# simonamtoft/downsampled-diffusion

Measured on AMD Instinct MI355X. Metric: images/sec (T=1000 sampling), 256x256 dDDPM-x3, higher is better.
Workload: dtype f32

## Files before the change

### downsampled-diffusion_amd/csrc/attention.hip

```cpp
#include <cstdlib>

#include "cluster_sync.h"
#include "conv_common.h"

namespace ddk {

constexpr int DH = 32;

constexpr int PART = DH + DH + DH * DH;

__global__ __launch_bounds__(256) void linattn_context_kernel(const float* __restrict__ qkv, float* __restrict__ ctx,
                                                              float* __restrict__ part, int HW, int heads, int splits, int rows_per_split,
                                                              int kv_only) {
    __shared__ __attribute__((aligned(16))) float stage[4 * 32 * 33];
    float* kexp = stage;
    float* vs = stage + 64 * DH;
    __shared__ float smax[8 * DH];
    const int bh = blockIdx.x / splits, sp = blockIdx.x % splits;
    const int b = bh / heads, h = bh % heads;
    const int HC = heads * DH, RS = (kv_only ? 2 : 3) * HC;
    const float* base = qkv + (long long)b * HW * RS;
    const float* kp = base + (kv_only ? 0 : HC) + h * DH;
    const float* vp = kp + HC;
    const int tid = threadIdx.x;
// ... 501 lines not shown
    if constexpr (ROWS >= 128) linattn_core_mfma<ROWS>(ks, vs, qs, cs, smax, part, ctx, out, b, h, HW, heads);
    else linattn_small_core<ROWS>(ks, vs, qs, cs, smax, ctx, out, b, h, HW, heads);
}

static size_t small_lds_bytes(int rows) {
    return ((size_t)rows * DH * 2 + (size_t)rows * (DH + 1) + DH * (DH + 4) + 16 * DH + (rows >= 128 ? 4 * 32 * 33 : 0)) * 4;
}

typedef float f32x4_att __attribute__((ext_vector_type(4)));
constexpr int QP_PITCH = 100;

__host__ __device__ static inline size_t small_qkv_lds_bytes(int MB, int C) {
    const size_t xs = (size_t)16 * MB * (C + 4), part = (size_t)4 * 16 * MB * QP_PITCH;
    const size_t core = 64 * DH * 2 + 64 * (DH + 1) + DH * (DH + 4) + 8 * DH + 128 + 192;
    return ((xs > part ? xs : part) + core) * 4;
}

template <int MB>
__global__ __launch_bounds__(256) void linattn_small_qkv_kernel(const float* __restrict__ x, const float* __restrict__ wop,
                                                                const float* __restrict__ c1, const float* __restrict__ c2, float ln_eps,
                                                                float* __restrict__ ctx, float* __restrict__ out, int HW, int C, int heads) {
    extern __shared__ __align__(16) float sm[];
    constexpr int ROWS = 16 * MB;
    const int pitch = C + 4, nch = C >> 5;
    const size_t big = (size_t)ROWS * pitch > (size_t)4 * ROWS * QP_PITCH ? (size_t)ROWS * pitch : (size_t)4 * ROWS * QP_PITCH;
    float* xs = sm;
    float* ks = sm + big;
    float* vs = ks + 64 * DH;
    float* qs = vs + 64 * DH;
    float* cs = qs + 64 * (DH + 1);
    float* smax = cs + DH * (DH + 4);
    float* rowstat = smax + 8 * DH;
    float* cfold = rowstat + 128;
    const int b = blockIdx.x / heads, h = blockIdx.x % heads;
    const int tid = threadIdx.x, lane = tid & 63;
    const int wave = __builtin_amdgcn_readfirstlane(tid >> 6);
    const int m = lane & 15, kq = lane >> 4;
    const int HC = heads * DH;

    const float* wl = wop + (size_t)h * nch * 3072 + lane * 4;
    float4 bA[6][2], bB[6][2];
    auto load_b = [&](int chunk, float4 (&bq)[6][2]) {
        chunk = chunk < nch ? chunk : nch - 1;
        const float* wp = wl + (size_t)chunk * 3072;
#pragma unroll
        for (int nb = 0; nb < 6; ++nb) {
            bq[nb][0] = *reinterpret_cast<const float4*>(wp + nb * 512);
            bq[nb][1] = *reinterpret_cast<const float4*>(wp + nb * 512 + 256);
        }
    };
    load_b(wave, bA);
    load_b(wave + 4, bB);
    if (tid < 192) {
        const int n = tid % 96;
        const int col = (n >> 5) * HC + h * DH + (n & 31);
        cfold[tid] = tid < 96 ? c1[col] : c2[col];
    }
    {
        const int q4 = C >> 2;
        for (int i = tid; i < ROWS * q4; i += 256) {
            const int row = i / q4, c = (i - row * q4) << 2;
            const float4 v = row < HW ? *reinterpret_cast<const float4*>(x + ((long long)b * HW + row) * C + c) : make_float4(0.f, 0.f, 0.f, 0.f);
            *reinterpret_cast<float4*>(xs + row * pitch + c) = v;
        }
    }
    __syncthreads();
    {
        constexpr int TPR = 256 / ROWS;
        const int row = tid / TPR, sub = tid % TPR;
        float s1 = 0.f;
        for (int c = sub * 4; c < C; c += TPR * 4) {
            const float4 v = *reinterpret_cast<const float4*>(xs + row * pitch + c);
            s1 += (v.x + v.y) + (v.z + v.w);
        }
#pragma unroll
        for (int o = 1; o < TPR; o <<= 1) s1 += __shfl_xor(s1, o, 64);
        const float inv_c = 1.0f / (float)C;
        const float mean = s1 * inv_c;
        float s2 = 0.f;
        for (int c = sub * 4; c < C; c += TPR * 4) {
            const float4 v = *reinterpret_cast<const float4*>(xs + row * pitch + c);
            const float a0 = v.x - mean, a1 = v.y - mean, a2 = v.z - mean, a3 = v.w - mean;
            s2 += (a0 * a0 + a1 * a1) + (a2 * a2 + a3 * a3);
        }
#pragma unroll
        for (int o = 1; o < TPR; o <<= 1) s2 += __shfl_xor(s2, o, 64);
        if (sub == 0) {
            const float var = s2 * inv_c;
            const float r = 1.0f / (sqrtf(var) + ln_eps);
            rowstat[2 * row] = r;
            rowstat[2 * row + 1] = r * mean;
        }
    }

    f32x4_att acc[MB][6];
#pragma unroll
    for (int i = 0; i < MB; ++i)
#pragma unroll
        for (int nb = 0; nb < 6; ++nb) acc[i][nb] = f32x4_att{0.f, 0.f, 0.f, 0.f};
    auto compute = [&](int chunk, const float4 (&bq)[6][2]) {
        float4 a[MB][2];
#pragma unroll
        for (int i = 0; i < MB; ++i) {
            const float* ap = xs + (i * 16 + m) * pitch + (chunk << 5) + kq * 8;
            a[i][0] = *reinterpret_cast<const float4*>(ap);
            a[i][1] = *reinterpret_cast<const float4*>(ap + 4);
        }
#pragma unroll
        for (int kk = 0; kk < 8; ++kk)
#pragma unroll
            for (int i = 0; i < MB; ++i) {
                const float av = reinterpret_cast<const float*>(&a[i][0])[kk];
#pragma unroll
                for (int nb = 0; nb < 6; ++nb)
                    acc[i][nb] = __builtin_amdgcn_mfma_f32_16x16x4f32(av, reinterpret_cast<const float*>(&bq[nb][0])[kk], acc[i][nb], 0, 0, 0);
            }
    };
    for (int c = wave; c < nch; c += 8) {
        compute(c, bA);
        load_b(c + 8, bA);
        if (c + 4 < nch) compute(c + 4, bB);
        load_b(c + 12, bB);
    }
    __syncthreads();
#pragma unroll
    for (int i = 0; i < MB; ++i)
#pragma unroll
        for (int nb = 0; nb < 6; ++nb)
#pragma unroll
            for (int r = 0; r < 4; ++r) xs[((wave * ROWS) + i * 16 + kq * 4 + r) * QP_PITCH + nb * 16 + m] = acc[i][nb][r];
    __syncthreads();
    for (int e = tid; e < ROWS * 96; e += 256) {
        const int row = e / 96, n = e - row * 96;
        const int sel = n >> 5, d = n & 31;
        float v = sel == 1 ? -INFINITY : 0.f;
        if (row < HW) {
            float s = xs[row * QP_PITCH + n];
#pragma unroll
            for (int w = 1; w < 4; ++w) s += xs[(w * ROWS + row) * QP_PITCH + n];
            v = rowstat[2 * row] * s - rowstat[2 * row + 1] * cfold[n] + cfold[96 + n];
        }
        if (sel == 0) qs[row * (DH + 1) + d] = v;
        else if (sel == 1) ks[row * DH + d] = v;
        else vs[row * DH + d] = v;
    }
    __syncthreads();
    linattn_small_core<ROWS>(ks, vs, qs, cs, smax, ctx, out, b, h, HW, heads);
}

constexpr int AS_REC = 1152;
constexpr int AS_CNT = 32;
constexpr int AS_RING = 4;

template <int ROWS>
struct AttnSplitGeom {
    static_assert(ROWS == 128 || ROWS == 32, "half of a 16x16 or of an 8x8 map");
    static constexpr int XP = ROWS / 8;
    static constexpr int NP = XP + 12;
    static constexpr int SLOT = (ROWS + 96) * 32;
    static constexpr int NB = ROWS == 128 ? 3 : 1;
    static constexpr int UNITS = ROWS == 128 ? 4 : 3;
    static constexpr int KPART = UNITS * NB * 16 * 64;
    static constexpr int SCR = KPART > 8 * 32 * 33 ? KPART : 8 * 32 * 33;
    static constexpr int RING_FL = AS_RING * SLOT;
    static_assert(SCR + 2 * ROWS * DH + ROWS * (DH + 1) <= RING_FL, "k, v, q of the half live behind the scratch area in the drained ring");
    static constexpr int TAIL = DH * (DH + 4) + 2 * ROWS + 16 * DH + 16 * DH + DH + 192 + AS_REC + 32;
    static constexpr int LDS_FL = RING_FL + TAIL;
};

struct AttnSplitParams {
    const float* x;
    const float* w;
    const float* c1;
    const float* c2;
    float eps;
    float* ctx;
    float* out;
    unsigned* cnt;
    float* rec;
    unsigned* fail;
    int C;
};

__device__ __forceinline__ void wait_vmcnt_le(int n) {
    if (n >= 8) wait_vmcnt<8>();
    else if (n >= 6) wait_vmcnt<6>();
    else if (n >= 4) wait_vmcnt<4>();
    else if (n >= 3) wait_vmcnt<3>();
    else if (n >= 2) wait_vmcnt<2>();
    else wait_vmcnt<0>();
}

template <int ROWS>
__global__ __launch_bounds__(512) void attn_split_kernel(const AttnSplitParams p) {
    using G = AttnSplitGeom<ROWS>;
    constexpr int HW = 2 * ROWS, HC = 4 * DH;
    extern __shared__ __attribute__((aligned(16))) float smem[];
    float* scr = smem;
    float* ks = smem + G::SCR;
    float* vs = ks + ROWS * DH;
    float* qs = vs + ROWS * DH;
    float* cs = smem + G::RING_FL;
    float* rowstat = cs + DH * (DH + 4);
    float* smax = rowstat + 2 * ROWS;
    float* dpart = smax + 16 * DH;
    float* mx = dpart + 16 * DH;
    float* cfold = mx + DH;
    float* own = cfold + 192;
    int* gave_up = reinterpret_cast<int*>(own + AS_REC);
    const int tid = threadIdx.x, lane = tid & 63;
    const int wid = __builtin_amdgcn_readfirstlane(tid >> 6);
    const int half = blockIdx.x, h = blockIdx.y, b = blockIdx.z;
    const int C = p.C, nch = C >> 5;
    const float* xb = p.x + ((long long)b * HW + half * ROWS) * C;
    const unsigned lds_base = (unsigned)(size_t)(__attribute__((address_space(3))) float*)smem;

    const int prow = lane >> 3, ppos = lane & 7;
    const int npw = (G::NP - wid + 7) >> 3;
    unsigned voff[4];
#pragma unroll
    for (int j = 0; j < 4; ++j) {
        const int pj = wid + 8 * j;
        const int r = 8 * (pj < G::XP ? pj : pj - G::XP) + prow;
        const int src = pj < G::XP ? r : (r >> 5) * HC + h * DH + (r & 31);
        voff[j] = (unsigned)((src * C + ((ppos ^ ((r >> 1) & 7)) << 2)) * 4);
    }
    auto issue = [&](int chunk) {
        const unsigned dst = lds_base + (unsigned)(((chunk & (AS_RING - 1)) * G::SLOT) * 4);
#pragma unroll
        for (int j = 0; j < 4; ++j) {
            const int pj = wid + 8 * j;
            if (pj < G::NP) lds_dma16_s(pj < G::XP ? xb : p.w, voff[j] + (unsigned)(chunk * 128), dst + (unsigned)(pj * 1024));
        }
    };
    for (int c = 0; c < AS_RING - 1 && c < nch; ++c) issue(c);
    if (tid < 192) {
        const int n = tid % 96;
        const int col = (n >> 5) * HC + h * DH + (n & 31);
        cfold[tid] = tid < 96 ? p.c1[col] : p.c2[col];
    }
    if (tid < 4 * ROWS) {
        const int row = tid >> 2, sub = tid & 3, n16 = C >> 4;
        const float4* rp = reinterpret_cast<const float4*>(xb + (long long)row * C);
        float4 v[16];
        float s = 0.f;
#pragma unroll
        for (int i = 0; i < 16; ++i)
            if (i < n16) {
                v[i] = rp[sub + 4 * i];
                s += (v[i].x + v[i].y) + (v[i].z + v[i].w);
            }
        s += __shfl_xor(s, 1, 64);
        s += __shfl_xor(s, 2, 64);
        const float inv_c = 1.0f / (float)C;
        const float mean = s * inv_c;
        float qq = 0.f;
#pragma unroll
        for (int i = 0; i < 16; ++i)
            if (i < n16) {
                const float a0 = v[i].x - mean, a1 = v[i].y - mean, a2 = v[i].z - mean, a3 = v[i].w - mean;
                qq += (a0 * a0 + a1 * a1) + (a2 * a2 + a3 * a3);
            }
        qq += __shfl_xor(qq, 1, 64);
        qq += __shfl_xor(qq, 2, 64);
        if (sub == 0) {
            const float r = 1.0f / (sqrtf(qq * inv_c) + p.eps);
            rowstat[2 * row] = r;
            rowstat[2 * row + 1] = r * mean;
        }
    }

    const int pl = lane & 31, hl = lane >> 5;
    const bool active = ROWS == 128 || wid < 6;
    const int kh = ROWS == 128 ? wid >> 2 : (wid >= 3 ? 1 : 0);
    const int unit = ROWS == 128 ? (wid & 3) : (wid >= 3 ? wid - 3 : wid);
    const int pb = ROWS == 128 ? unit : 0, blk0 = ROWS == 128 ? 0 : unit;
    f32x16 acc[G::NB];
#pragma unroll
    for (int i = 0; i < G::NB; ++i)
#pragma unroll
        for (int r = 0; r < 16; ++r) acc[i][r] = 0.f;
    const int fsw = (pl >> 1) & 7;
    for (int c = 0; c < nch; ++c) {
        const int later = nch - 1 - c < AS_RING - 2 ? nch - 1 - c : AS_RING - 2;
        wait_vmcnt_le(later * npw);
        asm volatile("s_waitcnt lgkmcnt(0)\n\ts_barrier" ::: "memory");
        if (c + AS_RING - 1 < nch) issue(c + AS_RING - 1);
        if (active) {
            const float* Xs = smem + (c & (AS_RING - 1)) * G::SLOT + pb * (32 * 32);
            const float* Ws = smem + (c & (AS_RING - 1)) * G::SLOT + ROWS * 32 + blk0 * (32 * 32);
#pragma unroll
            for (int q2 = 0; q2 < 2; ++q2) {
                const int off = pl * 32 + (((2 * (2 * kh + q2) + hl) ^ fsw) << 2);
                const float4 xv = *reinterpret_cast<const float4*>(Xs + off);
                float4 wv[G::NB];
#pragma unroll
                for (int i = 0; i < G::NB; ++i) wv[i] = *reinterpret_cast<const float4*>(Ws + i * (32 * 32) + off);
#pragma unroll
                for (int e = 0; e < 4; ++e) {
                    const float xe = e == 0 ? xv.x : e == 1 ? xv.y : e == 2 ? xv.z : xv.w;
#pragma unroll
                    for (int i = 0; i < G::NB; ++i)
                        acc[i] = __builtin_amdgcn_mfma_f32_32x32x2f32(e == 0 ? wv[i].x : e == 1 ? wv[i].y : e == 2 ? wv[i].z : wv[i].w, xe, acc[i], 0, 0, 0);
                }
            }
        }
    }
    __syncthreads();
    if (active && kh == 1) {
#pragma unroll
        for (int i = 0; i < G::NB; ++i)
#pragma unroll
            for (int r = 0; r < 16; ++r) scr[((unit * G::NB + i) * 16 + r) * 64 + lane] = acc[i][r];
    }
    __syncthreads();
    if (active && kh == 0) {
        const int n = pb * 32 + pl;
        const float r = rowstat[2 * n], rm = rowstat[2 * n + 1];
#pragma unroll
        for (int i = 0; i < G::NB; ++i) {
            const int blk = blk0 + i;
#pragma unroll
            for (int q = 0; q < 4; ++q) {
                const int d0 = 8 * q + 4 * hl;
                float o4[4];
#pragma unroll
                for (int e = 0; e < 4; ++e) {
                    const float a = acc[i][4 * q + e] + scr[((unit * G::NB + i) * 16 + 4 * q + e) * 64 + lane];
                    o4[e] = r * a - rm * cfold[blk * 32 + d0 + e] + cfold[96 + blk * 32 + d0 + e];
                }
                if (blk == 0) {
#pragma unroll
                    for (int e = 0; e < 4; ++e) qs[n * (DH + 1) + d0 + e] = o4[e];
                } else {
                    *reinterpret_cast<float4*>((blk == 1 ? ks : vs) + n * DH + d0) = make_float4(o4[0], o4[1], o4[2], o4[3]);
                }
            }
        }
    }
    __syncthreads();

    {
        const int d = tid & 31, ng = tid >> 5;
        float m = -INFINITY;
        for (int n = ng; n < ROWS; n += 16) m = fmaxf(m, ks[n * DH + d]);
        smax[ng * DH + d] = m;
        __syncthreads();
        if (tid < DH) {
            float mm = smax[tid];
#pragma unroll
            for (int j = 1; j < 16; ++j) mm = fmaxf(mm, smax[j * DH + tid]);
            mx[tid] = mm;
        }
        __syncthreads();
#pragma unroll
        for (int j = 0; j < ROWS / 16; ++j) {
            const int i = tid + j * 512;
            ks[i] = __expf(ks[i] - mx[i & 31]);
        }
        __syncthreads();
        float t = 0.f;
        for (int n = ng; n < ROWS; n += 16) t += ks[n * DH + d];
        dpart[ng * DH + d] = t;
    }
    {
        constexpr int RPW = ROWS / 8;
        f32x16 cacc;
#pragma unroll
        for (int r = 0; r < 16; ++r) cacc[r] = 0.f;
        const float* kp = ks + (wid * RPW + hl) * DH + pl;
        const float* vp = vs + (wid * RPW + hl) * DH + pl;
#pragma unroll
        for (int j = 0; j < RPW / 2; ++j) cacc = __builtin_amdgcn_mfma_f32_32x32x2f32(kp[j * 2 * DH], vp[j * 2 * DH], cacc, 0, 0, 0);
#pragma unroll
        for (int r = 0; r < 16; ++r) scr[(wid * 32 + (r & 3) + 8 * (r >> 2) + 4 * hl) * 33 + pl] = cacc[r];
    }
    __syncthreads();
    const int md = (tid >> 3) & 31, me0 = (tid & 7) * 4;
    if (tid < 256) {
        float den = 0.f;
#pragma unroll
        for (int g = 0; g < 16; ++g) den += dpart[g * DH + md];
#pragma unroll
        for (int e = 0; e < 4; ++e) {
            float t = scr[md * 33 + me0 + e];
#pragma unroll
            for (int w = 1; w < 8; ++w) t += scr[(w * 32 + md) * 33 + me0 + e];
            own[2 * DH + md * DH + me0 + e] = t;
        }
        if (me0 == 0) { own[md] = mx[md]; own[DH + md] = den; }
    }
    __syncthreads();
    unsigned* cnt = p.cnt + (b * 4 + h) * AS_CNT;
    float* rec = p.rec + (long long)(b * 4 + h) * 2 * AS_REC;
    if (wid == 0) {
        unsigned* mine = reinterpret_cast<unsigned*>(rec + half * AS_REC);
#pragma unroll
        for (int i = 0; i < (2 * DH + DH * DH) / 64; ++i)
            __hip_atomic_store(mine + lane + 64 * i, __float_as_uint(own[lane + 64 * i]), __ATOMIC_RELAXED, __HIP_MEMORY_SCOPE_AGENT);
        asm volatile("s_waitcnt vmcnt(0)" ::: "memory");
        if (lane == 0) {
            __hip_atomic_fetch_add(cnt, 1u, __ATOMIC_RELAXED, __HIP_MEMORY_SCOPE_AGENT);
            *gave_up = cl_wait_ge<2>(cnt, 2u, p.fail) ? 1 : 0;
        }
    }
    __syncthreads();
    const bool poisoned = *gave_up != 0;
    if (tid < 256) {
        const unsigned* theirs = reinterpret_cast<const unsigned*>(rec + (half ^ 1) * AS_REC);
        const float tm = __uint_as_float(__hip_atomic_load(theirs + md, __ATOMIC_RELAXED, __HIP_MEMORY_SCOPE_AGENT));
        const float td = __uint_as_float(__hip_atomic_load(theirs + DH + md, __ATOMIC_RELAXED, __HIP_MEMORY_SCOPE_AGENT));
        float ta[4];
#pragma unroll
        for (int e = 0; e < 4; ++e)
            ta[e] = __uint_as_float(__hip_atomic_load(theirs + 2 * DH + md * DH + me0 + e, __ATOMIC_RELAXED, __HIP_MEMORY_SCOPE_AGENT));
        if (tid == 0) cl_depart(cnt, cnt + 1, 2u);
        const float om = own[md], od = own[DH + md];
        const float m0 = half ? tm : om, m1 = half ? om : tm;
        const float d0 = half ? td : od, d1 = half ? od : td;
        const float M = fmaxf(m0, m1);
        const float w0 = expf(m0 - M), w1 = expf(m1 - M);
        float den = 0.f;
        den += d0 * w0;
        den += d1 * w1;
        const float inv = poisoned ? __builtin_nanf("") : 1.0f / den;
        float c4[4];
#pragma unroll
        for (int e = 0; e < 4; ++e) {
            const float oa = own[2 * DH + md * DH + me0 + e];
            const float a0 = half ? ta[e] : oa, a1 = half ? oa : ta[e];
            float a = 0.f;
            a += a0 * w0;
            a += a1 * w1;
            c4[e] = a * inv;
            cs[md * (DH + 4) + me0 + e] = c4[e];
        }
        if (half == 0) *reinterpret_cast<float4*>(p.ctx + (((long long)b * 4 + h) * DH + md) * DH + me0) = make_float4(c4[0], c4[1], c4[2], c4[3]);
    }
    __syncthreads();
    if (wid < ROWS / 32) {
        const int n0 = wid * 32;
        f32x16 oacc;
#pragma unroll
        for (int r = 0; r < 16; ++r) oacc[r] = 0.f;
        const float* qp = qs + (n0 + pl) * (DH + 1) + hl;
        const float* cp = cs + hl * (DH + 4) + pl;
#pragma unroll
        for (int j = 0; j < DH / 2; ++j) oacc = __builtin_amdgcn_mfma_f32_32x32x2f32(qp[2 * j], cp[2 * j * (DH + 4)], oacc, 0, 0, 0);
        float* op = p.out + ((long long)b * HW + half * ROWS + n0) * HC + h * DH + pl;
#pragma unroll
        for (int r = 0; r < 16; ++r) op[((r & 3) + 8 * (r >> 2) + 4 * hl) * HC] = oacc[r];
    }
}

__global__ __launch_bounds__(256) void qkv_operand_pack_kernel(const float* __restrict__ lnw, float* __restrict__ wop, int heads, int cp,
                                                               long long total) {
    const int nch = cp >> 5, HC = heads * DH;
    for (long long idx = blockIdx.x * 256LL + threadIdx.x; idx < total; idx += (long long)gridDim.x * 256) {
        const int j = (int)(idx & 3), lane = (int)((idx >> 2) & 63), half = (int)((idx >> 8) & 1);
        long long r = idx >> 9;
        const int nb = (int)(r % 6); r /= 6;
        const int chunk = (int)(r % nch);
        const int head = (int)(r / nch);
        const int o = (nb >> 1) * HC + head * DH + (nb & 1) * 16 + (lane & 15);
        const int i = chunk * 32 + (lane >> 4) * 8 + half * 4 + j;
        wop[idx] = lnw[(long long)o * cp + i];
    }
}

typedef float f32x16_att __attribute__((ext_vector_type(16)));
__global__ __launch_bounds__(512) void linattn_apply_kernel(const float* __restrict__ qkv, const float* __restrict__ ctx,
                                                            float* __restrict__ out, int HW, int heads, int tiles_per_sample) {
    extern __shared__ __attribute__((aligned(16))) float qs[];
    const int b = blockIdx.x / tiles_per_sample, tile = blockIdx.x % tiles_per_sample;
    const int HC = heads * DH, RS = 3 * HC;
    const int nthreads = 64 * heads;
    const int n0 = tile * 64;
    const int f4_per_row = HC / 4;
    for (int i = threadIdx.x; i < 64 * f4_per_row; i += nthreads) {
        const int row = i / f4_per_row, c4 = i - row * f4_per_row;
        float4 v = make_float4(0.f, 0.f, 0.f, 0.f);
        if (n0 + row < HW) v = *reinterpret_cast<const float4*>(qkv + ((long long)b * HW + n0 + row) * RS + c4 * 4);
        const int hh = (c4 * 4) / DH, d = (c4 * 4) % DH;
        float* dst = qs + (hh * 64 + row) * 33 + d;
        dst[0] = v.x; dst[1] = v.y; dst[2] = v.z; dst[3] = v.w;
    }
    const int h = threadIdx.x >> 6, lane = threadIdx.x & 63;
    const int l31 = lane & 31, fh = lane >> 5;
    const float* cp = ctx + ((long long)b * heads + h) * DH * DH + l31;
    float bf[16];
#pragma unroll
    for (int kk = 0; kk < 16; ++kk) bf[kk] = cp[(2 * kk + fh) * DH];
    __syncthreads();
    const float* qh = qs + h * 64 * 33;
    f32x16_att acc0, acc1;
#pragma unroll
    for (int r = 0; r < 16; ++r) { acc0[r] = 0.f; acc1[r] = 0.f; }
#pragma unroll
    for (int kk = 0; kk < 16; ++kk) {
        const float a0 = qh[l31 * 33 + 2 * kk + fh], a1 = qh[(32 + l31) * 33 + 2 * kk + fh];
        acc0 = __builtin_amdgcn_mfma_f32_32x32x2f32(a0, bf[kk], acc0, 0, 0, 0);
        acc1 = __builtin_amdgcn_mfma_f32_32x32x2f32(a1, bf[kk], acc1, 0, 0, 0);
    }
#pragma unroll
    for (int r = 0; r < 16; ++r) {
        const int px = (r & 3) + 8 * (r >> 2) + 4 * fh;
        if (n0 + px < HW) out[((long long)b * HW + n0 + px) * HC + h * DH + l31] = acc0[r];
        if (n0 + 32 + px < HW) out[((long long)b * HW + n0 + 32 + px) * HC + h * DH + l31] = acc1[r];
    }
}

static void linattn_splits(int B, int HW, int heads, int& splits, int& rows) {
    const int max_s = (int)ceil_div(HW, 64);
#ifdef DDK_TUNING
    const char* cap_env = getenv("DDK_LINATTN_WGS");
    const int cap = cap_env ? atoi(cap_env) : 1024;
#else
    const int cap = 1024;
#endif
    int s = cap / (B * heads);
    if (s < 1) s = 1;
    if (s > max_s) s = max_s;
    rows = (int)(ceil_div(ceil_div(HW, s), 64) * 64);
    splits = (int)ceil_div(HW, rows);
}

size_t linattn_context_workspace_bytes(int B, int HW, int heads) {
    if (B <= 0 || HW <= 0 || heads <= 0) return 0;
    int s, rows;
    linattn_splits(B, HW, heads, s, rows);
    return s > 1 ? (size_t)B * heads * s * PART * sizeof(float) : 0;
}

int linattn_context(const float* qkv, float* ctx, int B, int HW, int heads, void* workspace, size_t workspace_bytes, hipStream_t st,
                    bool kv_only) {
    DDK_REQUIRE(qkv && ctx && B > 0 && HW > 0 && heads > 0, "linattn_context: arguments");
    DDK_REQUIRE(aligned16(qkv) && aligned16(ctx) && aligned16(workspace), "linattn_context: alignment");
    int s, rows;
    linattn_splits(B, HW, heads, s, rows);
    if (s > 1 && (!workspace || workspace_bytes < (size_t)B * heads * s * PART * sizeof(float))) {
        if (workspace) {
            set_error("linattn_context: workspace too small (%zu < %zu)", workspace_bytes, (size_t)B * heads * s * PART * sizeof(float));
            return DDK_ERR_WORKSPACE;
        }
        s = 1;
        rows = HW;
    }
    hipLaunchKernelGGL(linattn_context_kernel, dim3(B * heads * s), dim3(256), 0, st, qkv, ctx, static_cast<float*>(workspace), HW, heads, s, rows,
                       kv_only ? 1 : 0);
    DDK_TRY(check_launch("linattn_context_kernel"));
    if (s > 1) {
        hipLaunchKernelGGL(linattn_merge_kernel, dim3(B * heads), dim3(256), 0, st, static_cast<const float*>(workspace), ctx, s);
        DDK_TRY(check_launch("linattn_merge_kernel"));
    }
    return DDK_OK;
}

int linattn_fused_small(const float* qkv, float* ctx, float* out, int B, int HW, int heads, hipStream_t st) {
    DDK_REQUIRE(qkv && ctx && out && B > 0 && HW > 0 && HW <= 256 && heads > 0, "linattn_fused_small: arguments (HW <= 256)");
    DDK_REQUIRE(aligned16(qkv) && aligned16(ctx) && aligned16(out), "linattn_fused_small: alignment");
    DDK_TRY(ensure_device_init());
    if (HW <= 64)
        hipLaunchKernelGGL(linattn_small_kernel<64>, dim3(B * heads), dim3(256), small_lds_bytes(64), st, qkv, ctx, out, HW, heads);
    else
        hipLaunchKernelGGL(linattn_small_kernel<256>, dim3(B * heads), dim3(256), small_lds_bytes(256), st, qkv, ctx, out, HW, heads);
    return check_launch("linattn_small_kernel");
}

bool linattn_small_qkv_ok(int HW, int C) { return HW > 0 && HW <= 64 && C % 32 == 0 && C >= 32 && small_qkv_lds_bytes(HW <= 16 ? 1 : 4, C) <= 160 * 1024; }

constexpr int FOLD_C = 128;
constexpr int FOLD_LDS_FLOATS = FOLD_C * FOLD_C + 32 * (FOLD_C + 1) + 2 * FOLD_C;
typedef float f32x16_att __attribute__((ext_vector_type(16)));
__global__ __launch_bounds__(256) void attn_fold_kernel(const float* __restrict__ ctx, const float* __restrict__ wqg,
                                                        const float* __restrict__ c1q, const float* __restrict__ c2q,
                                                        const float* __restrict__ wout, const float* __restrict__ bout,
                                                        float* __restrict__ A, float* __restrict__ a1, float* __restrict__ a2) {
    extern __shared__ __align__(16) float sm[];
    float* T = sm;
    float* Wq = T + FOLD_C * FOLD_C;
    float* t1 = Wq + 32 * (FOLD_C + 1);
    float* t2 = t1 + FOLD_C;
    const int b = blockIdx.x, nq = blockIdx.y, tid = threadIdx.x, lane = tid & 63;
    const int wave = __builtin_amdgcn_readfirstlane(tid >> 6);
    const int l31 = lane & 31, kh = lane >> 5;
    {
        const float* cp = ctx + ((long long)b * 4 + wave) * DH * DH;
        const float* wp = wqg + (long long)wave * DH * FOLD_C;
        f32x16_att acc[4];
#pragma unroll
        for (int j = 0; j < 4; ++j)
#pragma unroll
            for (int r = 0; r < 16; ++r) acc[j][r] = 0.f;
        float av[DH / 2], bv[DH / 2][4];
#pragma unroll
        for (int s2 = 0; s2 < DH / 2; ++s2) {
            const int d = 2 * s2 + kh;
            av[s2] = cp[d * DH + l31];
#pragma unroll
            for (int j = 0; j < 4; ++j) bv[s2][j] = wp[d * FOLD_C + j * 32 + l31];
        }
        __builtin_amdgcn_sched_barrier(0);
#pragma unroll
        for (int s2 = 0; s2 < DH / 2; ++s2)
#pragma unroll
            for (int j = 0; j < 4; ++j) acc[j] = __builtin_amdgcn_mfma_f32_32x32x2f32(av[s2], bv[s2][j], acc[j], 0, 0, 0);
#pragma unroll
        for (int j = 0; j < 4; ++j)
#pragma unroll
            for (int r = 0; r < 16; ++r) T[(wave * DH + (r & 3) + 8 * (r >> 2) + 4 * kh) * FOLD_C + j * 32 + l31] = acc[j][r];
    }
    for (int i = tid; i < 32 * FOLD_C; i += 256) Wq[(i >> 7) * (FOLD_C + 1) + (i & 127)] = wout[(long long)nq * 32 * FOLD_C + i];
    if (tid < FOLD_C) {
        const int h = tid >> 5, e = tid & 31;
        const float* ch = ctx + ((long long)b * 4 + h) * DH * DH;
        float u1 = 0.f, u2 = 0.f;
#pragma unroll
        for (int d = 0; d < DH; ++d) {
            const float cv = ch[d * DH + e];
            u1 += cv * c1q[h * DH + d];
            u2 += cv * c2q[h * DH + d];
        }
        t1[tid] = u1;
        t2[tid] = u2;
    }
    __syncthreads();
    {
        f32x16_att acc;
#pragma unroll
        for (int r = 0; r < 16; ++r) acc[r] = 0.f;
#pragma unroll 8
        for (int s2 = 0; s2 < FOLD_C / 2; ++s2) {
            const int he = 2 * s2 + kh;
            acc = __builtin_amdgcn_mfma_f32_32x32x2f32(Wq[l31 * (FOLD_C + 1) + he], T[he * FOLD_C + wave * 32 + l31], acc, 0, 0, 0);
        }
        float* Ab = A + ((long long)b * FOLD_C + nq * 32) * FOLD_C + wave * 32 + l31;
#pragma unroll
        for (int r = 0; r < 16; ++r) Ab[((r & 3) + 8 * (r >> 2) + 4 * kh) * FOLD_C] = acc[r];
        if (tid < 32) {
            float u1 = 0.f, u2 = 0.f;
#pragma unroll 16
            for (int he = 0; he < FOLD_C; ++he) {
                u1 += Wq[tid * (FOLD_C + 1) + he] * t1[he];
                u2 += Wq[tid * (FOLD_C + 1) + he] * t2[he];
            }
            const int n = nq * 32 + tid;
            a1[(long long)b * FOLD_C + n] = u1;
            a2[(long long)b * FOLD_C + n] = u2 + (bout ? bout[n] : 0.f);
        }
    }
}

int linattn_small_qkv_init_device() {
    DDK_HIP(hipFuncSetAttribute(reinterpret_cast<const void*>(attn_kvctx_kernel), hipFuncAttributeMaxDynamicSharedMemorySize,
                                (int)(KC_LDS_FLOATS * sizeof(float))));
    DDK_HIP(hipFuncSetAttribute(reinterpret_cast<const void*>(attn_fold_kernel), hipFuncAttributeMaxDynamicSharedMemorySize,
                                (int)(FOLD_LDS_FLOATS * sizeof(float))));
    DDK_HIP(hipFuncSetAttribute(reinterpret_cast<const void*>(linattn_small_kernel<256>), hipFuncAttributeMaxDynamicSharedMemorySize, 160 * 1024));
    DDK_HIP(hipFuncSetAttribute(reinterpret_cast<const void*>(linattn_small_qkv_kernel<1>), hipFuncAttributeMaxDynamicSharedMemorySize, 160 * 1024));
    DDK_HIP(hipFuncSetAttribute(reinterpret_cast<const void*>(linattn_small_qkv_kernel<4>), hipFuncAttributeMaxDynamicSharedMemorySize, 160 * 1024));
    DDK_HIP(hipFuncSetAttribute(reinterpret_cast<const void*>(attn_split_kernel<128>), hipFuncAttributeMaxDynamicSharedMemorySize,
                                (int)(AttnSplitGeom<128>::LDS_FL * sizeof(float))));
    DDK_HIP(hipFuncSetAttribute(reinterpret_cast<const void*>(attn_split_kernel<32>), hipFuncAttributeMaxDynamicSharedMemorySize,
                                (int)(AttnSplitGeom<32>::LDS_FL * sizeof(float))));
    return DDK_OK;
}

int qkv_operand_pack(const float* lnw, float* wop, int heads, int cp, hipStream_t st) {
    DDK_REQUIRE(lnw && wop && heads > 0 && cp > 0 && cp % 32 == 0, "qkv_operand_pack: arguments");
    const long long total = (long long)3 * heads * DH * cp;
    const long long blocks = ceil_div(total, 256);
    hipLaunchKernelGGL(qkv_operand_pack_kernel, dim3((unsigned)(blocks < 2048 ? blocks : 2048)), dim3(256), 0, st, lnw, wop, heads, cp, total);
    return check_launch("qkv_operand_pack_kernel");
}

int linattn_small_qkv(const float* x, const float* wop, const float* c1, const float* c2, float ln_eps, float* ctx, float* out, int B, int HW,
                      int C, int heads, hipStream_t st) {
    DDK_REQUIRE(x && wop && c1 && c2 && ctx && out && B > 0 && heads > 0, "linattn_small_qkv: arguments");
    DDK_REQUIRE(linattn_small_qkv_ok(HW, C), "linattn_small_qkv: needs H*W <= 64 and C % 32 == 0 (LDS budget)");
    DDK_REQUIRE(aligned16(x) && aligned16(wop) && aligned16(ctx) && aligned16(out), "linattn_small_qkv: alignment");
    DDK_TRY(ensure_device_init());
    if (HW <= 16)
        hipLaunchKernelGGL(linattn_small_qkv_kernel<1>, dim3(B * heads), dim3(256), small_qkv_lds_bytes(1, C), st, x, wop, c1, c2, ln_eps, ctx, out,
                           HW, C, heads);
    else
        hipLaunchKernelGGL(linattn_small_qkv_kernel<4>, dim3(B * heads), dim3(256), small_qkv_lds_bytes(4, C), st, x, wop, c1, c2, ln_eps, ctx, out,
                           HW, C, heads);
    return check_launch("linattn_small_qkv_kernel");
}

bool attn_kvctx_ok(int B, int HW, int C, int heads) { return B > 0 && C == KC_K && heads == 4 && HW >= 4 * KC_BM && HW % KC_BM == 0; }
int attn_kvctx_splits(int B, int HW) {
    const int tiles = HW / KC_BM;
    int s = 1;
    while (s * 2 <= tiles && tiles % (s * 2) == 0 && (long long)B * 2 * (s * 2) <= 256) s *= 2;
    return s;
}
size_t attn_kvctx_workspace_bytes(int B, int HW) { return (size_t)B * 4 * attn_kvctx_splits(B, HW) * PART * sizeof(float); }

int attn_kvctx(const float* x, const float* w_kv, const float* c1, const float* c2, float ln_eps, float* ctx, int B, int HW, void* workspace,
               size_t workspace_bytes, hipStream_t st) {
    DDK_REQUIRE(x && w_kv && c1 && c2 && ctx && workspace, "attn_kvctx: null pointer");
    DDK_REQUIRE(attn_kvctx_ok(B, HW, KC_K, 4), "attn_kvctx: needs 128 channels, 4 heads, H*W a multiple of 64 and >= 256");
    DDK_REQUIRE(aligned16(x) && aligned16(w_kv) && aligned16(c1) && aligned16(c2) && aligned16(ctx) && aligned16(workspace), "attn_kvctx: alignment");
    DDK_REQUIRE((long long)B * HW * KC_K * 4 < (1LL << 32) && B <= 65535, "attn_kvctx: input of 4 GiB or more, or more than 65535 images");
    const int s = attn_kvctx_splits(B, HW);
    if (workspace_bytes < attn_kvctx_workspace_bytes(B, HW)) {
        set_error("attn_kvctx: workspace too small (%zu < %zu)", workspace_bytes, attn_kvctx_workspace_bytes(B, HW));
        return DDK_ERR_WORKSPACE;
    }
    DDK_TRY(ensure_device_init());
    KvCtxParams p{x, w_kv, c1, c2, ln_eps, static_cast<float*>(workspace), HW / KC_BM, HW / KC_BM / s, s};
    hipLaunchKernelGGL(attn_kvctx_kernel, dim3((unsigned)s, 2, (unsigned)B), dim3(512), KC_LDS_FLOATS * sizeof(float), st, p);
    DDK_TRY(check_launch("attn_kvctx_kernel"));
    hipLaunchKernelGGL(linattn_merge_kernel, dim3(B * 4), dim3(256), 0, st, static_cast<const float*>(workspace), ctx, s);
    return check_launch("linattn_merge_kernel");
}

constexpr int AS_CUS = 256;
bool attn_split_ok(int B, int HW, int C, int heads) {
    return B > 0 && (HW == 64 || HW == 256) && C >= 32 && C <= 256 && C % 32 == 0 && heads == 4 && 8 * (long long)B <= AS_CUS &&
           conv_wino_cluster_device_ok();
}
size_t attn_split_counter_words(int B) { return (size_t)B * 4 * AS_CNT; }
size_t attn_split_record_floats(int B) { return (size_t)B * 4 * 2 * AS_REC; }
size_t attn_split_workspace_bytes(int B) { return B > 0 ? (32 + attn_split_counter_words(B) + attn_split_record_floats(B)) * sizeof(float) : 0; }
unsigned attention_cluster_timeouts() { return cl_timeouts_read(); }

int attn_split(const float* x, const float* w, const float* c1, const float* c2, float ln_eps, float* ctx, float* out, int B, int HW, int C,
               unsigned* counters, float* records, unsigned* fail, hipStream_t st) {
    DDK_REQUIRE(x && w && c1 && c2 && ctx && out && counters && records, "attn_split: null pointer");
    DDK_REQUIRE(attn_split_ok(B, HW, C, 4), "attn_split: needs H*W of 64 or 256, C % 32 == 0, C <= 256, 4 heads, 8 * B <= the CU count of a whole MI355X");
    DDK_REQUIRE(aligned16(x) && aligned16(w) && aligned16(ctx) && aligned16(out) && aligned16(counters) && aligned16(records), "attn_split: alignment");
    DDK_TRY(ensure_device_init());
    const AttnSplitParams p{x, w, c1, c2, ln_eps, ctx, out, counters, records, fail, C};
    if (HW == 256)
        hipLaunchKernelGGL(attn_split_kernel<128>, dim3(2, 4, (unsigned)B), dim3(512), AttnSplitGeom<128>::LDS_FL * sizeof(float), st, p);
    else
        hipLaunchKernelGGL(attn_split_kernel<32>, dim3(2, 4, (unsigned)B), dim3(512), AttnSplitGeom<32>::LDS_FL * sizeof(float), st, p);
    return check_launch("attn_split_kernel");
}

bool attn_fold_ok(int C, int heads) { return C == FOLD_C && heads * DH == FOLD_C; }
size_t attn_fold_out_floats(int B) { return (size_t)B * (FOLD_C * FOLD_C + 2 * FOLD_C); }

int attn_fold(const float* ctx, const float* wqg, const float* c1q, const float* c2q, const float* wout, const float* bout, float* A,
              float* a1, float* a2, int B, int C, int heads, hipStream_t st) {
    DDK_REQUIRE(ctx && wqg && c1q && c2q && wout && A && a1 && a2 && B > 0, "attn_fold: arguments");
    DDK_REQUIRE(attn_fold_ok(C, heads), "attn_fold: C == 128 and heads * 32 == 128 only");
    DDK_REQUIRE(aligned16(ctx) && aligned16(wout) && aligned16(A), "attn_fold: alignment");
    DDK_TRY(ensure_device_init());
    hipLaunchKernelGGL(attn_fold_kernel, dim3(B, 4), dim3(256), FOLD_LDS_FLOATS * sizeof(float), st, ctx, wqg, c1q, c2q, wout, bout, A, a1, a2);
    return check_launch("attn_fold_kernel");
}

int linattn_apply(const float* qkv, const float* ctx, float* out, int B, int HW, int heads, hipStream_t st) {
    DDK_REQUIRE(qkv && ctx && out && B > 0 && HW > 0, "linattn_apply: arguments");
    DDK_REQUIRE(heads >= 1 && heads <= 8, "linattn_apply: heads must be in 1..8");
    DDK_REQUIRE(aligned16(qkv) && aligned16(ctx) && aligned16(out), "linattn_apply: alignment");
    const int tiles = (int)ceil_div(HW, 64);
    const size_t lds = (size_t)heads * 64 * 33 * sizeof(float);
    hipLaunchKernelGGL(linattn_apply_kernel, dim3(B * tiles), dim3(64 * heads), lds, st, qkv, ctx, out, HW, heads, tiles);
    return check_launch("linattn_apply_kernel");
}

}

extern "C" {
size_t ddk_linattn_context_workspace_bytes(int B, int HW, int heads) { return ddk::linattn_context_workspace_bytes(B, HW, heads); }
int ddk_linattn_context(const float* qkv, float* ctx, int B, int HW, int heads, void* workspace, size_t workspace_bytes, ddk_stream_t s) {
    return ddk::linattn_context(qkv, ctx, B, HW, heads, workspace, workspace_bytes, ddk::as_stream(s), false);
}
int ddk_linattn_context_kv(const float* kv, float* ctx, int B, int HW, int heads, void* workspace, size_t workspace_bytes, ddk_stream_t s) {
    return ddk::linattn_context(kv, ctx, B, HW, heads, workspace, workspace_bytes, ddk::as_stream(s), true);
}
size_t ddk_attention_kv_context_workspace_bytes(int B, int HW) { return ddk::attn_kvctx_workspace_bytes(B, HW); }
int ddk_attention_kv_context_ok(int B, int HW, int C, int heads) { return ddk::attn_kvctx_ok(B, HW, C, heads) ? 1 : 0; }
int ddk_attention_kv_context(const float* x, const float* w_kv, const float* c1, const float* c2, float ln_eps, float* ctx, int B, int HW,
                             void* workspace, size_t workspace_bytes, ddk_stream_t s) {
    return ddk::attn_kvctx(x, w_kv, c1, c2, ln_eps, ctx, B, HW, workspace, workspace_bytes, ddk::as_stream(s));
}
size_t ddk_attention_split_workspace_bytes(int B) { return ddk::attn_split_workspace_bytes(B); }
int ddk_attention_split_ok(int B, int HW, int C, int heads) { return ddk::attn_split_ok(B, HW, C, heads) ? 1 : 0; }
int ddk_attention_split_from_x(const float* x, const float* w_folded, const float* c1, const float* c2, float ln_eps, float* ctx, float* out,
                               int B, int HW, int C, int heads, void* workspace, size_t workspace_bytes, ddk_stream_t s) {
    using namespace ddk;
    DDK_REQUIRE(workspace && B > 0 && heads == 4, "attention_split_from_x: arguments (4 heads)");
    if (workspace_bytes < attn_split_workspace_bytes(B)) {
        set_error("attention_split_from_x: workspace too small (%zu < %zu)", workspace_bytes, attn_split_workspace_bytes(B));
        return DDK_ERR_WORKSPACE;
    }
    unsigned* words = static_cast<unsigned*>(workspace);
    return attn_split(x, w_folded, c1, c2, ln_eps, ctx, out, B, HW, C, words + 32, static_cast<float*>(workspace) + 32 + attn_split_counter_words(B),
                      words, as_stream(s));
}
int ddk_attention_fold(const float* ctx, const float* wqg, const float* c1q, const float* c2q, const float* wout, const float* bout, float* A,
                       float* a1, float* a2, int B, int C, int heads, ddk_stream_t s) {
    return ddk::attn_fold(ctx, wqg, c1q, c2q, wout, bout, A, a1, a2, B, C, heads, ddk::as_stream(s));
}
int ddk_linattn_fused_small(const float* qkv, float* ctx, float* out, int B, int HW, int heads, ddk_stream_t s) {
    return ddk::linattn_fused_small(qkv, ctx, out, B, HW, heads, ddk::as_stream(s));
}
int ddk_pack_qkv_operand(const float* folded_w, float* dst, int heads, int c_pad, ddk_stream_t s) {
    return ddk::qkv_operand_pack(folded_w, dst, heads, c_pad, ddk::as_stream(s));
}
int ddk_linattn_small_from_x(const float* x, const float* w_operand, const float* c1, const float* c2, float ln_eps, float* ctx, float* out,
                             int B, int HW, int C, int heads, ddk_stream_t s) {
    return ddk::linattn_small_qkv(x, w_operand, c1, c2, ln_eps, ctx, out, B, HW, C, heads, ddk::as_stream(s));
}
int ddk_linattn_apply(const float* qkv, const float* ctx, float* out, int B, int HW, int heads, ddk_stream_t s) {
    return ddk::linattn_apply(qkv, ctx, out, B, HW, heads, ddk::as_stream(s));
}
}
```

### downsampled-diffusion_amd/csrc/ddk_internal.h

```cpp
#pragma once
#include <hip/hip_runtime.h>

#include <cstdarg>
#include <cstddef>
#include <cstdint>
#include <cstdio>

#include "ddk.h"

#ifdef DDK_HOST_SANITIZE
#include "host_sanitize.h"
#endif

namespace ddk {

void set_error(const char* fmt, ...);

inline int fail_arg(const char* what) {
    set_error("bad argument: %s", what);
    return DDK_ERR_ARG;
}

inline int check_launch(const char* what) {
    hipError_t e = hipGetLastError();
// ... 67 lines not shown
    const int lane = threadIdx.x & 63, wid = threadIdx.x >> 6, nw = blockDim.x >> 6;
    __syncthreads();
    if (lane == 0) red[wid] = v;
    __syncthreads();
    float t = (lane < nw) ? red[lane] : 0.0f;
    t = wave_sum(t);
    return t;
}

__device__ __forceinline__ float block_max(float v, float* red) {
    v = wave_max(v);
    const int lane = threadIdx.x & 63, wid = threadIdx.x >> 6, nw = blockDim.x >> 6;
    __syncthreads();
    if (lane == 0) red[wid] = v;
    __syncthreads();
    float t = (lane < nw) ? red[lane] : -INFINITY;
    t = wave_max(t);
    return t;
}

int ensure_device_init();
int conv_init_device();
int wgrad_init_device();

size_t conv_workspace_bytes(int kind, int B, int H, int W, int cin, int N);
struct ConvLnFold {
    const float* c1;
    const float* c2;
    float eps;
};
struct WinoGnFuse {
    const float* gamma;
    const float* beta;
    const float* temb;
    const long long* temb_rows;
    int temb_stride;
    float eps;
    int groups;
    float* records;
    unsigned* counters;
    unsigned* fail;
    unsigned* pairs = nullptr;
    const float* res_x = nullptr;
    const float* res_w = nullptr;
    const float* res_b = nullptr;
    int res_cin = 0, res_ld = 0;
};
bool conv_ln_fold_ok(int B, int H, int W, int cin, int N);
int conv_forward(const ddk_conv_args& a, hipStream_t st, const ConvLnFold* ln = nullptr, const WinoGnFuse* fuse = nullptr);
int conv_splits(int kind, int B, int H, int W, int cin, int N);
bool conv_wino_ok(int kind, int H, int W, int cin, int N);
int conv_wino_splits(int B, int H, int W, int cin, int N);
int conv_wino_forward(const ddk_conv_args& a, int splits, hipStream_t st, const WinoGnFuse* fuse = nullptr);
int conv_wino_cluster_np(int B, int H, int W, int cin, int N, int groups);
int conv_wino_cluster_split_np(int B, int H, int W, int cin, int N, int groups, int* splits_out);
size_t conv_wino_cluster_pair_words(int B, int H, int W, int N);
bool conv_wino_variant_new(int B, int H, int W, int N);
bool conv_wino_cluster_device_ok();
size_t conv_wino_cluster_ws_floats(int B, int H, int W, int N);
unsigned conv_wino_cluster_timeouts();
unsigned conv_first_cluster_timeouts();
unsigned level_chain_cluster_timeouts();
unsigned attention_cluster_timeouts();
constexpr size_t CL_PAIR_WORDS = 128 * 16;
inline size_t cl_fail_offset(int B) { return (size_t)B * 8 * 16; }
inline size_t cl_front_floats(int B) { return cl_fail_offset(B) + 16; }
inline size_t cl_chain_offset(int B) { return cl_front_floats(B); }
inline size_t cl_pair_offset(int B) { return cl_chain_offset(B) + (size_t)B * 64; }
inline size_t cl_attn_offset(int B) { return cl_pair_offset(B) + CL_PAIR_WORDS; }
inline size_t cl_counter_floats(int B) { return cl_attn_offset(B) + (size_t)B * 4 * 32; }
struct ClWords { unsigned* counters; unsigned* fail; };
inline ClWords cl_words(float* cl, int B) { return {reinterpret_cast<unsigned*>(cl), reinterpret_cast<unsigned*>(cl + cl_fail_offset(B))}; }
int cluster_fail_check(unsigned* word, hipStream_t st, const char* who, const char* tail);
bool convT_wino_ok(int H, int W, int cin, int N);
int convT_wino_splits(int B, int H, int W, int cin, int N);
int convT_wino_forward(const ddk_conv_args& a, int splits, hipStream_t st);
int conv_wino_init_device();
int conv_wino_stats_parts(int B, int H, int W, int cin, int N, int groups);
bool conv_first_ok(int cin, int N, int H, int W, int groups);
int conv_first(const float* x, const float* wp, const float* bias, float* out, float* gn_partials, int B, int H, int W, int cin, int N,
               int groups, int64_t* counter, int64_t* t_cur, hipStream_t st);
int conv_first_init_device();
bool conv_first_gn_ok(int cin, int N, int H, int W, int groups);
size_t conv_first_gn_ws_floats(int B, int H, int W);
int conv_first_gn(const float* x, const float* wp, const float* bias, const float* gamma, const float* beta, const float* temb,
                  int temb_stride, const long long* temb_rows, float eps, float* out, int B, int H, int W, int cin, int N, int groups,
                  float* records, unsigned* counters, unsigned* fail, int64_t* counter, int64_t* t_cur, hipStream_t st);
bool conv1x1_sm_ok(long long M, int c0, int c1, int N);
int conv1x1_sm(const float* src0, int c0, const float* src1, int c1, const float* w, const float* bias, const float* resid, float* out,
               long long M, int N, const ConvLnFold* ln, hipStream_t st);
int conv1x1_sm_init_device();
bool conv1x1_stream_ok(long long M, int cin, int N);
int conv1x1_stream(const float* x, int cin, const float* w, const float* bias, const float* dmish_src, const float* resid, float* out,
                   float* mish_out, long long M, int N, int pre_mish, int post_mish, hipStream_t st);
bool conv1x1_ws_ok(long long M, int K, int N);
int conv1x1_ws(const float* x, const float* w, const float* bias, const float* resid, float* out, long long M, int N, const ConvLnFold* ln,
               hipStream_t st, int images = 0);
int conv1x1_ws_init_device();
struct AddendSlabs {
    int n = 1;
    long long stride = 0;
    const float* bias = nullptr;
};
bool conv_gn_local_ok(int H, int W, int cin, int c0, int N, int groups);
int conv_gn_local(const float* src0, int c0, const float* src1, int c1, const float* w, const float* bias, const float* gamma,
                  const float* beta, const float* temb, int temb_stride, const long long* temb_rows, const float* addend, float* out,
                  int B, int H, int W, int N, int groups, float eps, hipStream_t st, const AddendSlabs& as = AddendSlabs(),
                  const AddendSlabs& src_slabs = AddendSlabs());
int conv_gn_local_init_device();
bool conv_gn_wlocal_ok(int H, int W, int cin, int c0, int N, int groups);
int conv_gn_wlocal(const float* src0, int c0, const float* src1, int c1, const float* w, const float* bias, const float* gamma,
                   const float* beta, const float* temb, int temb_stride, const long long* temb_rows, const float* addend, float* out,
                   int B, int H, int W, int N, int groups, float eps, hipStream_t st, const AddendSlabs& as = AddendSlabs(),
                   const AddendSlabs& src_slabs = AddendSlabs());
double conv_flops(int kind, int B, int H, int W, int cin, int N);
size_t groupnorm_workspace_bytes(int B, int HW, int C, int groups);
int gn_train_nsplit(int HW, int cpg);
int gn_stats_partials(const float* x, float* part, int B, int HW, int C, int groups, int ns, hipStream_t st);
int groupnorm_mish(const float* x, const float* gamma, const float* beta, const float* temb, int temb_stride,
                   const float* addend, float* out, int B, int HW, int C, int groups, float eps, void* ws, size_t ws_bytes,
                   hipStream_t st, const long long* temb_rows = nullptr);
int groupnorm_mish_ex(const float* x, int nslab, long long slab_stride, const float* cbias, const float* gamma,
                      const float* beta, const float* temb, int temb_stride, const float* addend, float* out, int B, int HW, int C,
                      int groups, float eps, void* ws, size_t ws_bytes, hipStream_t st, const long long* temb_rows = nullptr);
int groupnorm_mish_parts(const float* x, const float* part, int np, const float* gamma, const float* beta, const float* temb,
                         int temb_stride, const float* addend, float* out, int B, int HW, int C, int groups, float eps, hipStream_t st,
                         const long long* temb_rows = nullptr, const float* rc_x = nullptr, const float* rc_w = nullptr,
                         const float* rc_b = nullptr, int rc_cin = 0, int rc_ld = 0);
int chan_layernorm(const float* x, const float* g, const float* b, float* out, long long M, int C, float eps, hipStream_t st);
int groupnorm_mish_generic(const float* x, const float* gamma, const float* beta, const float* temb, int temb_stride, const float* addend,
                           float* out, int B, int HW, int CP, int C, int groups, float eps, hipStream_t st, const long long* temb_rows = nullptr);
int chan_layernorm_generic(const float* x, const float* g, const float* b, float* out, long long M, int CP, int C, float eps, hipStream_t st);
int unary(int op, const float* x, float* out, long long n, hipStream_t st);
int add(const float* a, const float* b, float* out, long long n, hipStream_t st);
int avgpool2(const float* x, float* out, int B, int H, int W, int C, hipStream_t st);
int upsample_nearest2(const float* x, float* out, int B, int H, int W, int C, hipStream_t st);
size_t linattn_context_workspace_bytes(int B, int HW, int heads);
int linattn_context(const float* qkv, float* ctx, int B, int HW, int heads, void* workspace, size_t workspace_bytes, hipStream_t st,
                    bool kv_only = false);
bool attn_fold_ok(int C, int heads);
bool attn_kvctx_ok(int B, int HW, int C, int heads);
size_t attn_kvctx_workspace_bytes(int B, int HW);
int attn_kvctx(const float* x, const float* w_kv, const float* c1, const float* c2, float ln_eps, float* ctx, int B, int HW, void* workspace,
               size_t workspace_bytes, hipStream_t st);
size_t attn_fold_out_floats(int B);
int attn_fold(const float* ctx, const float* wqg, const float* c1q, const float* c2q, const float* wout, const float* bout, float* A,
              float* a1, float* a2, int B, int C, int heads, hipStream_t st);
int linattn_apply(const float* qkv, const float* ctx, float* out, int B, int HW, int heads, hipStream_t st);
int linattn_fused_small(const float* qkv, float* ctx, float* out, int B, int HW, int heads, hipStream_t st);
bool attn_split_ok(int B, int HW, int C, int heads);
size_t attn_split_counter_words(int B);
size_t attn_split_record_floats(int B);
int attn_split(const float* x, const float* w, const float* c1, const float* c2, float ln_eps, float* ctx, float* out, int B, int HW, int C,
               unsigned* counters, float* records, unsigned* fail, hipStream_t st);
bool linattn_small_qkv_ok(int HW, int C);
int linattn_small_qkv_init_device();
int qkv_operand_pack(const float* lnw, float* wop, int heads, int cp, hipStream_t st);
int linattn_small_qkv(const float* x, const float* wop, const float* c1, const float* c2, float ln_eps, float* ctx, float* out, int B, int HW,
                      int C, int heads, hipStream_t st);
int time_mlp(const int64_t* t, const float* freqs, const float* w1t, const float* b1, const float* w2t, const float* b2,
             float* act, float* raw, int B, int dim, hipStream_t st);
int time_proj(const float* act, const float* wt, const float* bias, float* out, int B, int dim, int n_out, hipStream_t st);
int conv1x1_small_n(const float* x, const float* w, const float* bias, float* out, long long M, int C, int n_out, hipStream_t st);
struct InpaintOps {
    const float* known;
    const float* mask;
    const float *ka, *kb;
    const float *ja, *jb;
};
struct NoisyTables {
    const float *lam, *sgm;
};
constexpr uint32_t INPAINT_Z2_BIT = 0x40000000u;
constexpr uint32_t INPAINT_Z3_BIT = 0x20000000u;
struct RestoreOps {
    const float* y;
    int n;
    int H, W;
    int gray;
    const float* mask;
};
static_assert(sizeof(RestoreOps) == 32 && offsetof(RestoreOps, mask) == 24, "RestoreOps: gray fills the padding, nothing moves");
constexpr int GRAY_MEAN = 1;
constexpr int GRAY_LUMA = 2;
struct VlbStep {
    const float* x;
    float* xt;
    const float* noise;
    long long noise_step_stride;
    int t_first;
    const float *c_recip, *c_recipm1, *c1, *c2, *logvar;
    float* partials;
    int nslot;
};
constexpr uint32_t VLB_STREAM_BIT = 0x80000000u;

enum class StepKind {
    Eps,
    Ancestral,
    Multistep,
    Inpaint,
    Restore,
    RestoreMasked,
    Vlb,
    RestoreMultistep,
    RestoreNoisy,
    RestoreGray
};
struct StepRule {
    StepKind kind;
    float* eps_out;
    float* x;
    const float* noise;
    long long noise_step_stride;
    int t_first;
    const float *c_recip, *c_recipm1, *c1, *c2, *sigma;
    float* x0_hist;
    const float* c3;
    union {
        InpaintOps inp;
        NoisyTables nsy;
    };
    const VlbStep* vlb;
    RestoreOps rst;
};
inline StepRule vlb_rule(const VlbStep& v) {
    StepRule r{};
    r.kind = StepKind::Vlb;
    r.x = const_cast<float*>(v.x); r.noise = v.noise; r.noise_step_stride = v.noise_step_stride; r.t_first = v.t_first;
    r.c_recip = v.c_recip; r.c_recipm1 = v.c_recipm1; r.c1 = v.c1; r.c2 = v.c2;
    r.vlb = &v;
    return r;
}
struct ChainHooks {
    const int64_t* chain_state;
    int64_t* dec_counter;
    uint64_t seed;
    uint32_t stream_id;
};
int p_update(const StepRule& r, const float* eps_hat, const int64_t* t, int B, long long per, const ChainHooks& h, hipStream_t st,
             const char* who = "p_update");
int randn(float* out, long long n, uint64_t seed, uint32_t step, uint32_t stream_id, hipStream_t st);
int vlb_sweep_slots_unfused(int B, long long per);
int vlb_step_input(const VlbStep& v, const float* sqrt_acp, const float* sqrt_1m_acp, const int64_t* chain_state, int B, long long per,
                   hipStream_t st);
int vlb_sweep_finalize(const float* partials, int nslot, float* vlb_t, float* l_simple_t, int T, int B, long long per, hipStream_t st);
struct TailIn {
    const float* raw;
    const float* part;
    int np;
    const float *gamma, *beta;
    float eps;
    const float* w;
    const float* bias;
    int n_out, B, HW, C, groups;
};
bool final_tail_ok(int HW, int C, int groups, int n_out, int np, StepKind kind, int restore_w = 0, int restore_n = 0);
int final_tail(const TailIn& in, const StepRule& r, const int64_t* t, const ChainHooks& h, hipStream_t st);

}
```

### downsampled-diffusion_amd/csrc/unet_plan.hip

```cpp
#include <algorithm>
#include <mutex>
#include <string>
#include <vector>

#include "ddk_internal.h"
#include "level_chain.h"

namespace ddk {

constexpr int HEADS = 4;
constexpr int HIDDEN = HEADS * 32;
constexpr int GROUPS = 8;
constexpr float GN_EPS = 1e-5f, LN_EPS = 1e-5f;

static inline int pad32(int c) { return (c + 31) / 32 * 32; }

enum PackKind { PK_COPY = 0, PK_CONV = 1, PK_CONVT = 2, PK_LINEAR_T = 3, PK_WINO = 4, PK_LOCAL = 5, PK_WLOCAL = 6, PK_FIRST = 7, PK_CONVT_WINO = 8,
                PK_ROWS = 9 , PK_LOCAL1 = 10 ,
                PK_CONVT_LOCAL = 11  };

struct Slot {
    std::string name;
    long long numel;
    int kind;
    size_t off;
    int O, I, KH, KW, i_pad, ld, col0;
    int split = 0, split_pad = 0;
    int attn = -1;
};

struct ConvW {
    size_t w = 0, b = 0;
    bool has_bias = false;
    int cin = 0, cin_pad = 0, cout = 0;
    size_t wu = 0;
    bool has_wu = false;
    size_t wl = 0;
    bool has_wl = false;
    size_t wwl = 0;
    bool has_wwl = false;
    size_t wf = 0;
    bool has_wf = false;
    size_t wl1 = 0;
    bool has_wl1 = false;
    size_t wtl = 0;
    bool has_wtl = false;
};
struct NormW { size_t g = 0, b = 0; int c_real = 0; };
struct ResW {
    int ci = 0, ci_pad = 0, co = 0, temb_off = 0, ci_real = 0, co_real = 0;
    ConvW c1, c2, res;
    NormW n1, n2;
    bool has_res = false;
};
struct AttnW {
    int c = 0, c_real = 0;
    NormW ln;
    ConvW qkv, out;
    size_t qkv_lnw = 0, ln_c1 = 0, ln_c2 = 0;
    size_t qkv_op = 0;
};

}

using namespace ddk;

struct ChainKey {
    StepKind kind;
    const void* bufs[14];
    const void* ws;
    const void* noise;
    int B, H, W, t_start, device;
    unsigned long long pack_epoch;
    int restore_n = 0;
    bool restore_mask = false;
    int restore_gray = 0;
    bool operator==(const ChainKey& o) const {
        for (int i = 0; i < 14; ++i)
            if (bufs[i] != o.bufs[i]) return false;
        return kind == o.kind && ws == o.ws && noise == o.noise && B == o.B && H == o.H && W == o.W && t_start == o.t_start &&
               device == o.device && pack_epoch == o.pack_epoch && restore_n == o.restore_n && restore_mask == o.restore_mask && restore_gray == o.restore_gray;
    }
};
struct SamplerGraph {
    ChainKey key;
    hipGraph_t graph = nullptr;
    hipGraphExec_t exec = nullptr;
    hipGraph_t graph_multi = nullptr;
    hipGraphExec_t exec_multi = nullptr;
    hipEvent_t done = nullptr;
    unsigned long long last_use = 0;
};
constexpr int SAMPLER_MULTI = 16;

struct ddk_unet {
    std::mutex mu;
    std::vector<SamplerGraph> graphs;
    unsigned long long use_clock = 0;
    unsigned long long pack_epoch = 0;
    struct {
        const void* ws = nullptr;
        int t_start = -1, B = 0, H = 0, W = 0;
        unsigned long long pack_epoch = 0;
        std::vector<int64_t> map;
    } table;
    ddk_unet_config cfg;
    int cluster_gn = 1;
    int cluster_limit = 1 << 30;
    int cluster_np_max = 8;
    bool cluster_split = true;
    bool attn_kvctx = true;
    bool attn_split = true;
    bool fold_down_reduce = false;
    bool restore_fused = true;
    bool first_gn = true;
    int level_chain = 9;
    int level_chain_max_batch = 32;
    int attn_fold_min_hw = 256;
    bool attn_fold = true;
    bool generic = false;
    std::vector<int> dimp;
    std::vector<Slot> slots;
    size_t packed_floats = 0;
    int L = 0;
    std::vector<int> dims;
    int time_dim = 0, temb_total = 0;
    size_t freqs = 0, w1t = 0, b1 = 0, w2t = 0, b2 = 0, temb_wt = 0, temb_bias = 0;
    std::vector<ResW> down_res, up_res;
    std::vector<AttnW> down_attn, up_attn;
    std::vector<ConvW> down_conv, up_conv;
    ResW mid1, mid2;
    AttnW mid_attn;
    ConvW final_conv;
    NormW final_norm;
    size_t final_w = 0, final_b = 0;

    size_t alloc(size_t n) {
        const size_t o = packed_floats;
        packed_floats += (n + 3) / 4 * 4;
        return o;
    }
    size_t add_copy(const std::string& name, long long n) {
        const size_t o = alloc((size_t)n);
        slots.push_back(Slot{name, n, PK_COPY, o, 0, 0, 0, 0, 0, 0, 0});
        return o;
    }
    void add_copy_at(const std::string& name, long long n, size_t off) {
        slots.push_back(Slot{name, n, PK_COPY, off, 0, 0, 0, 0, 0, 0, 0});
    }
    ConvW add_conv(const std::string& prefix, int cout, int cin, int k, bool bias, bool gn_follows = false, int split = 0, bool local = false) {
        ConvW c;
        c.cin = cin; c.cin_pad = split > 0 ? pad32(split) + pad32(cin - split) : pad32(cin); c.cout = cout;
        const int cout_rows = pad32(cout);
        c.w = alloc((size_t)cout_rows * k * k * c.cin_pad);
        Slot sl{prefix + "weight", (long long)cout * cin * k * k, PK_CONV, c.w, cout, cin, k, k, c.cin_pad, 0, 0};
        if (split > 0 && c.cin_pad != cin) { sl.split = split; sl.split_pad = pad32(split); }
        slots.push_back(sl);
        c.has_bias = bias;
        if (bias) {
            c.b = alloc((size_t)cout_rows);
            slots.push_back(Slot{prefix + "bias", cout, PK_COPY, c.b, 0, 0, 0, 0, 0, 0, 0});
        }
        if (generic) return c;
        if (k == 1 && bias && cout % 32 == 0 && c.cin_pad == cin && cin % 32 == 0) {
            c.wl1 = alloc((size_t)cout * c.cin_pad);
            c.has_wl1 = true;
            slots.push_back(Slot{prefix + "weight", (long long)cout * cin, PK_LOCAL1, c.wl1, cout, cin, 1, 1, c.cin_pad, 0, 0});
        }
        if (k == 3 && cout % 64 == 0) {
            c.wu = alloc((size_t)16 * cout * c.cin_pad);
            c.has_wu = true;
            slots.push_back(Slot{prefix + "weight", (long long)cout * cin * k * k, PK_WINO, c.wu, cout, cin, k, k, c.cin_pad, 0, 0});
        }
        if (k == 3 && (gn_follows || local) && cout % 32 == 0) {
            c.wl = alloc((size_t)9 * cout * c.cin_pad);
            c.has_wl = true;
            slots.push_back(Slot{prefix + "weight", (long long)cout * cin * k * k, PK_LOCAL, c.wl, cout, cin, k, k, c.cin_pad, 0, 0});
            if (gn_follows && (c.cin_pad <= 320 || c.cin_pad == 512)) {
                c.wwl = alloc((size_t)16 * cout * c.cin_pad);
                c.has_wwl = true;
                slots.push_back(Slot{prefix + "weight", (long long)cout * cin * k * k, PK_WLOCAL, c.wwl, cout, cin, k, k, c.cin_pad, 0, 0});
            }
        }
        return c;
    }
    ConvW add_convT(const std::string& prefix, int ch, bool local = false) {
        ConvW c;
        c.cin = ch; c.cin_pad = pad32(ch); c.cout = ch;
        c.w = alloc((size_t)16 * pad32(ch) * pad32(ch));
        slots.push_back(Slot{prefix + "weight", (long long)16 * ch * ch, PK_CONVT, c.w, ch, ch, 4, 4, pad32(ch), 0, 0});
        c.has_bias = true;
        c.b = alloc((size_t)pad32(ch));
        slots.push_back(Slot{prefix + "bias", ch, PK_COPY, c.b, 0, 0, 0, 0, 0, 0, 0});
        if (local && ch % 32 == 0 && !generic) {
            c.wtl = alloc((size_t)16 * ch * ch);
            c.has_wtl = true;
            slots.push_back(Slot{prefix + "weight", (long long)16 * ch * ch, PK_CONVT_LOCAL, c.wtl, ch, ch, 4, 4, ch, 0, 0});
        }
        if (ch % 128 == 0) {
            c.wu = alloc((size_t)36 * ch * ch);
            c.has_wu = true;
            slots.push_back(Slot{prefix + "weight", (long long)16 * ch * ch, PK_CONVT_WINO, c.wu, ch, ch, 4, 4, ch, 0, 0});
        }
        return c;
    }
    NormW add_norm(const std::string& wname, const std::string& bname, int c) {
        NormW n;
        n.c_real = c;
        n.g = alloc((size_t)pad32(c));
        slots.push_back(Slot{wname, c, PK_COPY, n.g, 0, 0, 0, 0, 0, 0, 0});
        n.b = alloc((size_t)pad32(c));
        slots.push_back(Slot{bname, c, PK_COPY, n.b, 0, 0, 0, 0, 0, 0, 0});
        return n;
    }
    ResW add_res(const std::string& p, int ci, int co, int& temb_cursor, int split = 0) {
        ResW r;
        r.ci_real = ci; r.co_real = co;
        r.ci = ci; r.ci_pad = split > 0 ? pad32(split) + pad32(ci - split) : pad32(ci); r.co = pad32(co);
        if (!generic) r.co = co;
        r.temb_off = temb_cursor;
        temb_cursor += co;
        slots.push_back(Slot{p + "mlp.1.weight", (long long)co * time_dim, PK_LINEAR_T, temb_wt, co, time_dim, 0, 0, 0, temb_total, r.temb_off});
        add_copy_at(p + "mlp.1.bias", co, temb_bias + r.temb_off);
        r.c1 = add_conv(p + "block1.block.0.", co, ci, 3, true, true, split);
        r.n1 = add_norm(p + "block1.block.1.weight", p + "block1.block.1.bias", co);
        r.c2 = add_conv(p + "block2.block.0.", co, co, 3, true, true);
        r.n2 = add_norm(p + "block2.block.1.weight", p + "block2.block.1.bias", co);
        r.has_res = ci != co;
        if (r.has_res) r.res = add_conv(p + "res_conv.", co, ci, 1, true, false, split);
        return r;
    }
    int n_attn = 0;
    std::vector<AttnW> attn_all;
    AttnW add_attn(const std::string& p, int c) {
        AttnW a;
        a.c = generic ? pad32(c) : c;
        a.c_real = c;
        const size_t s0 = slots.size();
        a.qkv = add_conv(p + "fn.fn.to_qkv.", 3 * HIDDEN, c, 1, false);
        const size_t s1 = slots.size();
        a.out = add_conv(p + "fn.fn.to_out.", c, HIDDEN, 1, true);
        const size_t s2 = slots.size();
        a.ln = add_norm(p + "fn.norm.g", p + "fn.norm.b", c);
        for (size_t i = s0; i < s1; ++i) slots[i].attn = n_attn;
        for (size_t i = s2; i < slots.size(); ++i) slots[i].attn = n_attn;
        a.qkv_lnw = alloc((size_t)3 * HIDDEN * pad32(c));
        a.ln_c1 = alloc((size_t)3 * HIDDEN);
        a.ln_c2 = alloc((size_t)3 * HIDDEN);
        a.qkv_op = alloc((size_t)3 * HIDDEN * pad32(c));
        attn_all.push_back(a);
        ++n_attn;
        return a;
    }
};

static int total_temb(const ddk_unet& u) {
    int tot = 0;
    for (int l = 0; l < u.L; ++l) tot += 2 * u.dims[l + 1];
    tot += 2 * u.dims[u.L];
    for (int i = 0; i < u.L - 1; ++i) tot += 2 * u.dims[u.L - 1 - i];
    return tot;
}

extern "C" ddk_unet* ddk_unet_create(const ddk_unet_config* cfg) {
    if (!cfg || cfg->n_levels < 1 || cfg->n_levels > 8 || cfg->in_ch < 1 || cfg->chan < 8 || cfg->chan % 8 ||
        cfg->chan > 512) {
        set_error("unet_create: need 1 <= n_levels <= 8, in_ch >= 1, unet_chan a multiple of 8 in [8, 512]");
        return nullptr;
    }
    for (int i = 0; i < cfg->n_levels; ++i)
        if (cfg->mults[i] < 1) { set_error("unet_create: unet_dims entries must be >= 1"); return nullptr; }
    if (cfg->mults[0] != 1) {
        set_error("unet_create: unet_dims[0] must be 1 (the reference's final Block(dim, dim) meets dim * unet_dims[0] channels "
                  "otherwise and raises, unet.py:69-72)");
        return nullptr;
    }
    {
        int ndev = 0;
        if (hipGetDeviceCount(&ndev) == hipSuccess && ndev > 0 && ensure_device_init() != DDK_OK) return nullptr;
        (void)hipGetLastError();
    }
    ddk_unet* u = new ddk_unet();
    u->cfg = *cfg;
    u->L = cfg->n_levels;
    u->generic = cfg->chan % 32 != 0;
    for (int i = 0; i < cfg->n_levels; ++i)
        if (cfg->chan * cfg->mults[i] > 512) { set_error("unet_create: level widths above 512 channels are not supported"); delete u; return nullptr; }
    u->dims.push_back(cfg->in_ch);
    for (int i = 0; i < u->L; ++i) u->dims.push_back(cfg->chan * cfg->mults[i]);
    for (int d : u->dims) u->dimp.push_back(u->generic ? pad32(d) : d);
    u->time_dim = cfg->chan;
    u->temb_total = total_temb(*u);
    const int td = u->time_dim;

    u->freqs = u->add_copy("@sinusoidal_freqs", td / 2);
    u->w1t = u->alloc((size_t)td * 4 * td);
    u->slots.push_back(Slot{"time_mlp.1.weight", (long long)4 * td * td, PK_LINEAR_T, u->w1t, 4 * td, td, 0, 0, 0, 4 * td, 0});
    u->b1 = u->add_copy("time_mlp.1.bias", 4 * td);
    u->w2t = u->alloc((size_t)4 * td * td);
    u->slots.push_back(Slot{"time_mlp.3.weight", (long long)4 * td * td, PK_LINEAR_T, u->w2t, td, 4 * td, 0, 0, 0, td, 0});
    u->b2 = u->add_copy("time_mlp.3.bias", td);
    u->temb_wt = u->alloc((size_t)td * u->temb_total);
    u->temb_bias = u->alloc((size_t)u->temb_total);

    int cur = 0;
    for (int l = 0; l < u->L; ++l) {
        const std::string p = "downs." + std::to_string(l) + ".";
        const int ci = u->dims[l], co = u->dims[l + 1];
        u->down_res.push_back(u->add_res(p + "0.", ci, co, cur));
        if (l == 0 && ci <= 8 && co <= 256 && !u->generic) {
            ConvW& c1 = u->down_res[0].c1;
            const int K2 = (9 * ci + 1) / 2;
            c1.wf = u->alloc((size_t)(co / 32) * K2 * 64);
            c1.has_wf = true;
            u->slots.push_back(Slot{p + "0.block1.block.0.weight", (long long)co * ci * 9, PK_FIRST, c1.wf, co, ci, 3, 3, 0, 0, 0});
        }
        u->down_res.push_back(u->add_res(p + "1.", co, co, cur));
        u->down_attn.push_back(u->add_attn(p + "2.", co));
        if (l < u->L - 1) u->down_conv.push_back(u->add_conv(p + "3.conv.", co, co, 3, true, false, 0, l == u->L - 2));
    }
    const int mid = u->dims[u->L];
    u->mid1 = u->add_res("mid_block1.", mid, mid, cur);
    u->mid_attn = u->add_attn("mid_attn.", mid);
    u->mid2 = u->add_res("mid_block2.", mid, mid, cur);
    for (int i = 0; i < u->L - 1; ++i) {
        const std::string p = "ups." + std::to_string(i) + ".";
        const int din = u->dims[u->L - 1 - i], dout = u->dims[u->L - i];
        u->up_res.push_back(u->add_res(p + "0.", 2 * dout, din, cur, dout));
        u->up_res.push_back(u->add_res(p + "1.", din, din, cur));
        u->up_attn.push_back(u->add_attn(p + "2.", din));
        u->up_conv.push_back(u->add_convT(p + "3.conv.", din, i == 0));
    }
    u->final_conv = u->add_conv("final_conv.0.block.0.", cfg->chan, cfg->chan, 3, true, true);
    u->final_norm = u->add_norm("final_conv.0.block.1.weight", "final_conv.0.block.1.bias", cfg->chan);
    if (u->generic) {
        u->final_w = u->alloc((size_t)cfg->in_ch * pad32(cfg->chan));
        u->slots.push_back(Slot{"final_conv.1.weight", (long long)cfg->in_ch * cfg->chan, PK_ROWS, u->final_w, cfg->in_ch, cfg->chan, 0, 0, 0,
                                pad32(cfg->chan), 0});
    } else {
        u->final_w = u->add_copy("final_conv.1.weight", (long long)cfg->in_ch * cfg->chan);
    }
    u->final_b = u->add_copy("final_conv.1.bias", cfg->in_ch);
    if (cur != u->temb_total) {
        set_error("unet_create: internal temb accounting mismatch");
        delete u;
        return nullptr;
    }
    return u;
}

static void drop_graphs(ddk_unet* u) {
    for (SamplerGraph& g : u->graphs) {
        if (g.exec) (void)hipGraphExecDestroy(g.exec);
        if (g.graph) (void)hipGraphDestroy(g.graph);
        if (g.exec_multi) (void)hipGraphExecDestroy(g.exec_multi);
        if (g.graph_multi) (void)hipGraphDestroy(g.graph_multi);
        if (g.done) (void)hipEventDestroy(g.done);
    }
    u->graphs.clear();
    u->table.ws = nullptr;
}

extern "C" void ddk_unet_destroy(ddk_unet* u) {
    if (!u) return;
    if (!u->graphs.empty()) (void)hipDeviceSynchronize();
    drop_graphs(u);
    delete u;
}

extern "C" int ddk_sampler_invalidate(ddk_unet* u) {
    DDK_REQUIRE(u, "sampler_invalidate: null plan");
    std::lock_guard<std::mutex> lock(u->mu);
    if (!u->graphs.empty()) DDK_HIP(hipDeviceSynchronize());
    drop_graphs(u);
    return DDK_OK;
}
static void destroy_entry(SamplerGraph& g) {
    if (g.done) { (void)hipEventSynchronize(g.done); (void)hipEventDestroy(g.done); }
    if (g.exec) (void)hipGraphExecDestroy(g.exec);
    if (g.graph) (void)hipGraphDestroy(g.graph);
    if (g.exec_multi) (void)hipGraphExecDestroy(g.exec_multi);
    if (g.graph_multi) (void)hipGraphDestroy(g.graph_multi);
}

extern "C" int ddk_sampler_release_workspace(ddk_unet* u, const void* workspace) {
    DDK_REQUIRE(u && workspace, "sampler_release_workspace: arguments");
    std::lock_guard<std::mutex> lock(u->mu);
    for (size_t i = 0; i < u->graphs.size();) {
        if (u->graphs[i].key.ws == workspace) {
            destroy_entry(u->graphs[i]);
            u->graphs.erase(u->graphs.begin() + (long)i);
        } else {
            ++i;
        }
    }
    if (u->table.ws == workspace) u->table.ws = nullptr;
    return DDK_OK;
}

extern "C" int ddk_unet_set_option(ddk_unet* u, int option, int value) {
    DDK_REQUIRE(u, "unet_set_option: null plan");
    static const struct {
        int option;
        bool drops_graphs;
        void (*set)(ddk_unet&, int);
    } options[] = {
        {DDK_OPT_CLUSTER_GROUPNORM, true, [](ddk_unet& p, int v) { p.cluster_gn = v < 0 ? 0 : v > 2 ? 2 : v; }},
        {DDK_OPT_ATTENTION_FOLD, true, [](ddk_unet& p, int v) { p.attn_fold = v != 0; }},
        {DDK_OPT_ATTENTION_KV_CONTEXT, true, [](ddk_unet& p, int v) { p.attn_kvctx = v != 0; }},
        {DDK_OPT_FIRST_GROUPNORM, true, [](ddk_unet& p, int v) { p.first_gn = v != 0; }},
        {DDK_OPT_RESTORE_FUSED_TAIL, true, [](ddk_unet& p, int v) { p.restore_fused = v != 0; }},
        {DDK_OPT_ATTENTION_SPLIT, true, [](ddk_unet& p, int v) { p.attn_split = v != 0; }},
        {DDK_OPT_LEVEL_CHAIN, true, [](ddk_unet& p, int v) {
             p.level_chain = v == 1 ? 9 : v == 2 ? 1 : v == 3 ? 15 : v == 4 ? 6 : v == 8 ? 2 : v == 16 ? 4 : v != 0 ? 9 : 0;
         }},
        {DDK_OPT_FOLD_DOWNSAMPLE_REDUCE, true, [](ddk_unet& p, int v) { p.fold_down_reduce = v != 0; }},
        {10, true, [](ddk_unet& p, int v) { p.level_chain_max_batch = v; }},
        {9, true, [](ddk_unet& p, int v) { p.attn_fold_min_hw = v; }},
        {2, false, [](ddk_unet& p, int v) { p.cluster_limit = v; }},
        {4, true, [](ddk_unet& p, int v) { p.cluster_np_max = v; }},
        {11, true, [](ddk_unet& p, int v) { p.cluster_split = v != 0; }},
    };
    for (const auto& o : options) {
        if (o.option != option) continue;
        std::lock_guard<std::mutex> lock(u->mu);
        if (o.drops_graphs) {
            if (!u->graphs.empty()) DDK_HIP(hipDeviceSynchronize());
            drop_graphs(u);
        }
        o.set(*u, value);
        return DDK_OK;
    }
    return fail_arg("unet_set_option: unknown option");
}
extern "C" unsigned ddk_debug_cluster_timeouts(void) {
    unsigned sum = 0;
    for (unsigned v : {ddk::conv_wino_cluster_timeouts(), ddk::conv_first_cluster_timeouts(), ddk::level_chain_cluster_timeouts(),
                       ddk::attention_cluster_timeouts()}) {
        if (v == ~0u) return ~0u;
        sum += v;
    }
    return sum;
}
extern "C" int ddk_unet_num_slots(const ddk_unet* u) { return u ? (int)u->slots.size() : 0; }
extern "C" const char* ddk_unet_slot_name(const ddk_unet* u, int slot) {
    return (u && slot >= 0 && slot < (int)u->slots.size()) ? u->slots[slot].name.c_str() : nullptr;
}
extern "C" long long ddk_unet_slot_numel(const ddk_unet* u, int slot) {
    return (u && slot >= 0 && slot < (int)u->slots.size()) ? u->slots[slot].numel : -1;
}
extern "C" size_t ddk_unet_packed_bytes(const ddk_unet* u) { return u ? u->packed_floats * sizeof(float) : 0; }

__global__ __launch_bounds__(64) void ln_fold_kernel(const float* __restrict__ w, const float* __restrict__ g, const float* __restrict__ b,
                                                     float* __restrict__ wg, float* __restrict__ c1, float* __restrict__ c2, int C, int cp) {
    const int n = blockIdx.x;
    float s1 = 0.f, s2 = 0.f;
    for (int c = threadIdx.x; c < cp; c += 64) {
        const float wv = w[(long long)n * cp + c];
        const float gv = c < C ? g[c] : 0.f, bv = c < C ? b[c] : 0.f;
        wg[(long long)n * cp + c] = wv * gv;
        s1 += wv * gv;
        s2 += wv * bv;
    }
    s1 = wave_sum(s1);
    s2 = wave_sum(s2);
    if (threadIdx.x == 0) { c1[n] = s1; c2[n] = s2; }
}

static int fold_attn(const AttnW& a, float* P, hipStream_t st) {
    hipLaunchKernelGGL(ln_fold_kernel, dim3(3 * HIDDEN), dim3(64), 0, st, P + a.qkv.w, P + a.ln.g, P + a.ln.b, P + a.qkv_lnw, P + a.ln_c1,
                       P + a.ln_c2, a.c, pad32(a.c));
    DDK_TRY(check_launch("ln_fold_kernel"));
    return qkv_operand_pack(P + a.qkv_lnw, P + a.qkv_op, HEADS, pad32(a.c), st);
}

static void weights_changed(const ddk_unet* u) {
    ddk_unet* m = const_cast<ddk_unet*>(u);
    std::lock_guard<std::mutex> lock(m->mu);
    ++m->pack_epoch;
}

extern "C" int ddk_unet_finalize_pack(const ddk_unet* u, void* packed, ddk_stream_t s) {
    DDK_REQUIRE(u && packed, "unet_finalize_pack: arguments");
    weights_changed(u);
    for (const AttnW& a : u->attn_all) DDK_TRY(fold_attn(a, static_cast<float*>(packed), as_stream(s)));
    return DDK_OK;
}

extern "C" int ddk_unet_pack_slot(const ddk_unet* u, int slot, const float* canonical, void* packed, ddk_stream_t s) {
    DDK_REQUIRE(u && canonical && packed && slot >= 0 && slot < (int)u->slots.size(), "unet_pack_slot: arguments");
    const Slot& sl = u->slots[slot];
    float* dst = static_cast<float*>(packed) + sl.off;
    weights_changed(u);
    int rc;
    switch (sl.kind) {
        case PK_COPY:
            DDK_HIP(hipMemcpyAsync(dst, canonical, (size_t)sl.numel * sizeof(float), hipMemcpyDeviceToDevice, as_stream(s)));
            rc = DDK_OK;
            break;
        case PK_CONV:
            rc = sl.split > 0 ? ddk_pack_conv_weight_split(canonical, dst, sl.O, sl.I, sl.KH, sl.KW, sl.i_pad, sl.split, sl.split_pad, s)
                              : ddk_pack_conv_weight(canonical, dst, sl.O, sl.I, sl.KH, sl.KW, sl.i_pad, s);
            break;
        case PK_CONVT: rc = sl.i_pad == sl.I ? ddk_pack_convT_weight(canonical, dst, sl.I, sl.O, s)
                                             : ddk_pack_convT_weight_padded(canonical, dst, sl.I, sl.O, sl.i_pad, s); break;
        case PK_ROWS:
            DDK_HIP(hipMemcpy2DAsync(dst, (size_t)sl.ld * sizeof(float), canonical, (size_t)sl.I * sizeof(float), (size_t)sl.I * sizeof(float),
                                     (size_t)sl.O, hipMemcpyDeviceToDevice, as_stream(s)));
            rc = DDK_OK;
            break;
        case PK_LINEAR_T: rc = ddk_pack_linear_T(canonical, dst, sl.O, sl.I, sl.ld, sl.col0, s); break;
        case PK_WINO: rc = ddk_pack_conv_weight_wino(canonical, dst, sl.O, sl.I, sl.i_pad, s); break;
        case PK_LOCAL: rc = ddk_pack_conv_weight_local(canonical, dst, sl.O, sl.I, sl.i_pad, s); break;
        case PK_LOCAL1: rc = ddk_pack_conv1x1_weight_local(canonical, dst, sl.O, sl.I, sl.i_pad, s); break;
        case PK_CONVT_LOCAL: rc = ddk_pack_convT_weight_local(canonical, dst, sl.I, sl.O, s); break;
        case PK_WLOCAL: rc = ddk_pack_conv_weight_wino_local(canonical, dst, sl.O, sl.I, sl.i_pad, s); break;
        case PK_FIRST: rc = ddk_pack_conv_weight_first(canonical, dst, sl.O, sl.I, s); break;
        case PK_CONVT_WINO: rc = ddk_pack_convT_weight_wino(canonical, dst, sl.I, sl.O, sl.i_pad, s); break;
        default: return fail_arg("unet_pack_slot: slot kind");
    }
    DDK_TRY(rc);
    if (sl.attn >= 0) DDK_TRY(fold_attn(u->attn_all[sl.attn], static_cast<float*>(packed), as_stream(s)));
    return DDK_OK;
}

namespace ddk {

struct Layout {
    size_t act = 0;
    size_t qkv = 0, o = 0, ctx = 0, splitk = 0, gn_ws = 0, cl = 0, chain = 0;
    std::vector<size_t> skip;
    size_t xpad = 0, temb = 0, tact = 0;
    size_t off_A = 0, off_B = 0, off_C = 0, off_raw = 0, off_a1 = 0, off_res = 0, off_xn = 0, off_qkv = 0, off_o = 0, off_ctx = 0,
           off_splitk = 0, off_gn = 0, off_xpad = 0, off_temb = 0, off_tact = 0, off_cl = 0, off_chain = 0;
    std::vector<size_t> off_skip;
    size_t total = 0;
};

static size_t al4(size_t n) { return (n + 3) / 4 * 4; }

static void upd(size_t& m, size_t v) { if (v > m) m = v; }

static bool convT_wino_use(int B, int H, int W, int cin, int N) {
    return convT_wino_ok(H, W, cin, N) && convT_wino_splits(B, H, W, cin, N) <= 2;
}
static bool use_wino(const ConvW& cw, int H, int W, int cin, int N) {
    return cw.has_wu && conv_wino_ok(DDK_CONV3X3_S1, H, W, cin, N);
}
static size_t conv3_ws_floats(const ConvW& cw, int B, int H, int W, int cin, int N) {
    if (!use_wino(cw, H, W, cin, N)) return conv_workspace_bytes(DDK_CONV3X3_S1, B, H, W, cin, N) / 4;
    const int s = conv_wino_splits(B, H, W, cin, N);
    return s > 1 ? (size_t)s * B * H * W * N : 0;
}

constexpr int CHAIN_BUFS = 18;
constexpr int CHAIN8_BUFS = 5;

static void res_sizes(const ResW& r, int B, int H, int W, Layout& ly) {
    const size_t M = (size_t)B * H * W;
    upd(ly.act, M * r.co);
    upd(ly.splitk, conv3_ws_floats(r.c1, B, H, W, r.ci_pad, r.co));
    upd(ly.splitk, conv3_ws_floats(r.c2, B, H, W, r.co, r.co));
    if (r.has_res) upd(ly.splitk, conv_workspace_bytes(DDK_CONV1X1, B, H, W, r.ci_pad, r.co) / 4);
    upd(ly.gn_ws, groupnorm_workspace_bytes(B, H * W, r.co, GROUPS) / 4);
    upd(ly.gn_ws, (size_t)2 * GROUPS * (M / 128 + 1));
// ... 161 lines not shown
    CG_SLABS,
    CG_PLAIN
};
struct ConvGnChoice {
    ConvGnPath path = CG_PLAIN;
    int np = 0;
    int cl_splits = 1;
    int splits = 1;
    bool wino = false;
    bool local() const { return path == CG_LOCAL || path == CG_WLOCAL; }
};
static ConvGnChoice classify_conv_gn(const ddk_unet& u, const ConvW& cw, int B, int H, int W, int c0, int c1, int N, bool first_input,
                                     bool cluster, size_t splitk_floats) {
    ConvGnChoice k;
    const int cin = c0 + c1;
    auto is = [&](ConvGnPath p) { k.path = p; return k; };
    if (u.generic) return is(CG_GENERIC);
    if (cw.has_wl && (H * W == 16 || (H * W == 4 && B % 4 == 0)) && conv_gn_local_ok(H, W, cin, c0, N, GROUPS)) return is(CG_LOCAL);
    if (cw.has_wwl && H * W == 64 && conv_gn_wlocal_ok(H, W, cin, c0, N, GROUPS)) return is(CG_WLOCAL);
    k.wino = use_wino(cw, H, W, cin, N);
    if (cw.has_wf && first_input && conv_first_ok(u.cfg.in_ch, N, H, W, GROUPS)) return is(CG_FIRST);
    cluster = cluster && cw.has_wu && conv_wino_cluster_device_ok();
    k.np = cluster ? conv_wino_cluster_np(B, H, W, cin, N, GROUPS) : 0;
    if (k.np > 0 && k.np <= u.cluster_np_max) return is(CG_CLUSTER);
    k.np = cluster && u.cluster_split ? conv_wino_cluster_split_np(B, H, W, cin, N, GROUPS, &k.cl_splits) : 0;
    if (k.np > 0 && k.np <= u.cluster_np_max && (size_t)k.cl_splits * B * H * W * N <= splitk_floats &&
        conv_wino_cluster_pair_words(B, H, W, N) <= CL_PAIR_WORDS)
        return is(CG_CLUSTER_SPLIT);
    k.np = cw.has_wu ? conv_wino_stats_parts(B, H, W, cin, N, GROUPS) : 0;
    if (k.np > 0) return is(CG_PARTS);
    k.splits = k.wino ? conv_wino_splits(B, H, W, cin, N) : conv_splits(DDK_CONV3X3_S1, B, H, W, cin, N);
    return is(k.splits > 1 && groupnorm_workspace_bytes(B, H * W, N, GROUPS) == 0 ? CG_SLABS : CG_PLAIN);
}
static bool conv_gn_is_local(const ddk_unet& u, const ConvW& cw, int B, int H, int W, int c0, int c1, int N) {
    return classify_conv_gn(u, cw, B, H, W, c0, c1, N, false, false, 0).local();
}

static int run_conv_gn(Ctx& c, const ConvW& cw, const float* src0, int c0, const float* src1, int c1, float* raw, const NormW& n,
                       const float* temb, const float* addend, float* out, int H, int W, int N, const AddendSlabs& as = AddendSlabs(),
                       const AddendSlabs& ss = AddendSlabs()) {
    const ConvGnChoice k = classify_conv_gn(c.u, cw, c.B, H, W, c0, c1, N, c.x_first && src0 == c.x_padded && !src1,
                                            c.allow_cluster && c.n_cluster < c.u.cluster_limit, c.ly.splitk);
    if (ss.n > 1 && !k.local()) return fail_arg("run_conv_gn: slab source on a path that cannot sum it");
    if (as.n > 1 && !k.local())
        return fail_arg(k.path == CG_GENERIC ? "run_conv_gn: slab addend / source on the generic path"
                                             : "run_conv_gn: slab addend on a path that cannot sum it");
    const float* bias = cw.has_bias ? c.P + cw.b : nullptr;
    const float *g = c.P + n.g, *b = c.P + n.b;
    float* gnp = c.W + c.ly.off_gn;
    switch (k.path) {
        case CG_GENERIC:
            DDK_TRY(run_conv(c, DDK_CONV3X3_S1, cw, src0, c0, src1, c1, nullptr, raw, H, W, N));
            return groupnorm_mish_generic(raw, g, b, temb, c.u.temb_total, addend, out, c.B, H * W, N, n.c_real, GROUPS, GN_EPS, c.st, c.temb_rows);
        case CG_LOCAL:
        case CG_WLOCAL:
            return (k.path == CG_LOCAL ? conv_gn_local : conv_gn_wlocal)(src0, c0, src1, c1, c.P + (k.path == CG_LOCAL ? cw.wl : cw.wwl), bias, g, b,
                       temb, c.u.temb_total, c.temb_rows, addend, out, c.B, H, W, N, GROUPS, GN_EPS, c.st, as, ss);
        case CG_FIRST:
            DDK_TRY(conv_first(c.x_first, c.P + cw.wf, bias, raw, nullptr, c.B, H, W, c.u.cfg.in_ch, N, GROUPS, nullptr, nullptr, c.st));
            break;
        case CG_CLUSTER:
        case CG_CLUSTER_SPLIT: {
            ++c.n_cluster;
            ddk_conv_args a = c.conv_args(DDK_CONV3X3_S1, cw, src0, c0, src1, c1, out, H, W, N);
            a.resid = addend;
            WinoGnFuse f = c.gn_fuse(n, temb, c.temb_rows);
            if (k.path == CG_CLUSTER_SPLIT) f.pairs = reinterpret_cast<unsigned*>(c.W + c.ly.off_cl + cl_pair_offset(c.B));
            return conv_forward(a, c.st, nullptr, &f);
        }
        case CG_PARTS:
            DDK_TRY(run_conv_parts(c, cw, src0, c0, src1, c1, raw, H, W, N));
            return groupnorm_mish_parts(raw, gnp, k.np, g, b, temb, c.u.temb_total, addend, out, c.B, H * W, N, GROUPS, GN_EPS, c.st, c.temb_rows);
        case CG_SLABS: {
            AddendSlabs sl;
            DDK_TRY(run_conv_slabs(c, DDK_CONV3X3_S1, cw, src0, c0, src1, c1, raw, H, W, N, k.splits, sl));
            return groupnorm_mish_ex(c.W + c.ly.off_splitk, sl.n, sl.stride, sl.bias, g, b, temb, c.u.temb_total, addend, out, c.B, H * W, N,
                                     GROUPS, GN_EPS, nullptr, 0, c.st, c.temb_rows);
        }
        case CG_PLAIN:
            DDK_TRY(run_conv(c, DDK_CONV3X3_S1, cw, src0, c0, src1, c1, nullptr, raw, H, W, N));
            break;
    }
    return groupnorm_mish(raw, g, b, temb, c.u.temb_total, addend, out, c.B, H * W, N, GROUPS, GN_EPS, gnp, c.ly.gn_ws * sizeof(float), c.st,
                          c.temb_rows);
}

static bool res_takes_slab_source(const ddk_unet& u, const ResW& r, int B, int H, int W, int c0) {
    return !u.generic && !r.has_res && conv_gn_is_local(u, r.c1, B, H, W, c0, 0, r.co) && conv_gn_is_local(u, r.c2, B, H, W, r.co, 0, r.co);
}

static int run_res(Ctx& c, const ResW& r, const float* src0, int c0, const float* src1, int c1, float* out, int H, int W,
                   const AddendSlabs& ss = AddendSlabs()) {
    float* raw = c.W + c.ly.off_raw;
    float* a1 = c.W + c.ly.off_a1;
    float* res = c.W + c.ly.off_res;
    const float* addend = src0;
    AddendSlabs as;
    if (ss.n > 1) {
        if (r.has_res || src1) return fail_arg("run_res: slab source with a skip conv or a second source");
        as = ss;
    }
    if (r.has_res) {
        const int rs = conv_splits(DDK_CONV1X1, c.B, H, W, c0 + c1, r.co);
        if (rs > 1 && !conv1x1_sm_ok((long long)c.B * H * W, c0, c1, r.co) && conv_gn_is_local(c.u, r.c1, c.B, H, W, c0, c1, r.co) &&
            conv_gn_is_local(c.u, r.c2, c.B, H, W, r.co, 0, r.co)) {
            DDK_TRY(run_conv_slabs(c, DDK_CONV1X1, r.res, src0, c0, src1, c1, res, H, W, r.co, rs, as));
            addend = c.W + c.ly.off_splitk;
        } else {
            DDK_TRY(run_conv(c, DDK_CONV1X1, r.res, src0, c0, src1, c1, nullptr, res, H, W, r.co));
            addend = res;
        }
    }
    DDK_TRY(run_conv_gn(c, r.c1, src0, c0, src1, c1, raw, r.n1, c.temb + r.temb_off, nullptr, a1, H, W, r.co, AddendSlabs(), ss));
    return run_conv_gn(c, r.c2, a1, r.co, nullptr, 0, raw, r.n2, nullptr, addend, out, H, W, r.co, as);
}

static bool attn_fold_eligible(const ddk_unet& u, const AttnW& a, int B, int H, int W) {
    const long long M = (long long)B * H * W;
    return u.attn_fold && H * W > u.attn_fold_min_hw && (H * W) % 64 == 0 && attn_fold_ok(a.c, HEADS) && conv1x1_ws_ok(M, a.c, a.c) &&
           conv_ln_fold_ok(B, H, W, a.c, 2 * HIDDEN) && B <= 256;
}

static int run_attn(Ctx& c, const AttnW& a, const float* x, float* out, int H, int W) {
    float* xn = c.W + c.ly.off_xn;
    float* qkv = c.W + c.ly.off_qkv;
    float* ctx = c.W + c.ly.off_ctx;
    float* o = c.W + c.ly.off_o;
    const long long M = (long long)c.B * H * W;
    if (!c.u.generic && H * W <= 16 && a.c % 32 == 0 && linattn_small_qkv_ok(H * W, a.c)) {
        DDK_TRY(linattn_small_qkv(x, c.P + a.qkv_op, c.P + a.ln_c1, c.P + a.ln_c2, LN_EPS, ctx, o, c.B, H * W, a.c, HEADS, c.st));
        return run_conv(c, DDK_CONV1X1, a.out, o, HIDDEN, nullptr, 0, x, out, H, W, a.c);
    }
    if (!c.u.generic && attn_fold_eligible(c.u, a, c.B, H, W)) {
        if (c.u.attn_kvctx && attn_kvctx_ok(c.B, H * W, a.c, HEADS) && c.ly.splitk * sizeof(float) >= attn_kvctx_workspace_bytes(c.B, H * W)) {
            DDK_TRY(attn_kvctx(x, c.P + a.qkv_lnw + (size_t)HIDDEN * a.c, c.P + a.ln_c1 + HIDDEN, c.P + a.ln_c2 + HIDDEN, LN_EPS, ctx, c.B, H * W,
                               c.W + c.ly.off_splitk, c.ly.splitk * sizeof(float), c.st));
        } else {
            const ConvLnFold lnkv{c.P + a.ln_c1 + HIDDEN, c.P + a.ln_c2 + HIDDEN, LN_EPS};
            DDK_TRY(run_conv(c, DDK_CONV1X1, a.qkv, x, a.c, nullptr, 0, nullptr, qkv, H, W, 2 * HIDDEN, c.P + a.qkv_lnw + (size_t)HIDDEN * a.c,
                             &lnkv));
            DDK_TRY(linattn_context(qkv, ctx, c.B, H * W, HEADS, c.W + c.ly.off_splitk, c.ly.splitk * sizeof(float), c.st, true));
        }
        float* A = o;
        float* a1 = A + (size_t)c.B * a.c * a.c;
        float* a2 = a1 + (size_t)c.B * a.c;
        DDK_TRY(attn_fold(ctx, c.P + a.qkv_lnw, c.P + a.ln_c1, c.P + a.ln_c2, c.P + a.out.w, a.out.has_bias ? c.P + a.out.b : nullptr, A, a1,
                          a2, c.B, a.c, HEADS, c.st));
        const ConvLnFold lnA{a1, a2, LN_EPS};
        return conv1x1_ws(x, A, nullptr, x, out, M, a.c, &lnA, c.st, c.B);
    }
    if (!c.u.generic && c.u.attn_split && c.allow_cluster && a.c >= 128 && attn_split_ok(c.B, H * W, a.c, HEADS)) {
        float* cl = c.W + c.ly.off_cl;
        DDK_TRY(attn_split(x, c.P + a.qkv_lnw, c.P + a.ln_c1, c.P + a.ln_c2, LN_EPS, ctx, o, c.B, H * W, a.c,
                           reinterpret_cast<unsigned*>(cl + cl_attn_offset(c.B)), cl + cl_counter_floats(c.B), cl_words(cl, c.B).fail, c.st));
        return run_conv(c, DDK_CONV1X1, a.out, o, HIDDEN, nullptr, 0, x, out, H, W, a.c);
    }
    if (!c.u.generic && conv_ln_fold_ok(c.B, H, W, a.c, 3 * HIDDEN)) {
        const ConvLnFold ln{c.P + a.ln_c1, c.P + a.ln_c2, LN_EPS};
        DDK_TRY(run_conv(c, DDK_CONV1X1, a.qkv, x, a.c, nullptr, 0, nullptr, qkv, H, W, 3 * HIDDEN, c.P + a.qkv_lnw, &ln));
    } else {
        DDK_TRY(c.u.generic ? chan_layernorm_generic(x, c.P + a.ln.g, c.P + a.ln.b, xn, M, a.c, a.c_real, LN_EPS, c.st)
                            : chan_layernorm(x, c.P + a.ln.g, c.P + a.ln.b, xn, M, a.c, LN_EPS, c.st));
        DDK_TRY(run_conv(c, DDK_CONV1X1, a.qkv, xn, a.c, nullptr, 0, nullptr, qkv, H, W, 3 * HIDDEN));
    }
    if (H * W <= 256) {
        DDK_TRY(linattn_fused_small(qkv, ctx, o, c.B, H * W, HEADS, c.st));
    } else {
        DDK_TRY(linattn_context(qkv, ctx, c.B, H * W, HEADS, c.W + c.ly.off_splitk, c.ly.splitk * sizeof(float), c.st));
        DDK_TRY(linattn_apply(qkv, ctx, o, c.B, H * W, HEADS, c.st));
    }
    return run_conv(c, DDK_CONV1X1, a.out, o, HIDDEN, nullptr, 0, x, out, H, W, a.c);
}

static bool level_chain_use(const Ctx& c, int H0, int W0, int bit) {
    return c.allow_cluster && (c.u.level_chain & bit) && c.B <= c.u.level_chain_max_batch && c.ly.chain > 0 &&
           (bit == 1 ? level_chain_shape_ok(c.u, H0, W0) : level8_chain_shape_ok(c.u, H0, W0)) && level_chain_device_ok();
}

static int run_level_chain(Ctx& c, int part, const float* in, float* skip, float* out, const float* down_src = nullptr, float* up_out = nullptr) {
    const ddk_unet& u = c.u;
    const int hw = part == 0 ? 16 : 64;
    const bool wino = hw == 64;
    ChainParams p{};
    int n = 0, e = 0;
    const size_t per = (size_t)c.B * hw * 256;
    auto buf = [&](int i) { return c.W + c.ly.off_chain + (size_t)i * per; };
    auto conv3 = [&](const ConvW& cw, const NormW& nw, const float* s0, int c0, const float* s1, int c1, int temb_off, int flags, float* o) {
        ChainOp& op = p.op[n++];
        op = ChainOp{s0, s1, c.P + (wino ? cw.wwl : cw.wl), c.P + cw.b, c.P + nw.g, c.P + nw.b, o, c0, c1, CH_CONV3, flags, temb_off, 256};
    };
    auto conv1 = [&](const ConvW& cw, const float* s0, int c0, const float* s1, int c1, int flags, float* o) {
        ChainOp& op = p.op[n++];
        op = ChainOp{s0, s1, c.P + cw.wl1, c.P + cw.b, nullptr, nullptr, o, c0, c1, CH_CONV1, flags, -1, 256};
    };
    auto attn = [&](const AttnW& a, const float* s0, float* o) {
        ChainOp& op = p.op[n++];
        op = ChainOp{s0, nullptr, c.P + a.qkv_op, nullptr, c.P + a.ln_c1, c.P + a.ln_c2, o, a.c, 0, CH_ATTN, CHF_WAIT | CHF_SIGNAL, -1, HIDDEN};
    };
    const int WS = CHF_WAIT | CHF_SIGNAL, RES = CHF_ADD_KEEP | CHF_SAVE_KEEP;
    auto res_plain = [&](const ResW& r, const float* x, bool external, float* o) {
        float* h = buf(e++);
        conv3(r.c1, r.n1, x, 256, nullptr, 0, r.temb_off, external ? (CHF_SIGNAL | CHF_KEEP_FROM_SRC) : WS, h);
        conv3(r.c2, r.n2, h, 256, nullptr, 0, -1, WS | RES, o);
    };
    auto attn_block = [&](const AttnW& a, const float* x, float* o, bool signals) {
        float* heads = buf(e++);
        attn(a, x, heads);
        conv1(a.out, heads, HIDDEN, nullptr, 0, (signals ? WS : CHF_WAIT) | RES, o);
    };
    auto res_cat = [&](const ResW& r, const float* x, bool x_external, const float* sk, float* o) {
        conv1(r.res, x, 256, sk, 256, (x_external ? 0 : CHF_WAIT) | CHF_SAVE_KEEP2 | CHF_NO_OUT, nullptr);
        float* h = buf(e++);
        conv3(r.c1, r.n1, x, 256, sk, 256, r.temb_off, CHF_SIGNAL, h);
        conv3(r.c2, r.n2, h, 256, nullptr, 0, -1, WS | CHF_ADD_KEEP2 | CHF_SAVE_KEEP, o);
    };
    if (part == 0) {
        const int sh = u.L - 1;
        if (down_src) {
            const ConvW& dc = u.down_conv[sh - 1];
            float* dn = buf(e++);
            ChainOp& op = p.op[n++];
            op = ChainOp{down_src, nullptr, c.P + dc.wl, c.P + dc.b, nullptr, nullptr, dn, 256, 0, CH_CONV3,
                         CHF_DOWN | CHF_NO_GN | CHF_SIGNAL | CHF_SAVE_KEEP, -1, 256};
            in = dn;
        }
        float* d0 = buf(e++);
        res_plain(u.down_res[2 * sh], in, down_src == nullptr, d0);
        float* d1 = buf(e++);
        res_plain(u.down_res[2 * sh + 1], d0, false, d1);
        attn_block(u.down_attn[sh], d1, skip, true);
        float* m1 = buf(e++);
        res_plain(u.mid1, skip, false, m1);
        float* ma = buf(e++);
        attn_block(u.mid_attn, m1, ma, true);
        float* m2 = buf(e++);
        res_plain(u.mid2, ma, false, m2);
        float* u0 = buf(e++);
        res_cat(u.up_res[0], m2, false, skip, u0);
        float* u1 = buf(e++);
        res_plain(u.up_res[1], u0, false, u1);
        if (up_out) {
            float* ua = buf(e++);
            attn_block(u.up_attn[0], u1, ua, true);
            const ConvW& uc = u.up_conv[0];
            ChainOp& op = p.op[n++];
            op = ChainOp{ua, nullptr, c.P + uc.wtl, c.P + uc.b, nullptr, nullptr, up_out, 256, 0, CH_UPT, CHF_WAIT, -1, 256};
        } else {
            attn_block(u.up_attn[0], u1, out, false);
        }
    } else if (part == 1) {
        const int sh = u.L - 2;
        float* d0 = buf(e++);
        res_plain(u.down_res[2 * sh], in, true, d0);
        float* d1 = buf(e++);
        res_plain(u.down_res[2 * sh + 1], d0, false, d1);
        attn_block(u.down_attn[sh], d1, skip, false);
    } else {
        float* u0 = buf(e++);
        res_cat(u.up_res[2], in, true, skip, u0);
        float* u1 = buf(e++);
        res_plain(u.up_res[3], u0, false, u1);
        attn_block(u.up_attn[1], u1, out, false);
    }
    if (n > CH_MAX_OPS || e > (part == 0 ? CHAIN_BUFS : CHAIN8_BUFS)) return fail_arg("level_chain: internal op / buffer count");
    p.n_ops = n;
    p.B = c.B;
    p.hw = hw;
    p.temb = c.temb;
    p.temb_rows = c.temb_rows;
    p.temb_stride = u.temb_total;
    float* cl = c.W + c.ly.off_cl;
    p.cnt = reinterpret_cast<unsigned*>(cl + cl_chain_offset(c.B));
    p.done = p.cnt + (size_t)c.B * 32;
    p.fail = cl_words(cl, c.B).fail;
    p.gn_eps = GN_EPS;
    p.ln_eps = LN_EPS;
    return level_chain_launch(p, c.st);
}

struct StepArgs {
    int64_t* state;
    float* eps_hat;
    long long per;
    StepRule rule;
};

static bool restore_kind(StepKind k) {
    return k == StepKind::Restore || k == StepKind::RestoreMasked || k == StepKind::RestoreMultistep || k == StepKind::RestoreNoisy ||
           k == StepKind::RestoreGray;
}
static int fused_tail_parts(const ddk_unet& u, int B, int H, int W, int cin, StepKind kind, int restore_n = 0) {
    const int chan = u.generic ? pad32(u.cfg.chan) : u.cfg.chan, n_out = u.cfg.in_ch;
    const int npf = u.final_conv.has_wu ? conv_wino_stats_parts(B, H, W, cin, chan, GROUPS) : 0;
    if (npf <= 0 || (restore_kind(kind) && !u.restore_fused)) return 0;
    return final_tail_ok(H * W, chan, GROUPS, n_out, npf, kind, W, restore_n) ? npf : 0;
}

__global__ __launch_bounds__(256) void step_prepare_kernel(const float* __restrict__ x, float* __restrict__ xpad, long long total,
                                                           int C, int c_pad, int64_t* __restrict__ counter,
                                                           int64_t* __restrict__ t_cur, int B) {
    if (blockIdx.x == 0) {
        const int64_t v = *counter;
        for (int b = threadIdx.x; b < B; b += blockDim.x) t_cur[b] = v;
        __syncthreads();
        if (threadIdx.x == 0) *counter = v - 1;
    }
    for (long long i = blockIdx.x * 256LL + threadIdx.x; i < total; i += (long long)gridDim.x * 256) {
// ... 858 lines not shown
```

### downsampled-diffusion_amd/ddk/lib.py

```python
import ctypes as C
import os

import torch

_HERE = os.path.dirname(os.path.abspath(__file__))
LIB_PATH = os.environ.get("DDK_LIB", os.path.join(os.path.dirname(_HERE), "csrc", "libddk.so"))


class DDKError(RuntimeError):
    pass


ABI_VERSION = 400
ERR_CLUSTER = -4


class ConvArgs(C.Structure):
    _fields_ = [
        ("kind", C.c_int), ("src0", C.c_void_p), ("src1", C.c_void_p), ("c0", C.c_int), ("c1", C.c_int),
        ("weight", C.c_void_p), ("bias", C.c_void_p), ("resid", C.c_void_p), ("out", C.c_void_p),
        ("B", C.c_int), ("H", C.c_int), ("W", C.c_int), ("N", C.c_int), ("pre_mish", C.c_int), ("post_mish", C.c_int), ("defer_reduce", C.c_int),
        ("workspace", C.c_void_p), ("workspace_bytes", C.c_size_t), ("weight_wino", C.c_void_p),
        ("gn_partials", C.c_void_p), ("gn_groups", C.c_int), ("mish_out", C.c_void_p), ("dmish_src", C.c_void_p),
    ]


class UnetConfig(C.Structure):
    _fields_ = [("in_ch", C.c_int), ("chan", C.c_int), ("n_levels", C.c_int), ("mults", C.c_int * 8)]


class SamplerArgs(C.Structure):
    _fields_ = [
        ("unet", C.c_void_p), ("packed", C.c_void_p), ("x", C.c_void_p), ("noise", C.c_void_p),
        ("c_recip", C.c_void_p), ("c_recipm1", C.c_void_p), ("c1", C.c_void_p), ("c2", C.c_void_p),
        ("sigma", C.c_void_p), ("B", C.c_int), ("H", C.c_int), ("W", C.c_int), ("t_start", C.c_int),
        ("t_end", C.c_int), ("seed", C.c_uint64), ("stream_id", C.c_uint32), ("use_graph", C.c_int),
        ("workspace", C.c_void_p), ("workspace_bytes", C.c_size_t),
    ]


class InpaintArgs(C.Structure):
    _fields_ = [
        ("timestep_map", C.POINTER(C.c_int64)), ("known", C.c_void_p), ("mask", C.c_void_p), ("ka", C.c_void_p), ("kb", C.c_void_p),
        ("ja", C.c_void_p), ("jb", C.c_void_p),
    ]


class VlbSweepArgs(C.Structure):
    _fields_ = [
        ("unet", C.c_void_p), ("packed", C.c_void_p), ("x", C.c_void_p), ("noise", C.c_void_p),
        ("sqrt_acp", C.c_void_p), ("sqrt_1m_acp", C.c_void_p), ("c_recip", C.c_void_p), ("c_recipm1", C.c_void_p),
        ("c1", C.c_void_p), ("c2", C.c_void_p), ("post_logvar", C.c_void_p), ("B", C.c_int), ("H", C.c_int), ("W", C.c_int),
        ("T", C.c_int), ("seed", C.c_uint64), ("stream_id", C.c_uint32), ("use_graph", C.c_int),
        ("workspace", C.c_void_p), ("workspace_bytes", C.c_size_t), ("vlb_t", C.c_void_p), ("l_simple_t", C.c_void_p),
    ]


class WgradReduceJob(C.Structure):
    _fields_ = [("slab", C.c_void_p), ("grad", C.c_void_p), ("bias_slab", C.c_void_p), ("grad_b", C.c_void_p), ("slab_stride", C.c_longlong),
                ("block0", C.c_longlong), ("splits", C.c_int), ("N", C.c_int), ("ntaps", C.c_int), ("cx", C.c_int), ("c_real", C.c_int),
                ("cw", C.c_int), ("c_off", C.c_int), ("reserved", C.c_int)]


class RowsSumJob(C.Structure):
    _fields_ = [("rows", C.c_void_p), ("out", C.c_void_p * 4), ("batch_stride", C.c_longlong), ("row_stride", C.c_longlong),
                ("block0", C.c_longlong), ("nbatch", C.c_int), ("nrows", C.c_int), ("n", C.c_int), ("reserved", C.c_int)]


class PackJob(C.Structure):
    _fields_ = [("src", C.c_void_p), ("dst", C.c_void_p), ("total", C.c_longlong), ("block0", C.c_longlong), ("kind", C.c_int),
                ("p", C.c_int * 7)]


_P, _I, _LL, _F, _SZ = C.c_void_p, C.c_int, C.c_longlong, C.c_float, C.c_size_t

GRAY_WEIGHTS = {"mean": 1, "luma": 2}

SIGNATURES = {
    "ddk_version": (_I, []),
    "ddk_last_error": (C.c_char_p, []),
    "ddk_device_ok": (_I, []),
    "ddk_nchw_to_nhwc": (_I, [_P, _P, _I, _I, _I, _I, _I, _P]),
    "ddk_nhwc_to_nchw": (_I, [_P, _P, _I, _I, _I, _I, _I, _P]),
    "ddk_pad_channels": (_I, [_P, _P, _LL, _I, _I, _P]),
    "ddk_pack_conv_weight": (_I, [_P, _P, _I, _I, _I, _I, _I, _P]),
    "ddk_pack_convT_weight": (_I, [_P, _P, _I, _I, _P]),
    "ddk_pack_conv_weight_split": (_I, [_P, _P, _I, _I, _I, _I, _I, _I, _I, _P]),
    "ddk_pack_convT_weight_padded": (_I, [_P, _P, _I, _I, _I, _P]),
    "ddk_pack_linear_T": (_I, [_P, _P, _I, _I, _I, _I, _P]),
    "ddk_pack_conv_weight_wino": (_I, [_P, _P, _I, _I, _I, _P]),
    "ddk_pack_conv_weight_wino_dgrad": (_I, [_P, _P, _I, _I, _I, _I, _I, _P]),
    "ddk_conv_wino_splits": (_I, [_I, _I, _I, _I, _I]),
    "ddk_pack_convT_weight_wino": (_I, [_P, _P, _I, _I, _I, _P]),
    "ddk_convT_wino_splits": (_I, [_I, _I, _I, _I, _I]),
    "ddk_conv_gn_partials": (_I, [_I, _I, _I, _I, _I, _I]),
    "ddk_groupnorm_mish_partials": (_I, [_P, _P, _I, _P, _P, _P, _I, _P, _P, _I, _I, _I, _I, _F, _P]),
    "ddk_pack_conv_weight_first": (_I, [_P, _P, _I, _I, _P]),
    "ddk_conv_first_ok": (_I, [_I, _I, _I, _I, _I]),
    "ddk_conv_first": (_I, [_P, _P, _P, _P, _P, _I, _I, _I, _I, _I, _I, _P]),
    "ddk_conv1x1_ws_ok": (_I, [C.c_longlong, _I, _I]),
    "ddk_conv1x1_ws": (_I, [_P, _P, _P, _P, _P, C.c_longlong, _I, _P, _P, _F, _P]),
    "ddk_conv1x1_ws_images": (_I, [_P, _P, _P, _P, _P, C.c_longlong, _I, _P, _P, _F, _I, _P]),
    "ddk_linattn_context_kv": (_I, [_P, _P, _I, _I, _I, _P, _SZ, _P]),
    "ddk_attention_fold": (_I, [_P, _P, _P, _P, _P, _P, _P, _P, _P, _I, _I, _I, _P]),
    "ddk_groupnorm_mish_partials_res1x1": (_I, [_P, _P, _I, _P, _P, _P, _I, _P, _P, _P, _I, _P, _I, _I, _I, _I, _F, _P]),
    "ddk_final_tail": (_I, [_P, _P, _I, _P, _P, _F, _P, _P, _I, _P, _P, _P, _P, _P, _P, _P, _P, _P, C.c_uint64, C.c_uint32, _I, _I, _I, _I, _P]),
    "ddk_pack_conv_weight_local": (_I, [_P, _P, _I, _I, _I, _P]),
    "ddk_pack_conv1x1_weight_local": (_I, [_P, _P, _I, _I, _I, _P]),
    "ddk_pack_convT_weight_local": (_I, [_P, _P, _I, _I, _P]),
    "ddk_pack_conv_weight_wino_local": (_I, [_P, _P, _I, _I, _I, _P]),
    "ddk_conv3x3_gn_mish_wino_ok": (_I, [_I, _I, _I, _I, _I, _I]),
    "ddk_conv3x3_gn_mish_wino": (_I, [_P, _I, _P, _I, _P, _P, _P, _P, _P, _I, _P, _P, _I, _I, _I, _I, _I, _F, _P]),
    "ddk_conv3x3_gn_mish_slabs": (_I, [_P, _I, _LL, _P, _I, _P, _P, _P, _P, _P, _I, _P, _I, _LL, _P, _P, _I, _I, _I, _I, _I, _F, _P]),
    "ddk_attention_kv_context_workspace_bytes": (_SZ, [_I, _I]),
    "ddk_attention_kv_context_ok": (_I, [_I, _I, _I, _I]),
    "ddk_attention_kv_context": (_I, [_P, _P, _P, _P, _F, _P, _I, _I, _P, _SZ, _P]),
    "ddk_attention_split_workspace_bytes": (_SZ, [_I]),
    "ddk_attention_split_ok": (_I, [_I, _I, _I, _I]),
    "ddk_attention_split_from_x": (_I, [_P, _P, _P, _P, _F, _P, _P, _I, _I, _I, _I, _P, _SZ, _P]),
    "ddk_pack_qkv_operand": (_I, [_P, _P, _I, _I, _P]),
    "ddk_linattn_small_from_x": (_I, [_P, _P, _P, _P, _F, _P, _P, _I, _I, _I, _I, _P]),
    "ddk_conv3x3_gn_mish_ok": (_I, [_I, _I, _I, _I, _I, _I]),
    "ddk_conv3x3_gn_mish": (_I, [_P, _I, _P, _I, _P, _P, _P, _P, _P, _I, _P, _P, _I, _I, _I, _I, _I, _F, _P]),
    "ddk_conv_workspace_bytes": (_SZ, [_I, _I, _I, _I, _I, _I]),
    "ddk_conv_splits": (_I, [_I, _I, _I, _I, _I, _I]),
    "ddk_conv_forward": (_I, [C.POINTER(ConvArgs), _P]),
    "ddk_debug_read_stamps": (_I, [_P]),
    "ddk_groupnorm_mish": (_I, [_P, _P, _P, _P, _I, _P, _P, _I, _I, _I, _I, _F, _P, _SZ, _P]),
    "ddk_groupnorm_workspace_bytes": (_SZ, [_I, _I, _I, _I]),
    "ddk_groupnorm_mish_slabs": (_I, [_P, _I, _LL, _P, _P, _P, _P, _I, _P, _P, _I, _I, _I, _I, _F, _P]),
    "ddk_chan_layernorm": (_I, [_P, _P, _P, _P, _LL, _I, _F, _P]),
    "ddk_mish": (_I, [_P, _P, _LL, _P]),
    "ddk_tanh": (_I, [_P, _P, _LL, _P]),
    "ddk_avgpool2": (_I, [_P, _P, _I, _I, _I, _I, _P]),
    "ddk_upsample_nearest2": (_I, [_P, _P, _I, _I, _I, _I, _P]),
    "ddk_add": (_I, [_P, _P, _P, _LL, _P]),
    "ddk_linattn_context_workspace_bytes": (_SZ, [_I, _I, _I]),
    "ddk_linattn_context": (_I, [_P, _P, _I, _I, _I, _P, _SZ, _P]),
    "ddk_linattn_apply": (_I, [_P, _P, _P, _I, _I, _I, _P]),
    "ddk_linattn_fused_small": (_I, [_P, _P, _P, _I, _I, _I, _P]),
    "ddk_time_mlp": (_I, [_P, _P, _P, _P, _P, _P, _P, _P, _I, _I, _P]),
    "ddk_time_proj": (_I, [_P, _P, _P, _P, _I, _I, _I, _P]),
    "ddk_conv1x1_small_n": (_I, [_P, _P, _P, _P, _LL, _I, _I, _P]),
    "ddk_q_sample": (_I, [_P, _P, _P, _P, _P, _P, _I, _LL, _P]),
    "ddk_p_sample_update": (_I, [_P, _P, _P, _P, _P, _P, _P, _P, _P, _I, _LL, C.c_uint64, C.c_uint32, _P]),
    "ddk_p_sample_update_multistep": (_I, [_P, _P, _P, _P, _P, _P, _P, _P, _P, _I, _LL, _P]),
    "ddk_p_sample_update_inpaint": (_I, [_P] * 14 + [_I, _LL, C.c_uint64, C.c_uint32, _P]),
    "ddk_p_sample_update_restore": (_I, [_P, _P, _P, _I] + [_P] * 6 + [_I, _I, _I, _I, C.c_uint64, C.c_uint32, _P]),
    "ddk_p_sample_update_restore_masked": (_I, [_P, _P, _P, _P, _I] + [_P] * 6 + [_I, _I, _I, _I, C.c_uint64, C.c_uint32, _P]),
    "ddk_p_sample_update_restore_multistep": (_I, [_P, _P, _P, _P, _P, _I] + [_P] * 6 + [_I, _I, _I, _I, _P]),
    "ddk_p_sample_update_restore_noisy": (_I, [_P, _P, _P, _P, _I] + [_P] * 8 + [_I, _I, _I, _I, C.c_uint64, C.c_uint32, _P]),
    "ddk_p_sample_update_restore_gray": (_I, [_P, _P, _P, _P, _I, _I] + [_P] * 8 + [_I, _I, _I, _I, C.c_uint64, C.c_uint32, _P]),
    "ddk_randn": (_I, [_P, _LL, C.c_uint64, C.c_uint32, C.c_uint32, _P]),
    "ddk_fix_samples": (_I, [_P, _P, _I, _I, _I, _I, _P]),
    "ddk_sq_err_sum": (_I, [_P, _P, _P, _I, _LL, _P]),
    "ddk_vlb_terms_workspace_bytes": (_SZ, [_I, _LL]),
    "ddk_vlb_terms": (_I, [_P, _P, _P, _P, _P, _P, _P, _P, _P, _P, _P, _P, _I, _LL, _P, _SZ, _P]),
    "ddk_image_metrics_workspace_bytes": (_SZ, [_I, _I, _I, _I]),
    "ddk_image_metrics": (_I, [_P, _P, _P, _I, _I, _I, _I, _P, _P, _P, _SZ, _P]),
    "ddk_unet_create": (_P, [C.POINTER(UnetConfig)]),
    "ddk_unet_destroy": (None, [_P]),
    "ddk_unet_num_slots": (_I, [_P]),
    "ddk_unet_slot_name": (C.c_char_p, [_P, _I]),
    "ddk_unet_slot_numel": (_LL, [_P, _I]),
    "ddk_unet_packed_bytes": (_SZ, [_P]),
    "ddk_unet_pack_slot": (_I, [_P, _I, _P, _P, _P]),
    "ddk_unet_finalize_pack": (_I, [_P, _P, _P]),
    "ddk_unet_workspace_bytes": (_SZ, [_P, _I, _I, _I]),
    "ddk_unet_forward": (_I, [_P, _P, _P, _P, _P, _I, _I, _I, _P, _SZ, _P]),
    "ddk_conv3x3_gn_mish_cluster_ok": (_I, [_I, _I, _I, _I, _I, _I]),
    "ddk_conv3x3_gn_mish_cluster_workspace_bytes": (_SZ, [_I, _I, _I, _I]),
    "ddk_conv3x3_gn_mish_cluster_split_workspace_bytes": (_SZ, [_I, _I, _I, _I, _I, _I]),
    "ddk_conv3x3_gn_mish_cluster": (_I, [_P, _I, _P, _I, _P, _P, _P, _P, _P, _I, _P, _P, _I, _I, _I, _I, _I, _F, _P, _SZ, _P]),
    "ddk_unet_set_option": (_I, [_P, _I, _I]),
    "ddk_debug_cluster_timeouts": (C.c_uint, []),
    "ddk_conv3x3_gn_mish_cluster_check": (_I, [_P, _I, _P]),
    "ddk_unet_cluster_check": (_I, [_P, _P, _I, _I, _I, _P]),
    "ddk_debug_occupy": (_I, [_I, _I, _I, _P]),
    "ddk_debug_clock_probe": (_I, [_P, _I, _P]),
    "ddk_unet_flops": (C.c_double, [_P, _I, _I, _I]),
    "ddk_unet_flops_executed": (C.c_double, [_P, _I, _I, _I]),
    "ddk_sampler_workspace_bytes": (_SZ, [_P, _I, _I, _I, _I]),
    "ddk_sampler_run": (_I, [C.POINTER(SamplerArgs), _P]),
    "ddk_sampler_run_spaced": (_I, [C.POINTER(SamplerArgs), C.POINTER(C.c_int64), _P]),
    "ddk_sampler_multistep_workspace_bytes": (_SZ, [_P, _I, _I, _I, _I]),
    "ddk_sampler_run_multistep": (_I, [C.POINTER(SamplerArgs), C.POINTER(C.c_int64), _P, _P]),
    "ddk_sampler_inpaint_workspace_bytes": (_SZ, [_P, _I, _I, _I, _I]),
    "ddk_sampler_run_inpaint": (_I, [C.POINTER(SamplerArgs), C.POINTER(InpaintArgs), _P]),
    "ddk_sampler_restore_workspace_bytes": (_SZ, [_P, _I, _I, _I, _I]),
    "ddk_sampler_restore_tail_parts": (_I, [_P, _I, _I, _I, _I]),
    "ddk_sampler_run_restore": (_I, [C.POINTER(SamplerArgs), C.POINTER(C.c_int64), _P, _I, _P]),
    "ddk_sampler_restore_masked_workspace_bytes": (_SZ, [_P, _I, _I, _I, _I, _I]),
    "ddk_sampler_restore_masked_tail_parts": (_I, [_P, _I, _I, _I, _I]),
    "ddk_sampler_run_restore_masked": (_I, [C.POINTER(SamplerArgs), C.POINTER(C.c_int64), _P, _P, _I, _P]),
    "ddk_sampler_restore_multistep_workspace_bytes": (_SZ, [_P, _I, _I, _I, _I, _I]),
    "ddk_sampler_restore_multistep_tail_parts": (_I, [_P, _I, _I, _I, _I]),
    "ddk_sampler_run_restore_multistep": (_I, [C.POINTER(SamplerArgs), C.POINTER(C.c_int64), _P, _P, _P, _I, _P]),
    "ddk_sampler_restore_noisy_workspace_bytes": (_SZ, [_P, _I, _I, _I, _I, _I]),
    "ddk_sampler_restore_noisy_tail_parts": (_I, [_P, _I, _I, _I, _I]),
    "ddk_sampler_run_restore_noisy": (_I, [C.POINTER(SamplerArgs), C.POINTER(C.c_int64), _P, _P, _P, _P, _I, _P]),
    "ddk_sampler_restore_gray_workspace_bytes": (_SZ, [_P, _I, _I, _I, _I, _I]),
    "ddk_sampler_restore_gray_tail_parts": (_I, [_P, _I, _I, _I, _I]),
    "ddk_sampler_run_restore_gray": (_I, [C.POINTER(SamplerArgs), C.POINTER(C.c_int64), _P, _P, _P, _P, _I, _I, _P]),
    "ddk_sampler_invalidate": (_I, [_P]),
    "ddk_sampler_release_workspace": (_I, [_P, _P]),
    "ddk_vlb_sweep_workspace_bytes": (_SZ, [_P, _I, _I, _I, _I]),
    "ddk_vlb_sweep_run": (_I, [C.POINTER(VlbSweepArgs), _P]),
    "ddk_pack_conv_weight_dgrad": (_I, [_P, _P, _I, _I, _I, _I, _I, _I, _P]),
    "ddk_zero_stuff2": (_I, [_P, _P, _I, _I, _I, _I, _I, _I, _P]),
    "ddk_conv_wgrad_workspace_bytes": (_SZ, [_I, _I, _I, _I, _I, _I]),
    "ddk_conv_wgrad": (_I, [_I, _P, _P, _P, _I, _I, _I, _I, _I, _I, _I, _I, _P, _SZ, _P]),
    "ddk_conv_wgrad_bias": (_I, [_I, _P, _P, _P, _P, _I, _I, _I, _I, _I, _I, _I, _I, _P, _SZ, _P]),
    "ddk_bias_grad": (_I, [_P, _P, _LL, _I, _I, _P, _SZ, _P]),
    "ddk_groupnorm_train_workspace_bytes": (_SZ, [_I, _I, _I, _I]),
    "ddk_dropout_epoch": (_I, [C.c_uint64, _I, _P]),
    "ddk_groupnorm_mish_train_fwd": (_I, [_P, _P, _P, _P, _I, _P, _F, C.c_uint64, C.c_uint32, _P, _I, _I, _I, _I, _F, _P, _SZ, _P]),
    "ddk_groupnorm_mish_bwd": (_I, [_P, _P, _P, _F, C.c_uint64, C.c_uint32, _P, _P, _P, _I, _I, _I, _I, _F, _P, _SZ, _P]),
    "ddk_groupnorm_mish_train_fwd_slabs": (_I, [_P, _I, _LL, _P, _P, _P, _P, _P, _I, _P, _F, C.c_uint64, C.c_uint32, _P, _I, _I, _I, _I,
                                                _F, _P]),
    "ddk_groupnorm_mish_bwd_slabs": (_I, [_P, _P, _P, _F, C.c_uint64, C.c_uint32, _P, _I, _LL, _P, _P, _I, _I, _I, _I, _F, _P]),
    "ddk_rows_sum": (_I, [_P, _I, _LL, _P, _I, _I, _P]),
    "ddk_rows_sum_batched": (_I, [_P, _I, _LL, _I, _LL, _P, _I, _I, _P]),
    "ddk_rows_sum_targets": (_I, [_P, _I, _LL, _I, _LL, _P, _P, _P, _P, _I, _I, _P]),
    "ddk_multi_add": (_I, [_P, _P, _I, _LL, _P]),
    "ddk_conv_wgrad_defer": (_I, [_I, _P, _P, _P, _P, _I, _I, _I, _I, _I, _I, _I, _I, _P, _SZ, _P, _P]),
    "ddk_wgrad_reduce_jobs": (_I, [_P, _I, _P]),
    "ddk_rows_sum_jobs": (_I, [_P, _I, _P]),
    "ddk_pack_jobs_layout": (_LL, [_P, _I]),
    "ddk_pack_jobs": (_I, [_P, _I, _LL, _P]),
    "ddk_chan_layernorm_bwd": (_I, [_P, _P, _P, _P, _P, _I, C.POINTER(C.c_int), _LL, _I, _F, _P]),
    "ddk_chan_layernorm_bwd_add": (_I, [_P, _P, _P, _P, _P, _P, _I, C.POINTER(C.c_int), _LL, _I, _F, _P]),
    "ddk_groupnorm_mish_generic_train_fwd": (_I, [_P, _P, _P, _P, _I, _P, _F, C.c_uint64, C.c_uint32, _P, _I, _I, _I, _I, _I, _F, _P]),
    "ddk_groupnorm_mish_generic_bwd": (_I, [_P, _P, _P, _F, C.c_uint64, C.c_uint32, _P, _P, _P, _I, _I, _I, _I, _I, _F, _P]),
    "ddk_chan_layernorm_generic": (_I, [_P, _P, _P, _P, _LL, _I, _I, _F, _P]),
    "ddk_chan_layernorm_generic_bwd": (_I, [_P, _P, _P, _P, _P, _P, _I, C.POINTER(C.c_int), _LL, _I, _I, _F, _P]),
    "ddk_linattn_train_workspace_bytes": (_SZ, [_I, _I, _I]),
    "ddk_linattn_stats": (_I, [_P, _P, _I, _I, _I, _P, _SZ, _P]),
    "ddk_linattn_bwd": (_I, [_P, _P, _P, _P, _P, _P, _I, _I, _I, _P, _SZ, _P]),
    "ddk_linattn_bwd_recompute": (_I, [_P, _P, _P, _P, _P, _P, _I, _I, _I, _P, _SZ, _P]),
    "ddk_mish_bwd": (_I, [_P, _P, _P, _LL, _P]),
    "ddk_tanh_bwd": (_I, [_P, _P, _P, _LL, _P]),
    "ddk_avgpool2_bwd": (_I, [_P, _P, _I, _I, _I, _I, _P]),
    "ddk_upsample_nearest2_bwd": (_I, [_P, _P, _I, _I, _I, _I, _P]),
    "ddk_sq_err_grad": (_I, [_P, _P, _P, _P, _I, _LL, _P]),
    "ddk_ae_objective": (_I, [_P, _P, _P, _I, _I, _P, _P]),
    "ddk_ae_objective_bwd": (_I, [_P, _P, _I, _I, _P, _P, _P]),
    "ddk_scale_per_sample": (_I, [_P, _P, _P, _I, _LL, _P]),
    "ddk_conv1x1_small_n_bwd": (_I, [_P, _P, _P, _P, _P, _I, C.POINTER(C.c_int), _LL, _I, _I, _P]),
    "ddk_small_gemm_workspace_bytes": (_SZ, [_I, _I, _I, _I]),
    "ddk_small_gemm": (_I, [_I, _P, _P, _P, _I, _I, _I, _I, _I, _I, _I, _P, _SZ, _P]),
    "ddk_sincos_embed": (_I, [_P, _P, _P, _I, _I, _P]),
    "ddk_bias_act": (_I, [_P, _P, _P, _LL, _I, _P]),
    "ddk_grad_norm_clip": (_I, [_P, _LL, _F, _P, _P, _SZ, _P]),
    "ddk_adam_step": (_I, [_P, _P, _P, _P, _LL, C.c_double, C.c_double, C.c_double, C.c_double, _I, _P, _P]),
    "ddk_ema_update": (_I, [_P, _P, _LL, _F, _P]),
    "ddk_bicubic_resize": (_I, [_P, _P, _P, _P, _P, _P, _LL, _I, _I, _I, _I, _P]),
    "ddk_bicubic_resize_grad": (_I, [_P, _P, _P, _P, _P, _P, _P, _P, _I, _LL, _I, _I, _I, _I, _P]),
    "ddk_conv_small_s2": (_I, [_P, _P, _P, _P, _I, _I, _I, _I, _I, _P]),
    "ddk_conv_small_s2_dgrad": (_I, [_P, _P, _P, _I, _I, _I, _I, _I, _P]),
    "ddk_conv_small_s2_wgrad_workspace_bytes": (_SZ, [_I, _I, _I, _I, _I]),
    "ddk_conv_small_s2_wgrad": (_I, [_P, _P, _P, _P, _I, _I, _I, _I, _I, _P, _SZ, _P]),
    "ddk_convt_small_s2": (_I, [_P, _P, _P, _P, _I, _I, _I, _I, _I, _P]),
    "ddk_convt_small_s2_dgrad": (_I, [_P, _P, _P, _I, _I, _I, _I, _I, _P]),
    "ddk_convt_small_s2_wgrad_workspace_bytes": (_SZ, [_I, _I, _I, _I, _I]),
    "ddk_convt_small_s2_wgrad": (_I, [_P, _P, _P, _P, _I, _I, _I, _I, _I, _P, _SZ, _P]),
}

_lib = None


def load():
    global _lib
# ... 40 lines not shown
```

### downsampled-diffusion_amd/ddk/ops.py

```python
import ctypes as C

import torch

from . import lib as L

CONV3X3_S1, CONV3X3_S2, CONV1X1, CONVT4X4_S2 = 0, 1, 2, 3
GN_GROUPS, GN_EPS, LN_EPS = 8, 1e-5, 1e-5


def pad32(c):
    return (c + 31) // 32 * 32


class _PackEntry:
    __slots__ = ("wref", "out", "job", "fresh", "pooled")


_pack_cache = {}
_weights_epoch = [0]
_pack_table = {}
pack_stats = {"single": 0, "batched_launches": 0, "batched_jobs": 0}
_graph_tables = []
_graph_keep = [_graph_tables]

# ... 1002 lines not shown
                                                       float(drop_p), seed, layer, L.ptr(out), b, h * w, c, groups, eps, L.stream()),
                "groupnorm_mish_train_fwd_slabs")
        return out
    nbytes = lib.ddk_groupnorm_train_workspace_bytes(b, h * w, c, groups)
    ws = _ws(x.device, nbytes, "gn_train") if nbytes else None
    L.check(lib.ddk_groupnorm_mish_train_fwd(L.ptr(_f32(x)), L.ptr(gamma), L.ptr(beta),
                                             temb.data_ptr() if temb is not None else None, stride, L.ptr(addend),
                                             float(drop_p), seed, layer, L.ptr(out), b, h * w, c, groups, eps, L.ptr(ws), nbytes,
                                             L.stream()),
            "groupnorm_mish_train_fwd")
    return out


def groupnorm_mish_bwd(x, gamma, beta, dy, drop_p=0.0, seed=0, layer=0, groups=GN_GROUPS, eps=GN_EPS, acc=None, dy_slabs=None):
    b, h, w, c = x.shape
    dx = torch.empty_like(x)
    part = torch.empty((4, b, c), device=x.device, dtype=torch.float32)
    lib = L.load()
    if dy_slabs is not None:
        L.check(lib.ddk_groupnorm_mish_bwd_slabs(L.ptr(_f32(x)), L.ptr(gamma), L.ptr(beta), float(drop_p), seed, layer, L.ptr(dy_slabs),
                                                 dy_slabs.shape[0], dy_slabs.stride(0), L.ptr(dx), L.ptr(part), b, h * w, c, groups, eps,
                                                 L.stream()), "groupnorm_mish_bwd_slabs")
    else:
        nbytes = lib.ddk_groupnorm_train_workspace_bytes(b, h * w, c, groups)
        ws = _ws(x.device, nbytes, "gn_train") if nbytes else None
        L.check(lib.ddk_groupnorm_mish_bwd(L.ptr(_f32(x)), L.ptr(gamma), L.ptr(beta), float(drop_p), seed, layer, L.ptr(_f32(dy)),
                                           L.ptr(dx), L.ptr(part), b, h * w, c, groups, eps, L.ptr(ws), nbytes, L.stream()),
                "groupnorm_mish_bwd")
    sums = [None, None, None]
    missing = [k for k in range(3) if acc is None or acc[k] is None]
    if acc is not None and any(t is not None for t in acc):
        _rows_sum_targets(part[1], 3, b * c, b, c, [acc[0], acc[1], acc[2]], c)
    if missing:
        out = torch.empty((3, c), device=x.device, dtype=torch.float32)
        L.check(lib.ddk_rows_sum_batched(L.ptr(part[1]), 3, b * c, b, c, L.ptr(out), c, 0, L.stream()), "rows_sum_batched")
        for k in missing:
            sums[k] = out[k]
    return dx, part[0], sums


def groupnorm_mish_generic_train(x, gamma, beta, temb=None, addend=None, drop_p=0.0, seed=0, layer=0, groups=GN_GROUPS, eps=GN_EPS):
    b, h, w, cp = x.shape
    c = gamma.numel()
    out = torch.empty_like(x)
    stride = temb.stride(0) if temb is not None else 0
    L.check(L.load().ddk_groupnorm_mish_generic_train_fwd(L.ptr(_f32(x)), L.ptr(gamma), L.ptr(beta), temb.data_ptr() if temb is not None else None,
                                                          stride, L.ptr(addend), float(drop_p), seed, layer, L.ptr(out), b, h * w, cp, c, groups,
                                                          eps, L.stream()), "groupnorm_mish_generic_train_fwd")
    return out


def groupnorm_mish_generic_bwd(x, gamma, beta, dy, drop_p=0.0, seed=0, layer=0, groups=GN_GROUPS, eps=GN_EPS):
    b, h, w, cp = x.shape
    c = gamma.numel()
    dx = torch.empty_like(x)
    part = torch.empty((4, b, c), device=x.device, dtype=torch.float32)
    lib = L.load()
    L.check(lib.ddk_groupnorm_mish_generic_bwd(L.ptr(_f32(x)), L.ptr(gamma), L.ptr(beta), float(drop_p), seed, layer, L.ptr(_f32(dy)), L.ptr(dx),
                                               L.ptr(part), b, h * w, cp, c, groups, eps, L.stream()), "groupnorm_mish_generic_bwd")
    sums = torch.empty((3, c), device=x.device, dtype=torch.float32)
    L.check(lib.ddk_rows_sum_batched(L.ptr(part[1]), 3, b * c, b, c, L.ptr(sums), c, 0, L.stream()), "rows_sum_batched")
    return dx, part[0], sums


def chan_layernorm_generic(x, g, b, eps=LN_EPS):
    cp, c = x.shape[-1], g.numel()
    out = torch.empty_like(x)
    L.check(L.load().ddk_chan_layernorm_generic(L.ptr(_f32(x)), L.ptr(g.reshape(-1)), L.ptr(b.reshape(-1)), L.ptr(out), x.numel() // cp, cp, c,
                                                eps, L.stream()), "chan_layernorm_generic")
    return out


def chan_layernorm_generic_bwd(x, g, dy, eps=LN_EPS, addend=None):
    cp, c = x.shape[-1], g.numel()
    m = x.numel() // cp
    dx = torch.empty_like(x)
    max_parts = 512
    part = torch.empty((2, max_parts, c), device=x.device, dtype=torch.float32)
    n = C.c_int(0)
    lib = L.load()
    L.check(lib.ddk_chan_layernorm_generic_bwd(L.ptr(_f32(x)), L.ptr(g.reshape(-1)), L.ptr(_f32(dy)), L.ptr(addend), L.ptr(dx), L.ptr(part),
                                               max_parts, C.byref(n), m, cp, c, eps, L.stream()), "chan_layernorm_generic_bwd")
    flat = part.view(-1)
    dg = rows_sum(flat[:n.value * c], n.value, c, c)
    db = rows_sum(flat[n.value * c:2 * n.value * c], n.value, c, c)
    return dx, dg, db


def rows_sum(rows, nrows, row_stride, n, out=None):
    if out is None:
        out = torch.empty(n, device=rows.device, dtype=torch.float32)
    L.check(L.load().ddk_rows_sum(rows.data_ptr(), nrows, row_stride, out.data_ptr(), n, 0, L.stream()), "rows_sum")
    return out


_multi_add_tables = {}


def multi_add_(src, segments):
    key = (str(src.device),) + tuple((int(o), d.data_ptr(), d.numel()) for o, d in segments)
    tab = _multi_add_tables.get(key)
    if tab is None:
        if len(_multi_add_tables) > 64:
            _multi_add_tables.clear()
        host = torch.tensor([[int(o), d.data_ptr(), d.numel()] for o, d in segments], dtype=torch.int64)
        tab = _multi_add_tables[key] = host.to(src.device)
    if torch.cuda.is_current_stream_capturing():
        _graph_keep[-1].append((tab, [d for _, d in segments]))
    L.check(L.load().ddk_multi_add(L.ptr(src), tab.data_ptr(), len(segments), max(d.numel() for _, d in segments), L.stream()), "multi_add")


def chan_layernorm_bwd(x, g, dy, eps=LN_EPS, acc=None, addend=None):
    c = x.shape[-1]
    m = x.numel() // c
    dx = torch.empty_like(x)
    max_parts = 512
    part = torch.empty((2, max_parts, c), device=x.device, dtype=torch.float32)
    n = C.c_int(0)
    lib = L.load()
    L.check(lib.ddk_chan_layernorm_bwd_add(L.ptr(_f32(x)), L.ptr(g.reshape(-1)), L.ptr(_f32(dy)), L.ptr(addend), L.ptr(dx), L.ptr(part),
                                           max_parts, C.byref(n), m, c, eps, L.stream()), "chan_layernorm_bwd")
    if acc is not None and acc[0] is not None and acc[1] is not None:
        _rows_sum_targets(part, 2, n.value * c, n.value, c, [acc[0], acc[1]], c)
        return dx, None, None
    out = torch.empty((2, c), device=x.device, dtype=torch.float32)
    L.check(lib.ddk_rows_sum_batched(L.ptr(part), 2, n.value * c, n.value, c, L.ptr(out), c, 0, L.stream()), "rows_sum_batched")
    return dx, out[0], out[1]


def linattn_small_from_x(x, w_qkv, ln_g, ln_b, heads=4, eps=LN_EPS):
    b, h, w, c = x.shape
    wq = w_qkv.reshape(w_qkv.shape[0], -1).to(torch.float32)
    g, bb = ln_g.reshape(-1).to(torch.float32), ln_b.reshape(-1).to(torch.float32)
    cp = pad32(c)
    lnw = torch.zeros((wq.shape[0], cp), device=x.device, dtype=torch.float32)
    lnw[:, :c] = wq * g[None, :]
    c1 = (wq * g[None, :]).sum(dim=1).contiguous()
    c2 = (wq * bb[None, :]).sum(dim=1).contiguous()
    wop = torch.empty_like(lnw)
    lib = L.load()
    L.check(lib.ddk_pack_qkv_operand(L.ptr(lnw), L.ptr(wop), heads, cp, L.stream()), "pack_qkv_operand")
    ctx = torch.empty((b, heads, 32, 32), device=x.device, dtype=torch.float32)
    out = torch.empty((b, h, w, heads * 32), device=x.device, dtype=torch.float32)
    L.check(lib.ddk_linattn_small_from_x(L.ptr(_f32(x)), L.ptr(wop), L.ptr(c1), L.ptr(c2), eps, L.ptr(ctx), L.ptr(out), b, h * w, c, heads,
                                         L.stream()), "linattn_small_from_x")
    return out, ctx


def attention_split_workspace(batch, device):
    nbytes = L.load().ddk_attention_split_workspace_bytes(batch)
    return torch.zeros(max(nbytes, 128) // 4, device=device, dtype=torch.float32)


def attention_split_from_x(x, w_qkv, ln_g, ln_b, heads=4, eps=LN_EPS, workspace=None):
    b, h, w, c = x.shape
    lib = L.load()
    if not lib.ddk_attention_split_ok(b, h * w, c, heads):
        raise L.DDKError(f"attention_split_from_x: shape {tuple(x.shape)} with {heads} heads not eligible "
                         "(H*W of 64 or 256, C % 32 == 0, C <= 256, 4 heads, 8 * B <= the CU count)")
    wq = w_qkv.reshape(w_qkv.shape[0], -1).to(torch.float32)
    g, bb = ln_g.reshape(-1).to(torch.float32), ln_b.reshape(-1).to(torch.float32)
    lnw = (wq * g[None, :]).contiguous()
    c1 = lnw.sum(dim=1).contiguous()
    c2 = (wq * bb[None, :]).sum(dim=1).contiguous()
    ws = attention_split_workspace(b, x.device) if workspace is None else workspace
    ctx = torch.empty((b, heads, 32, 32), device=x.device, dtype=torch.float32)
    out = torch.empty((b, h, w, heads * 32), device=x.device, dtype=torch.float32)
    L.check(lib.ddk_attention_split_from_x(L.ptr(_f32(x)), L.ptr(lnw), L.ptr(c1), L.ptr(c2), eps, L.ptr(ctx), L.ptr(out), b, h * w, c, heads,
                                           L.ptr(ws), ws.numel() * 4, L.stream()), "attention_split_from_x")
    return out, ctx


def linattn_train(qkv, heads=4):
    out, ctx = linattn(qkv, heads)
    b, h, w, _ = qkv.shape
    stats = torch.empty((b, heads, 2, 32), device=qkv.device, dtype=torch.float32)
    lib = L.load()
    nbytes = lib.ddk_linattn_train_workspace_bytes(b, h * w, heads)
    ws = _ws(qkv.device, nbytes, "linattn_train") if nbytes else None
    L.check(lib.ddk_linattn_stats(L.ptr(qkv), L.ptr(stats), b, h * w, heads, L.ptr(ws), nbytes, L.stream()), "linattn_stats")
    return out, ctx, stats


def linattn_bwd(qkv, dout, ctx, stats, heads=4):
    b, h, w, _ = qkv.shape
    dctx = torch.empty_like(ctx)
    dqkv = torch.empty_like(qkv)
    lib = L.load()
    nbytes = lib.ddk_linattn_train_workspace_bytes(b, h * w, heads)
    ws = _ws(qkv.device, nbytes, "linattn_train") if nbytes else None
    if stats is None:
        scratch = torch.empty((b, heads, 2, 32), device=qkv.device, dtype=torch.float32)
        L.check(lib.ddk_linattn_bwd_recompute(L.ptr(qkv), L.ptr(_f32(dout)), L.ptr(ctx), L.ptr(scratch), L.ptr(dctx), L.ptr(dqkv), b, h * w,
                                              heads, L.ptr(ws), nbytes, L.stream()), "linattn_bwd_recompute")
        return dqkv
    L.check(lib.ddk_linattn_bwd(L.ptr(qkv), L.ptr(_f32(dout)), L.ptr(ctx), L.ptr(stats), L.ptr(dctx), L.ptr(dqkv), b, h * w,
                                heads, L.ptr(ws), nbytes, L.stream()), "linattn_bwd")
    return dqkv


def ae_objective(l_ddpm, l_rec, t, t_rec_max):
    out = torch.empty(3, device=l_ddpm.device, dtype=torch.float32)
    L.check(L.load().ddk_ae_objective(L.ptr(_f32(l_ddpm)), L.ptr(_f32(l_rec)), t.data_ptr(), int(t_rec_max), l_ddpm.numel(), L.ptr(out),
                                      L.stream()), "ae_objective")
    return out


def ae_objective_bwd(g, t, t_rec_max):
    d1 = torch.empty(t.numel(), device=g.device, dtype=torch.float32)
    d2 = torch.empty_like(d1)
    L.check(L.load().ddk_ae_objective_bwd(L.ptr(_f32(g)), t.data_ptr(), int(t_rec_max), t.numel(), L.ptr(d1), L.ptr(d2), L.stream()),
            "ae_objective_bwd")
    return d1, d2


def mish_bwd(x, dy):
    dx = torch.empty_like(x)
    L.check(L.load().ddk_mish_bwd(L.ptr(_f32(x)), L.ptr(_f32(dy)), L.ptr(dx), x.numel(), L.stream()), "mish_bwd")
    return dx


def tanh_bwd(y, dy):
    dx = torch.empty_like(y)
    L.check(L.load().ddk_tanh_bwd(L.ptr(_f32(y)), L.ptr(_f32(dy)), L.ptr(dx), y.numel(), L.stream()), "tanh_bwd")
    return dx


def avgpool2_bwd(dy):
    b, h2, w2, c = dy.shape
    dx = torch.empty((b, 2 * h2, 2 * w2, c), device=dy.device, dtype=torch.float32)
    L.check(L.load().ddk_avgpool2_bwd(L.ptr(_f32(dy)), L.ptr(dx), b, 2 * h2, 2 * w2, c, L.stream()), "avgpool2_bwd")
    return dx


def upsample_nearest2_bwd(dy):
    b, h2, w2, c = dy.shape
    dx = torch.empty((b, h2 // 2, w2 // 2, c), device=dy.device, dtype=torch.float32)
    L.check(L.load().ddk_upsample_nearest2_bwd(L.ptr(_f32(dy)), L.ptr(dx), b, h2 // 2, w2 // 2, c, L.stream()), "upsample_nearest2_bwd")
    return dx


def sq_err_grad(a, b, scale):
    out = torch.empty_like(b)
    bsz = a.shape[0]
    L.check(L.load().ddk_sq_err_grad(L.ptr(_f32(a)), L.ptr(_f32(b)), L.ptr(_f32(scale)), L.ptr(out), bsz, a.numel() // bsz, L.stream()),
            "sq_err_grad")
    return out


def scale_per_sample(x, scale):
    out = torch.empty_like(x)
    bsz = x.shape[0]
    L.check(L.load().ddk_scale_per_sample(L.ptr(_f32(x)), L.ptr(_f32(scale)), L.ptr(out), bsz, x.numel() // bsz, L.stream()),
            "scale_per_sample")
    return out


def conv1x1_small_n_bwd(a, w, dy, acc=None):
    c = a.shape[-1]
    n_out = w.shape[0]
    m = a.numel() // c
    da = torch.empty_like(a)
    max_rows = 1024
    rowlen = n_out * c + n_out
    part = torch.empty((max_rows, rowlen), device=a.device, dtype=torch.float32)
    n = C.c_int(0)
    L.check(L.load().ddk_conv1x1_small_n_bwd(L.ptr(_f32(a)), L.ptr(w.reshape(n_out, c).contiguous()), L.ptr(_f32(dy)), L.ptr(da),
                                             L.ptr(part), max_rows, C.byref(n), m, c, n_out, L.stream()), "conv1x1_small_n_bwd")
    if acc is not None and acc[0] is not None and acc[1] is not None:
        flat = part.view(-1)
        _rows_sum_targets(flat, 1, 0, n.value, rowlen, [acc[0]], n_out * c)
        _rows_sum_targets(flat[n_out * c:], 1, 0, n.value, rowlen, [acc[1]], n_out)
        return da, None, None
    tot = rows_sum(part, n.value, rowlen, rowlen)
    return da, tot[:n_out * c].reshape(n_out, c), tot[n_out * c:]


def small_gemm(mode, a, b, out, m, n, k, lda, ldb, ldc, accumulate=False):
    lib = L.load()
    nbytes = lib.ddk_small_gemm_workspace_bytes(m, n, k, ldc)
    ws = _ws(out.device, nbytes, "small_gemm") if nbytes else None
    L.check(lib.ddk_small_gemm(mode, a.data_ptr(), b.data_ptr(), out.data_ptr(), m, n, k, lda, ldb, ldc, int(accumulate), L.ptr(ws), nbytes,
                               L.stream()), "small_gemm")
    return out


def sincos_embed(t, freqs):
    bsz, dim = t.shape[0], freqs.numel() * 2
    e = torch.empty((bsz, dim), device=t.device, dtype=torch.float32)
    L.check(L.load().ddk_sincos_embed(L.ptr(t), L.ptr(freqs), L.ptr(e), bsz, dim, L.stream()), "sincos_embed")
    return e


def bias_act_(y, bias, want_act):
    act = torch.empty_like(y) if want_act else None
    L.check(L.load().ddk_bias_act(L.ptr(y), L.ptr(bias), L.ptr(act), y.shape[0], y.shape[1], L.stream()), "bias_act")
    return act


def grad_norm_clip(flat_grad, max_norm):
    out = torch.empty(2, device=flat_grad.device, dtype=torch.float32)
    ws = _ws(flat_grad.device, 4096, "norm")
    L.check(L.load().ddk_grad_norm_clip(L.ptr(flat_grad), flat_grad.numel(), float(max_norm), L.ptr(out), L.ptr(ws), 4096, L.stream()),
            "grad_norm_clip")
    return out


def adam_step_(p, g, m, v, lr, step, clip=None, betas=(0.9, 0.999), eps=1e-8):
    L.check(L.load().ddk_adam_step(L.ptr(p), L.ptr(g), L.ptr(m), L.ptr(v), p.numel(), float(lr), float(betas[0]), float(betas[1]),
                                   float(eps), int(step), L.ptr(clip), L.stream()), "adam_step")


def ema_update_(p_ema, p, decay):
    L.check(L.load().ddk_ema_update(L.ptr(p_ema), L.ptr(p), p.numel(), float(decay), L.stream()), "ema_update")


BICUBIC_A = -0.75
_bicubic_cache = {}


def bicubic_taps(n_in, n_out):
    import numpy as np
# ... 154 lines not shown
```

### include/ddk.h

```cpp
#ifndef DDK_H
#define DDK_H

#include <stddef.h>
#include <stdint.h>

#ifdef __cplusplus
extern "C" {
#endif

typedef void* ddk_stream_t;

#define DDK_OK 0
#define DDK_ERR_ARG (-1)
#define DDK_ERR_HIP (-2)
#define DDK_ERR_WORKSPACE (-3)
#define DDK_ERR_CLUSTER (-4)

int ddk_version(void);
const char* ddk_last_error(void);
int ddk_device_ok(void);

int ddk_nchw_to_nhwc(const float* src, float* dst, int B, int C, int H, int W, int c_pad, ddk_stream_t s);
int ddk_nhwc_to_nchw(const float* src, float* dst, int B, int C, int H, int W, int c_stride, ddk_stream_t s);
int ddk_pad_channels(const float* src, float* dst, long long M, int C, int c_pad, ddk_stream_t s);
int ddk_pack_conv_weight(const float* w_oihw, float* dst, int O, int I, int KH, int KW, int i_pad, ddk_stream_t s);
int ddk_pack_conv_weight_split(const float* w_oihw, float* dst, int O, int I, int KH, int KW, int i_pad, int split, int split_pad,
                               ddk_stream_t s);
int ddk_pack_convT_weight(const float* w_iohw, float* dst, int I, int O, ddk_stream_t s);
int ddk_pack_convT_weight_padded(const float* w_iohw, float* dst, int I, int O, int c_pad, ddk_stream_t s);
int ddk_pack_linear_T(const float* w_oi, float* dst, int O, int I, int ld, int col0, ddk_stream_t s);

enum ddk_conv_kind {
    DDK_CONV3X3_S1 = 0,
    DDK_CONV3X3_S2 = 1,
    DDK_CONV1X1 = 2,
    DDK_CONVT4X4_S2 = 3,
    DDK_CONV4X4_S2 = 4
};

typedef struct ddk_conv_args {
    int kind;
    const float* src0;
    const float* src1;
    int c0, c1;
    const float* weight;
    const float* bias;
    const float* resid;
    float* out;
    int B, H, W;
    int N;
    int pre_mish;
    int post_mish;
    int defer_reduce;
    void* workspace;
    size_t workspace_bytes;
    const float* weight_wino;
    float* gn_partials;
    int gn_groups;
    float* mish_out;
    const float* dmish_src;
} ddk_conv_args;

int ddk_pack_conv_weight_wino(const float* w_oihw, float* dst, int O, int I, int i_pad, ddk_stream_t s);
int ddk_conv_gn_partials(int B, int H, int W, int cin, int N, int groups);
int ddk_conv_wino_splits(int B, int H, int W, int cin, int N);
size_t ddk_conv_workspace_bytes(int kind, int B, int H, int W, int cin, int N);
int ddk_conv_splits(int kind, int B, int H, int W, int cin, int N);
int ddk_conv_forward(const ddk_conv_args* a, ddk_stream_t s);
int ddk_debug_read_stamps(unsigned long long* host_out);

int ddk_groupnorm_mish(const float* x, const float* gamma, const float* beta, const float* temb,
                       int temb_stride, const float* addend, float* out, int B, int HW, int C, int groups,
                       float eps, void* workspace, size_t workspace_bytes, ddk_stream_t s);
size_t ddk_groupnorm_workspace_bytes(int B, int HW, int C, int groups);
int ddk_groupnorm_mish_slabs(const float* slabs, int nslab, long long slab_stride, const float* conv_bias,
                             const float* gamma, const float* beta, const float* temb, int temb_stride,
                             const float* addend, float* out, int B, int HW, int C, int groups, float eps,
                             ddk_stream_t s);
int ddk_pack_conv_weight_local(const float* w_oihw, float* dst, int O, int I, int i_pad, ddk_stream_t s);
int ddk_pack_conv1x1_weight_local(const float* w_oi, float* dst, int O, int I, int i_pad, ddk_stream_t s);
int ddk_pack_convT_weight_local(const float* w_iohw, float* dst, int I, int O, ddk_stream_t s);
int ddk_conv3x3_gn_mish_ok(int H, int W, int cin, int c0, int N, int groups);
int ddk_conv3x3_gn_mish(const float* src0, int c0, const float* src1, int c1, const float* weight, const float* bias,
                        const float* gamma, const float* beta, const float* temb, int temb_stride, const float* addend,
                        float* out, int B, int H, int W, int N, int groups, float eps, ddk_stream_t s);
int ddk_groupnorm_mish_partials(const float* x, const float* partials, int tiles_per_image, const float* gamma, const float* beta,
                                const float* temb, int temb_stride, const float* addend, float* out, int B, int HW, int C,
                                int groups, float eps, ddk_stream_t s);
int ddk_pack_conv_weight_first(const float* w_oihw, float* dst, int O, int I, ddk_stream_t s);
int ddk_conv_first_ok(int cin, int N, int H, int W, int groups);
int ddk_conv_first(const float* x, const float* w_first, const float* bias, float* out, float* gn_partials, int B, int H, int W,
                   int cin, int N, int groups, ddk_stream_t s);
int ddk_conv1x1_ws_ok(long long M, int K, int N);
int ddk_conv1x1_ws(const float* x, const float* w, const float* bias, const float* resid, float* out, long long M, int N,
                   const float* ln_c1, const float* ln_c2, float ln_eps, ddk_stream_t s);
int ddk_conv1x1_ws_images(const float* x, const float* w, const float* bias, const float* resid, float* out, long long M, int N,
                          const float* ln_c1, const float* ln_c2, float ln_eps, int images, ddk_stream_t s);
int ddk_groupnorm_mish_partials_res1x1(const float* x, const float* partials, int tiles_per_image, const float* gamma, const float* beta,
                                       const float* temb, int temb_stride, const float* res_x, const float* res_w, const float* res_b,
                                       int res_cin, float* out, int B, int HW, int C, int groups, float eps, ddk_stream_t s);
int ddk_pack_conv_weight_wino_local(const float* w_oihw, float* dst, int O, int I, int i_pad, ddk_stream_t s);
int ddk_conv3x3_gn_mish_wino_ok(int H, int W, int cin, int c0, int N, int groups);
int ddk_conv3x3_gn_mish_wino(const float* src0, int c0, const float* src1, int c1, const float* weight, const float* bias,
                             const float* gamma, const float* beta, const float* temb, int temb_stride, const float* addend,
                             float* out, int B, int H, int W, int N, int groups, float eps, ddk_stream_t s);
int ddk_conv3x3_gn_mish_slabs(const float* src, int src_slabs, long long src_stride, const float* src_bias, int c0, const float* weight,
                              const float* bias, const float* gamma, const float* beta, const float* temb, int temb_stride,
                              const float* addend, int addend_slabs, long long addend_stride, const float* addend_bias, float* out, int B,
                              int H, int W, int N, int groups, float eps, ddk_stream_t s);
int ddk_conv3x3_gn_mish_cluster_ok(int B, int H, int W, int cin, int N, int groups);
int ddk_conv3x3_gn_mish_cluster_check(void* workspace, int B, ddk_stream_t s);
size_t ddk_conv3x3_gn_mish_cluster_workspace_bytes(int B, int H, int W, int N);
size_t ddk_conv3x3_gn_mish_cluster_split_workspace_bytes(int B, int H, int W, int cin, int N, int groups);
int ddk_conv3x3_gn_mish_cluster(const float* src0, int c0, const float* src1, int c1, const float* weight_wino, const float* bias,
                                const float* gamma, const float* beta, const float* temb, int temb_stride, const float* addend,
                                float* out, int B, int H, int W, int N, int groups, float eps, void* workspace, size_t workspace_bytes,
                                ddk_stream_t s);
int ddk_chan_layernorm(const float* x, const float* g, const float* b, float* out, long long M, int C,
                       float eps, ddk_stream_t s);
int ddk_mish(const float* x, float* out, long long n, ddk_stream_t s);
int ddk_tanh(const float* x, float* out, long long n, ddk_stream_t s);
int ddk_avgpool2(const float* x, float* out, int B, int H, int W, int C, ddk_stream_t s);
int ddk_upsample_nearest2(const float* x, float* out, int B, int H, int W, int C, ddk_stream_t s);
int ddk_add(const float* a, const float* b, float* out, long long n, ddk_stream_t s);

size_t ddk_linattn_context_workspace_bytes(int B, int HW, int heads);
int ddk_linattn_context(const float* qkv, float* ctx, int B, int HW, int heads, void* workspace, size_t workspace_bytes, ddk_stream_t s);
int ddk_linattn_context_kv(const float* kv, float* ctx, int B, int HW, int heads, void* workspace, size_t workspace_bytes, ddk_stream_t s);
int ddk_attention_fold(const float* ctx, const float* wqg, const float* c1q, const float* c2q, const float* wout, const float* bout, float* A,
                       float* a1, float* a2, int B, int C, int heads, ddk_stream_t s);
size_t ddk_attention_kv_context_workspace_bytes(int B, int HW);
int ddk_attention_kv_context_ok(int B, int HW, int C, int heads);
int ddk_attention_kv_context(const float* x, const float* w_kv, const float* c1, const float* c2, float ln_eps, float* ctx, int B, int HW,
                             void* workspace, size_t workspace_bytes, ddk_stream_t s);
size_t ddk_attention_split_workspace_bytes(int B);
int ddk_attention_split_ok(int B, int HW, int C, int heads);
int ddk_attention_split_from_x(const float* x, const float* w_folded, const float* c1, const float* c2, float ln_eps, float* ctx, float* out,
                               int B, int HW, int C, int heads, void* workspace, size_t workspace_bytes, ddk_stream_t s);
int ddk_linattn_fused_small(const float* qkv, float* ctx, float* out, int B, int HW, int heads, ddk_stream_t s);
int ddk_linattn_apply(const float* qkv, const float* ctx, float* out, int B, int HW, int heads, ddk_stream_t s);
int ddk_pack_qkv_operand(const float* folded_w, float* dst, int heads, int c_pad, ddk_stream_t s);
int ddk_linattn_small_from_x(const float* x, const float* w_operand, const float* c1, const float* c2, float ln_eps, float* ctx,
                             float* out, int B, int HW, int C, int heads, ddk_stream_t s);

int ddk_time_mlp(const int64_t* t, const float* freqs, const float* w1t, const float* b1, const float* w2t,
                 const float* b2, float* act, float* raw, int B, int dim, ddk_stream_t s);
int ddk_time_proj(const float* act, const float* wt, const float* bias, float* out, int B, int dim, int n_out,
                  ddk_stream_t s);

int ddk_conv1x1_small_n(const float* x, const float* w, const float* bias, float* out, long long M, int C,
                        int n_out, ddk_stream_t s);

int ddk_q_sample(const float* x, const float* eps, const int64_t* t, const float* sqrt_acp,
                 const float* sqrt_1m_acp, float* out, int B, long long per, ddk_stream_t s);
int ddk_p_sample_update(float* x, const float* eps_hat, const float* noise, const int64_t* t,
                        const float* c_recip, const float* c_recipm1, const float* c1, const float* c2,
                        const float* sigma, int B, long long per, uint64_t seed, uint32_t stream_id,
                        ddk_stream_t s);
int ddk_p_sample_update_multistep(float* x, const float* eps_hat, float* x0_hist, const int64_t* t, const float* c_recip,
                                  const float* c_recipm1, const float* c1, const float* c2, const float* c3, int B, long long per,
                                  ddk_stream_t s);
int ddk_p_sample_update_inpaint(float* x, const float* eps_hat, const float* known, const float* mask, const int64_t* t,
                                const float* c_recip, const float* c_recipm1, const float* c1, const float* c2, const float* sigma,
                                const float* ka, const float* kb, const float* ja, const float* jb, int B, long long per, uint64_t seed,
                                uint32_t stream_id, ddk_stream_t s);
int ddk_p_sample_update_restore(float* x, const float* eps_hat, const float* y, int n, const int64_t* t, const float* c_recip,
                                const float* c_recipm1, const float* c1, const float* c2, const float* sigma, int B, int H, int W,
                                int channels, uint64_t seed, uint32_t stream_id, ddk_stream_t s);
int ddk_p_sample_update_restore_masked(float* x, const float* eps_hat, const float* y, const float* mask, int n, const int64_t* t,
                                       const float* c_recip, const float* c_recipm1, const float* c1, const float* c2, const float* sigma,
                                       int B, int H, int W, int channels, uint64_t seed, uint32_t stream_id, ddk_stream_t s);
int ddk_p_sample_update_restore_multistep(float* x, const float* eps_hat, float* x0_hist, const float* y, const float* mask, int n,
                                          const int64_t* t, const float* c_recip, const float* c_recipm1, const float* c1, const float* c2,
                                          const float* c3, int B, int H, int W, int channels, ddk_stream_t s);
int ddk_p_sample_update_restore_noisy(float* x, const float* eps_hat, const float* y, const float* mask, int n, const int64_t* t,
                                      const float* c_recip, const float* c_recipm1, const float* c1, const float* c2, const float* sigma,
                                      const float* lam, const float* sgm, int B, int H, int W, int channels, uint64_t seed, uint32_t stream_id,
                                      ddk_stream_t s);
int ddk_p_sample_update_restore_gray(float* x, const float* eps_hat, const float* y, const float* mask, int n, int weights, const int64_t* t,
                                     const float* c_recip, const float* c_recipm1, const float* c1, const float* c2, const float* sigma,
                                     const float* lam, const float* sgm, int B, int H, int W, int channels, uint64_t seed, uint32_t stream_id,
                                     ddk_stream_t s);
int ddk_final_tail(const float* raw, const float* partials, int tiles_per_image, const float* gamma, const float* beta, float eps,
                   const float* w, const float* bias, int n_out, float* eps_out, float* x, const float* noise, const int64_t* t,
                   const float* c_recip, const float* c_recipm1, const float* c1, const float* c2, const float* sigma, uint64_t seed,
                   uint32_t stream_id, int B, int HW, int C, int groups, ddk_stream_t s);
int ddk_randn(float* out, long long n, uint64_t seed, uint32_t step, uint32_t stream_id, ddk_stream_t s);
int ddk_fix_samples(const float* x_nchw, float* out_nhwc, int B, int C, int H, int W, ddk_stream_t s);
size_t ddk_vlb_terms_workspace_bytes(int B, long long per);
int ddk_vlb_terms(const float* x, const float* x_t, const float* eps_hat, const float* eps, const int64_t* t,
                  const float* c_recip, const float* c_recipm1, const float* c1, const float* c2,
                  const float* post_logvar, float* vlb, float* sqerr, int B, long long per, void* workspace,
                  size_t workspace_bytes, ddk_stream_t s);
int ddk_sq_err_sum(const float* a, const float* b, float* per_sample, int B, long long per, ddk_stream_t s);
size_t ddk_image_metrics_workspace_bytes(int N, int H, int W, int C);
int ddk_image_metrics(const uint8_t* a, const uint8_t* b, const uint8_t* mask, int N, int H, int W, int C,
                      unsigned long long* sq_sum_count, float* ssim, void* workspace, size_t workspace_bytes, ddk_stream_t s);

typedef struct ddk_unet_config {
    int in_ch;
    int chan;
    int n_levels;
    int mults[8];
} ddk_unet_config;

typedef struct ddk_unet ddk_unet;

ddk_unet* ddk_unet_create(const ddk_unet_config* cfg);
void ddk_unet_destroy(ddk_unet* u);
int ddk_unet_num_slots(const ddk_unet* u);
const char* ddk_unet_slot_name(const ddk_unet* u, int slot);
long long ddk_unet_slot_numel(const ddk_unet* u, int slot);
size_t ddk_unet_packed_bytes(const ddk_unet* u);
int ddk_unet_pack_slot(const ddk_unet* u, int slot, const float* canonical, void* packed, ddk_stream_t s);
int ddk_unet_finalize_pack(const ddk_unet* u, void* packed, ddk_stream_t s);
size_t ddk_unet_workspace_bytes(const ddk_unet* u, int B, int H, int W);
int ddk_unet_forward(const ddk_unet* u, const void* packed, const float* x, const int64_t* t, float* out,
                     int B, int H, int W, void* workspace, size_t workspace_bytes, ddk_stream_t s);
#define DDK_OPT_CLUSTER_GROUPNORM 1
#define DDK_OPT_ATTENTION_FOLD 3
#define DDK_OPT_FOLD_DOWNSAMPLE_REDUCE 5
#define DDK_OPT_ATTENTION_KV_CONTEXT 6
#define DDK_OPT_LEVEL_CHAIN 7
#define DDK_OPT_FIRST_GROUPNORM 8
#define DDK_OPT_RESTORE_FUSED_TAIL 12
#define DDK_OPT_ATTENTION_SPLIT 13
int ddk_unet_set_option(ddk_unet* u, int option, int value);
int ddk_unet_cluster_check(const ddk_unet* u, void* workspace, int B, int H, int W, ddk_stream_t s);
unsigned ddk_debug_cluster_timeouts(void);
int ddk_debug_clock_probe(unsigned long long* out, int workgroups, ddk_stream_t s);
int ddk_debug_occupy(int workgroups, int lds_bytes, int microseconds, ddk_stream_t s);
double ddk_unet_flops(const ddk_unet* u, int B, int H, int W);
double ddk_unet_flops_executed(const ddk_unet* u, int B, int H, int W);

typedef struct ddk_sampler_args {
    const ddk_unet* unet;
    const void* packed;
    float* x;
    const float* noise;
    const float* c_recip;
    const float* c_recipm1;
    const float* c1;
    const float* c2;
    const float* sigma;
    int B, H, W;
    int t_start;
    int t_end;
    uint64_t seed;
    uint32_t stream_id;
    int use_graph;
    void* workspace;
    size_t workspace_bytes;
} ddk_sampler_args;

size_t ddk_sampler_workspace_bytes(const ddk_unet* u, int B, int H, int W, int t_start);
int ddk_sampler_run(const ddk_sampler_args* a, ddk_stream_t s);
int ddk_sampler_run_spaced(const ddk_sampler_args* a, const int64_t* timestep_map, ddk_stream_t s);
size_t ddk_sampler_multistep_workspace_bytes(const ddk_unet* u, int B, int H, int W, int t_start);
int ddk_sampler_run_multistep(const ddk_sampler_args* a, const int64_t* timestep_map, const float* c3, ddk_stream_t s);
typedef struct ddk_inpaint_args {
    const int64_t* timestep_map;
    const float* known;
    const float* mask;
    const float* ka;
    const float* kb;
    const float* ja;
    const float* jb;
} ddk_inpaint_args;
size_t ddk_sampler_inpaint_workspace_bytes(const ddk_unet* u, int B, int H, int W, int n_ops);
int ddk_sampler_run_inpaint(const ddk_sampler_args* a, const ddk_inpaint_args* ip, ddk_stream_t s);
size_t ddk_sampler_restore_workspace_bytes(const ddk_unet* u, int B, int H, int W, int t_start);
int ddk_sampler_restore_tail_parts(const ddk_unet* u, int B, int H, int W, int n);
int ddk_sampler_run_restore(const ddk_sampler_args* a, const int64_t* timestep_map, const float* y, int n, ddk_stream_t s);
size_t ddk_sampler_restore_masked_workspace_bytes(const ddk_unet* u, int B, int H, int W, int t_start, int n);
int ddk_sampler_restore_masked_tail_parts(const ddk_unet* u, int B, int H, int W, int n);
int ddk_sampler_run_restore_masked(const ddk_sampler_args* a, const int64_t* timestep_map, const float* y, const float* mask, int n,
                                   ddk_stream_t s);
size_t ddk_sampler_restore_multistep_workspace_bytes(const ddk_unet* u, int B, int H, int W, int t_start, int n);
int ddk_sampler_restore_multistep_tail_parts(const ddk_unet* u, int B, int H, int W, int n);
int ddk_sampler_run_restore_multistep(const ddk_sampler_args* a, const int64_t* timestep_map, const float* c3, const float* y,
                                      const float* mask, int n, ddk_stream_t s);
size_t ddk_sampler_restore_noisy_workspace_bytes(const ddk_unet* u, int B, int H, int W, int t_start, int n);
int ddk_sampler_restore_noisy_tail_parts(const ddk_unet* u, int B, int H, int W, int n);
int ddk_sampler_run_restore_noisy(const ddk_sampler_args* a, const int64_t* timestep_map, const float* lam, const float* sgm, const float* y,
                                  const float* mask, int n, ddk_stream_t s);
size_t ddk_sampler_restore_gray_workspace_bytes(const ddk_unet* u, int B, int H, int W, int t_start, int n);
int ddk_sampler_restore_gray_tail_parts(const ddk_unet* u, int B, int H, int W, int n);
int ddk_sampler_run_restore_gray(const ddk_sampler_args* a, const int64_t* timestep_map, const float* lam, const float* sgm, const float* y,
                                 const float* mask, int n, int weights, ddk_stream_t s);
int ddk_sampler_invalidate(ddk_unet* u);
int ddk_sampler_release_workspace(ddk_unet* u, const void* workspace);
// ... 165 lines not shown
```

Before: 26.50.

## Keep whole 8x8 attention operands resident in LDS and vectorize cross-half exchange

```diff
diff --git a/downsampled-diffusion_amd/csrc/attention.hip b/downsampled-diffusion_amd/csrc/attention.hip
--- a/downsampled-diffusion_amd/csrc/attention.hip
+++ b/downsampled-diffusion_amd/csrc/attention.hip
@@ -677,20 +677,23 @@
 constexpr int AS_CNT = 32;
 constexpr int AS_RING = 4;
 
-template <int ROWS>
+template <int ROWS, bool RES = false>
 struct AttnSplitGeom {
     static_assert(ROWS == 128 || ROWS == 32, "half of a 16x16 or of an 8x8 map");
+    static_assert(!RES || ROWS == 32, "only an 8x8 site's operands are kept whole");
     static constexpr int XP = ROWS / 8;
     static constexpr int NP = XP + 12;
     static constexpr int SLOT = (ROWS + 96) * 32;
+    static constexpr int NSLOT = RES ? 8 : AS_RING;
     static constexpr int NB = ROWS == 128 ? 3 : 1;
     static constexpr int UNITS = ROWS == 128 ? 4 : 3;
     static constexpr int KPART = UNITS * NB * 16 * 64;
     static constexpr int SCR = KPART > 8 * 32 * 33 ? KPART : 8 * 32 * 33;
-    static constexpr int RING_FL = AS_RING * SLOT;
-    static_assert(SCR + 2 * ROWS * DH + ROWS * (DH + 1) <= RING_FL, "k, v, q of the half live behind the scratch area in the drained ring");
+    static constexpr int RING_FL = NSLOT * SLOT;
+    static_assert(SCR + 2 * ROWS * DH + ROWS * (DH + 1) <= RING_FL, "k, v, q of the half live behind the scratch area in the drained slots");
     static constexpr int TAIL = DH * (DH + 4) + 2 * ROWS + 16 * DH + 16 * DH + DH + 192 + AS_REC + 32;
     static constexpr int LDS_FL = RING_FL + TAIL;
+    static_assert(LDS_FL * sizeof(float) <= 160 * 1024, "one workgroup's LDS");
 };
 
 struct AttnSplitParams {
@@ -716,9 +719,48 @@
     else wait_vmcnt<0>();
 }
 
-template <int ROWS>
+__device__ __forceinline__ void wait_vmcnt_le16(int n) {
+    switch (n) {
+        case 0: wait_vmcnt<0>(); break;
+        case 1: wait_vmcnt<1>(); break;
+        case 2: wait_vmcnt<2>(); break;
+        case 3: wait_vmcnt<3>(); break;
+        case 4: wait_vmcnt<4>(); break;
+        case 5: wait_vmcnt<5>(); break;
+        case 6: wait_vmcnt<6>(); break;
+        case 7: wait_vmcnt<7>(); break;
+        case 8: wait_vmcnt<8>(); break;
+        case 9: wait_vmcnt<9>(); break;
+        case 10: wait_vmcnt<10>(); break;
+        case 11: wait_vmcnt<11>(); break;
+        case 12: wait_vmcnt<12>(); break;
+        case 13: wait_vmcnt<13>(); break;
+        case 14: wait_vmcnt<14>(); break;
+        case 15: wait_vmcnt<15>(); break;
+        default: wait_vmcnt<16>(); break;
+    }
+}
+
+typedef float as_f32x4 __attribute__((ext_vector_type(4)));
+__device__ __forceinline__ void as_st_sc1_f4(float* p, float4 v) {
+    const as_f32x4 t = {v.x, v.y, v.z, v.w};
+    asm volatile("global_store_dwordx4 %0, %1, off sc1\n\ts_nop 1" ::"v"(p), "v"(t) : "memory");
+}
+__device__ __forceinline__ void as_ld_sc1_f4x3(float4& a, float4& b, float4& c, const float* pa, const float* pb, const float* pc) {
+    as_f32x4 x, y, z;
+    asm volatile("global_load_dwordx4 %0, %3, off sc1\n\tglobal_load_dwordx4 %1, %4, off sc1\n\tglobal_load_dwordx4 %2, %5, off sc1\n\t"
+                 "s_waitcnt vmcnt(0)"
+                 : "=&v"(x), "=&v"(y), "=&v"(z)
+                 : "v"(pa), "v"(pb), "v"(pc)
+                 : "memory");
+    a = make_float4(x.x, x.y, x.z, x.w); b = make_float4(y.x, y.y, y.z, y.w); c = make_float4(z.x, z.y, z.z, z.w);
+}
+__device__ __forceinline__ float as_pick(float4 v, int i) { return i == 0 ? v.x : i == 1 ? v.y : i == 2 ? v.z : v.w; }
+
+template <int ROWS, bool RES>
 __global__ __launch_bounds__(512) void attn_split_kernel(const AttnSplitParams p) {
-    using G = AttnSplitGeom<ROWS>;
+    constexpr bool LDS_STATS = RES, REC16 = RES;
+    using G = AttnSplitGeom<ROWS, RES>;
     constexpr int HW = 2 * ROWS, HC = 4 * DH;
     extern __shared__ __attribute__((aligned(16))) float smem[];
     float* scr = smem;
@@ -740,6 +782,13 @@
     const float* xb = p.x + ((long long)b * HW + half * ROWS) * C;
     const unsigned lds_base = (unsigned)(size_t)(__attribute__((address_space(3))) float*)smem;
 
+    float cf0 = 0.f, cf1 = 0.f;
+    if (LDS_STATS && wid >= 6) {
+        const int t = tid - 384, n0 = t % 96, n1 = (t + 128) % 96;
+        const int col0 = (n0 >> 5) * HC + h * DH + (n0 & 31), col1 = (n1 >> 5) * HC + h * DH + (n1 & 31);
+        cf0 = t < 96 ? p.c1[col0] : p.c2[col0];
+        if (t < 64) cf1 = p.c2[col1];
+    }
     const int prow = lane >> 3, ppos = lane & 7;
     const int npw = (G::NP - wid + 7) >> 3;
     unsigned voff[4];
@@ -751,28 +800,27 @@
         voff[j] = (unsigned)((src * C + ((ppos ^ ((r >> 1) & 7)) << 2)) * 4);
     }
     auto issue = [&](int chunk) {
-        const unsigned dst = lds_base + (unsigned)(((chunk & (AS_RING - 1)) * G::SLOT) * 4);
+        const unsigned dst = lds_base + (unsigned)(((RES ? chunk : chunk & (AS_RING - 1)) * G::SLOT) * 4);
 #pragma unroll
         for (int j = 0; j < 4; ++j) {
             const int pj = wid + 8 * j;
             if (pj < G::NP) lds_dma16_s(pj < G::XP ? xb : p.w, voff[j] + (unsigned)(chunk * 128), dst + (unsigned)(pj * 1024));
         }
     };
-    for (int c = 0; c < AS_RING - 1 && c < nch; ++c) issue(c);
-    if (tid < 192) {
+    for (int c = 0; c < (RES ? G::NSLOT : AS_RING - 1) && c < nch; ++c) issue(c);
+    if (!LDS_STATS && tid < 192) {
         const int n = tid % 96;
         const int col = (n >> 5) * HC + h * DH + (n & 31);
         cfold[tid] = tid < 96 ? p.c1[col] : p.c2[col];
     }
-    if (tid < 4 * ROWS) {
-        const int row = tid >> 2, sub = tid & 3, n16 = C >> 4;
-        const float4* rp = reinterpret_cast<const float4*>(xb + (long long)row * C);
+    auto row_stats = [&](int row, int sub, auto load4) {
+        const int n16 = C >> 4;
         float4 v[16];
         float s = 0.f;
 #pragma unroll
         for (int i = 0; i < 16; ++i)
             if (i < n16) {
-                v[i] = rp[sub + 4 * i];
+                v[i] = load4(sub + 4 * i);
                 s += (v[i].x + v[i].y) + (v[i].z + v[i].w);
             }
         s += __shfl_xor(s, 1, 64);
@@ -793,6 +841,10 @@
             rowstat[2 * row] = r;
             rowstat[2 * row + 1] = r * mean;
         }
+    };
+    if (!LDS_STATS && tid < 4 * ROWS) {
+        const float4* rp = reinterpret_cast<const float4*>(xb + (long long)(tid >> 2) * C);
+        row_stats(tid >> 2, tid & 3, [&](int f) { return rp[f]; });
     }
 
     const int pl = lane & 31, hl = lane >> 5;
@@ -806,29 +858,49 @@
 #pragma unroll
         for (int r = 0; r < 16; ++r) acc[i][r] = 0.f;
     const int fsw = (pl >> 1) & 7;
-    for (int c = 0; c < nch; ++c) {
-        const int later = nch - 1 - c < AS_RING - 2 ? nch - 1 - c : AS_RING - 2;
-        wait_vmcnt_le(later * npw);
-        asm volatile("s_waitcnt lgkmcnt(0)\n\ts_barrier" ::: "memory");
-        if (c + AS_RING - 1 < nch) issue(c + AS_RING - 1);
-        if (active) {
-            const float* Xs = smem + (c & (AS_RING - 1)) * G::SLOT + pb * (32 * 32);
-            const float* Ws = smem + (c & (AS_RING - 1)) * G::SLOT + ROWS * 32 + blk0 * (32 * 32);
-#pragma unroll
-            for (int q2 = 0; q2 < 2; ++q2) {
-                const int off = pl * 32 + (((2 * (2 * kh + q2) + hl) ^ fsw) << 2);
-                const float4 xv = *reinterpret_cast<const float4*>(Xs + off);
-                float4 wv[G::NB];
-#pragma unroll
-                for (int i = 0; i < G::NB; ++i) wv[i] = *reinterpret_cast<const float4*>(Ws + i * (32 * 32) + off);
-#pragma unroll
-                for (int e = 0; e < 4; ++e) {
-                    const float xe = e == 0 ? xv.x : e == 1 ? xv.y : e == 2 ? xv.z : xv.w;
-#pragma unroll
-                    for (int i = 0; i < G::NB; ++i)
-                        acc[i] = __builtin_amdgcn_mfma_f32_32x32x2f32(e == 0 ? wv[i].x : e == 1 ? wv[i].y : e == 2 ? wv[i].z : wv[i].w, xe, acc[i], 0, 0, 0);
-                }
+    auto project = [&](int slot) {
+        const float* Xs = smem + slot * G::SLOT + pb * (32 * 32);
+        const float* Ws = smem + slot * G::SLOT + ROWS * 32 + blk0 * (32 * 32);
+#pragma unroll
+        for (int q2 = 0; q2 < 2; ++q2) {
+            const int off = pl * 32 + (((2 * (2 * kh + q2) + hl) ^ fsw) << 2);
+            const float4 xv = *reinterpret_cast<const float4*>(Xs + off);
+            float4 wv[G::NB];
+#pragma unroll
+            for (int i = 0; i < G::NB; ++i) wv[i] = *reinterpret_cast<const float4*>(Ws + i * (32 * 32) + off);
+#pragma unroll
+            for (int e = 0; e < 4; ++e) {
+                const float xe = e == 0 ? xv.x : e == 1 ? xv.y : e == 2 ? xv.z : xv.w;
+#pragma unroll
+                for (int i = 0; i < G::NB; ++i)
+                    acc[i] = __builtin_amdgcn_mfma_f32_32x32x2f32(e == 0 ? wv[i].x : e == 1 ? wv[i].y : e == 2 ? wv[i].z : wv[i].w, xe, acc[i], 0, 0, 0);
             }
+        }
+    };
+    if (RES) {
+        constexpr int GRP = 2;
+        for (int c0 = 0; c0 < nch; c0 += GRP) {
+            const int cend = c0 + GRP < nch ? c0 + GRP : nch;
+            wait_vmcnt_le16((nch - cend) * npw);
+            asm volatile("s_waitcnt lgkmcnt(0)\n\ts_barrier" ::: "memory");
+            if (active)
+                for (int c = c0; c < cend; ++c) project(c);
+        }
+        if (wid >= 6) {
+            const int t = tid - 384, row = t >> 2;
+            const float* xr = smem + row * 32;
+            const int sw = (row >> 1) & 7;
+            row_stats(row, t & 3, [&](int f) { return *reinterpret_cast<const float4*>(xr + (f >> 3) * G::SLOT + (((f & 7) ^ sw) << 2)); });
+            cfold[t] = cf0;
+            if (t < 64) cfold[128 + t] = cf1;
+        }
+    } else {
+        for (int c = 0; c < nch; ++c) {
+            const int later = nch - 1 - c < AS_RING - 2 ? nch - 1 - c : AS_RING - 2;
+            wait_vmcnt_le(later * npw);
+            asm volatile("s_waitcnt lgkmcnt(0)\n\ts_barrier" ::: "memory");
+            if (c + AS_RING - 1 < nch) issue(c + AS_RING - 1);
+            if (active) project(c & (AS_RING - 1));
         }
     }
     __syncthreads();
@@ -919,10 +991,19 @@
     unsigned* cnt = p.cnt + (b * 4 + h) * AS_CNT;
     float* rec = p.rec + (long long)(b * 4 + h) * 2 * AS_REC;
     if (wid == 0) {
-        unsigned* mine = reinterpret_cast<unsigned*>(rec + half * AS_REC);
-#pragma unroll
-        for (int i = 0; i < (2 * DH + DH * DH) / 64; ++i)
-            __hip_atomic_store(mine + lane + 64 * i, __float_as_uint(own[lane + 64 * i]), __ATOMIC_RELAXED, __HIP_MEMORY_SCOPE_AGENT);
+        if (REC16) {
+            float* mine = rec + half * AS_REC;
+#pragma unroll
+            for (int i = 0; i < ((2 * DH + DH * DH) / 4 + 63) / 64; ++i) {
+                const int f = lane + 64 * i;
+                if (f < (2 * DH + DH * DH) / 4) as_st_sc1_f4(mine + 4 * f, *reinterpret_cast<const float4*>(own + 4 * f));
+            }
+        } else {
+            unsigned* mine = reinterpret_cast<unsigned*>(rec + half * AS_REC);
+#pragma unroll
+            for (int i = 0; i < (2 * DH + DH * DH) / 64; ++i)
+                __hip_atomic_store(mine + lane + 64 * i, __float_as_uint(own[lane + 64 * i]), __ATOMIC_RELAXED, __HIP_MEMORY_SCOPE_AGENT);
+        }
         asm volatile("s_waitcnt vmcnt(0)" ::: "memory");
         if (lane == 0) {
             __hip_atomic_fetch_add(cnt, 1u, __ATOMIC_RELAXED, __HIP_MEMORY_SCOPE_AGENT);
@@ -932,13 +1013,22 @@
     __syncthreads();
     const bool poisoned = *gave_up != 0;
     if (tid < 256) {
-        const unsigned* theirs = reinterpret_cast<const unsigned*>(rec + (half ^ 1) * AS_REC);
-        const float tm = __uint_as_float(__hip_atomic_load(theirs + md, __ATOMIC_RELAXED, __HIP_MEMORY_SCOPE_AGENT));
-        const float td = __uint_as_float(__hip_atomic_load(theirs + DH + md, __ATOMIC_RELAXED, __HIP_MEMORY_SCOPE_AGENT));
-        float ta[4];
-#pragma unroll
-        for (int e = 0; e < 4; ++e)
-            ta[e] = __uint_as_float(__hip_atomic_load(theirs + 2 * DH + md * DH + me0 + e, __ATOMIC_RELAXED, __HIP_MEMORY_SCOPE_AGENT));
+        float tm, td, ta[4];
+        if (REC16) {
+            const float* theirs = rec + (half ^ 1) * AS_REC;
+            float4 m4, d4, a4;
+            as_ld_sc1_f4x3(m4, d4, a4, theirs + (md & ~3), theirs + DH + (md & ~3), theirs + 2 * DH + md * DH + me0);
+            tm = as_pick(m4, md & 3);
+            td = as_pick(d4, md & 3);
+            ta[0] = a4.x; ta[1] = a4.y; ta[2] = a4.z; ta[3] = a4.w;
+        } else {
+            const unsigned* theirs = reinterpret_cast<const unsigned*>(rec + (half ^ 1) * AS_REC);
+            tm = __uint_as_float(__hip_atomic_load(theirs + md, __ATOMIC_RELAXED, __HIP_MEMORY_SCOPE_AGENT));
+            td = __uint_as_float(__hip_atomic_load(theirs + DH + md, __ATOMIC_RELAXED, __HIP_MEMORY_SCOPE_AGENT));
+#pragma unroll
+            for (int e = 0; e < 4; ++e)
+                ta[e] = __uint_as_float(__hip_atomic_load(theirs + 2 * DH + md * DH + me0 + e, __ATOMIC_RELAXED, __HIP_MEMORY_SCOPE_AGENT));
+        }
         if (tid == 0) cl_depart(cnt, cnt + 1, 2u);
         const float om = own[md], od = own[DH + md];
         const float m0 = half ? tm : om, m1 = half ? om : tm;
@@ -1184,10 +1274,15 @@
     DDK_HIP(hipFuncSetAttribute(reinterpret_cast<const void*>(linattn_small_kernel<256>), hipFuncAttributeMaxDynamicSharedMemorySize, 160 * 1024));
     DDK_HIP(hipFuncSetAttribute(reinterpret_cast<const void*>(linattn_small_qkv_kernel<1>), hipFuncAttributeMaxDynamicSharedMemorySize, 160 * 1024));
     DDK_HIP(hipFuncSetAttribute(reinterpret_cast<const void*>(linattn_small_qkv_kernel<4>), hipFuncAttributeMaxDynamicSharedMemorySize, 160 * 1024));
-    DDK_HIP(hipFuncSetAttribute(reinterpret_cast<const void*>(attn_split_kernel<128>), hipFuncAttributeMaxDynamicSharedMemorySize,
-                                (int)(AttnSplitGeom<128>::LDS_FL * sizeof(float))));
-    DDK_HIP(hipFuncSetAttribute(reinterpret_cast<const void*>(attn_split_kernel<32>), hipFuncAttributeMaxDynamicSharedMemorySize,
-                                (int)(AttnSplitGeom<32>::LDS_FL * sizeof(float))));
+    const struct {
+        const void* fn;
+        size_t floats;
+    } split_forms[] = {
+        {reinterpret_cast<const void*>(attn_split_kernel<128, false>), AttnSplitGeom<128, false>::LDS_FL},
+        {reinterpret_cast<const void*>(attn_split_kernel<32, false>), AttnSplitGeom<32, false>::LDS_FL},
+        {reinterpret_cast<const void*>(attn_split_kernel<32, true>), AttnSplitGeom<32, true>::LDS_FL},
+    };
+    for (const auto& f : split_forms) DDK_HIP(hipFuncSetAttribute(f.fn, hipFuncAttributeMaxDynamicSharedMemorySize, (int)(f.floats * sizeof(float))));
     return DDK_OK;
 }
 
@@ -1252,17 +1347,23 @@
 size_t attn_split_workspace_bytes(int B) { return B > 0 ? (32 + attn_split_counter_words(B) + attn_split_record_floats(B)) * sizeof(float) : 0; }
 unsigned attention_cluster_timeouts() { return cl_timeouts_read(); }
 
+template <int ROWS, bool RES>
+static void attn_split_launch(const AttnSplitParams& p, int B, hipStream_t st) {
+    using G = AttnSplitGeom<ROWS, RES>;
+    hipLaunchKernelGGL((attn_split_kernel<ROWS, RES>), dim3(2, 4, (unsigned)B), dim3(512), G::LDS_FL * sizeof(float), st, p);
+}
 int attn_split(const float* x, const float* w, const float* c1, const float* c2, float ln_eps, float* ctx, float* out, int B, int HW, int C,
-               unsigned* counters, float* records, unsigned* fail, hipStream_t st) {
+               unsigned* counters, float* records, unsigned* fail, int form, hipStream_t st) {
     DDK_REQUIRE(x && w && c1 && c2 && ctx && out && counters && records, "attn_split: null pointer");
+    DDK_REQUIRE(form == 1 || form == 2, "attn_split: form must be 1 (ring) or 2 (resident operands, 16-byte records)");
     DDK_REQUIRE(attn_split_ok(B, HW, C, 4), "attn_split: needs H*W of 64 or 256, C % 32 == 0, C <= 256, 4 heads, 8 * B <= the CU count of a whole MI355X");
     DDK_REQUIRE(aligned16(x) && aligned16(w) && aligned16(ctx) && aligned16(out) && aligned16(counters) && aligned16(records), "attn_split: alignment");
     DDK_TRY(ensure_device_init());
     const AttnSplitParams p{x, w, c1, c2, ln_eps, ctx, out, counters, records, fail, C};
-    if (HW == 256)
-        hipLaunchKernelGGL(attn_split_kernel<128>, dim3(2, 4, (unsigned)B), dim3(512), AttnSplitGeom<128>::LDS_FL * sizeof(float), st, p);
-    else
-        hipLaunchKernelGGL(attn_split_kernel<32>, dim3(2, 4, (unsigned)B), dim3(512), AttnSplitGeom<32>::LDS_FL * sizeof(float), st, p);
+    static_assert(AttnSplitGeom<32, true>::NSLOT * 32 >= 256, "every eligible C has its slots");
+    if (HW == 256) attn_split_launch<128, false>(p, B, st);
+    else if (form == 1) attn_split_launch<32, false>(p, B, st);
+    else attn_split_launch<32, true>(p, B, st);
     return check_launch("attn_split_kernel");
 }
 
@@ -1307,8 +1408,8 @@
 }
 size_t ddk_attention_split_workspace_bytes(int B) { return ddk::attn_split_workspace_bytes(B); }
 int ddk_attention_split_ok(int B, int HW, int C, int heads) { return ddk::attn_split_ok(B, HW, C, heads) ? 1 : 0; }
-int ddk_attention_split_from_x(const float* x, const float* w_folded, const float* c1, const float* c2, float ln_eps, float* ctx, float* out,
-                               int B, int HW, int C, int heads, void* workspace, size_t workspace_bytes, ddk_stream_t s) {
+int ddk_attention_split_from_x_form(const float* x, const float* w_folded, const float* c1, const float* c2, float ln_eps, float* ctx, float* out,
+                                    int B, int HW, int C, int heads, int form, void* workspace, size_t workspace_bytes, ddk_stream_t s) {
     using namespace ddk;
     DDK_REQUIRE(workspace && B > 0 && heads == 4, "attention_split_from_x: arguments (4 heads)");
     if (workspace_bytes < attn_split_workspace_bytes(B)) {
@@ -1317,7 +1418,11 @@
     }
     unsigned* words = static_cast<unsigned*>(workspace);
     return attn_split(x, w_folded, c1, c2, ln_eps, ctx, out, B, HW, C, words + 32, static_cast<float*>(workspace) + 32 + attn_split_counter_words(B),
-                      words, as_stream(s));
+                      words, form, as_stream(s));
+}
+int ddk_attention_split_from_x(const float* x, const float* w_folded, const float* c1, const float* c2, float ln_eps, float* ctx, float* out,
+                               int B, int HW, int C, int heads, void* workspace, size_t workspace_bytes, ddk_stream_t s) {
+    return ddk_attention_split_from_x_form(x, w_folded, c1, c2, ln_eps, ctx, out, B, HW, C, heads, 2, workspace, workspace_bytes, s);
 }
 int ddk_attention_fold(const float* ctx, const float* wqg, const float* c1q, const float* c2q, const float* wout, const float* bout, float* A,
                        float* a1, float* a2, int B, int C, int heads, ddk_stream_t s) {
diff --git a/downsampled-diffusion_amd/csrc/ddk_internal.h b/downsampled-diffusion_amd/csrc/ddk_internal.h
--- a/downsampled-diffusion_amd/csrc/ddk_internal.h
+++ b/downsampled-diffusion_amd/csrc/ddk_internal.h
@@ -243,7 +243,7 @@
 size_t attn_split_counter_words(int B);
 size_t attn_split_record_floats(int B);
 int attn_split(const float* x, const float* w, const float* c1, const float* c2, float ln_eps, float* ctx, float* out, int B, int HW, int C,
-               unsigned* counters, float* records, unsigned* fail, hipStream_t st);
+               unsigned* counters, float* records, unsigned* fail, int form, hipStream_t st);
 bool linattn_small_qkv_ok(int HW, int C);
 int linattn_small_qkv_init_device();
 int qkv_operand_pack(const float* lnw, float* wop, int heads, int cp, hipStream_t st);
diff --git a/downsampled-diffusion_amd/csrc/unet_plan.hip b/downsampled-diffusion_amd/csrc/unet_plan.hip
--- a/downsampled-diffusion_amd/csrc/unet_plan.hip
+++ b/downsampled-diffusion_amd/csrc/unet_plan.hip
@@ -110,7 +110,7 @@
     int cluster_np_max = 8;
     bool cluster_split = true;
     bool attn_kvctx = true;
-    bool attn_split = true;
+    int attn_split = 2;
     bool fold_down_reduce = false;
     bool restore_fused = true;
     bool first_gn = true;
@@ -410,7 +410,7 @@
         {DDK_OPT_ATTENTION_KV_CONTEXT, true, [](ddk_unet& p, int v) { p.attn_kvctx = v != 0; }},
         {DDK_OPT_FIRST_GROUPNORM, true, [](ddk_unet& p, int v) { p.first_gn = v != 0; }},
         {DDK_OPT_RESTORE_FUSED_TAIL, true, [](ddk_unet& p, int v) { p.restore_fused = v != 0; }},
-        {DDK_OPT_ATTENTION_SPLIT, true, [](ddk_unet& p, int v) { p.attn_split = v != 0; }},
+        {DDK_OPT_ATTENTION_SPLIT, true, [](ddk_unet& p, int v) { p.attn_split = v <= 0 ? 0 : v == 1 ? 1 : 2; }},
         {DDK_OPT_LEVEL_CHAIN, true, [](ddk_unet& p, int v) {
              p.level_chain = v == 1 ? 9 : v == 2 ? 1 : v == 3 ? 15 : v == 4 ? 6 : v == 8 ? 2 : v == 16 ? 4 : v != 0 ? 9 : 0;
          }},
@@ -878,7 +878,7 @@
     if (!c.u.generic && c.u.attn_split && c.allow_cluster && a.c >= 128 && attn_split_ok(c.B, H * W, a.c, HEADS)) {
         float* cl = c.W + c.ly.off_cl;
         DDK_TRY(attn_split(x, c.P + a.qkv_lnw, c.P + a.ln_c1, c.P + a.ln_c2, LN_EPS, ctx, o, c.B, H * W, a.c,
-                           reinterpret_cast<unsigned*>(cl + cl_attn_offset(c.B)), cl + cl_counter_floats(c.B), cl_words(cl, c.B).fail, c.st));
+                           reinterpret_cast<unsigned*>(cl + cl_attn_offset(c.B)), cl + cl_counter_floats(c.B), cl_words(cl, c.B).fail, c.u.attn_split, c.st));
         return run_conv(c, DDK_CONV1X1, a.out, o, HIDDEN, nullptr, 0, x, out, H, W, a.c);
     }
     if (!c.u.generic && conv_ln_fold_ok(c.B, H, W, a.c, 3 * HIDDEN)) {
diff --git a/downsampled-diffusion_amd/ddk/lib.py b/downsampled-diffusion_amd/ddk/lib.py
--- a/downsampled-diffusion_amd/ddk/lib.py
+++ b/downsampled-diffusion_amd/ddk/lib.py
@@ -118,6 +118,7 @@
     "ddk_attention_split_workspace_bytes": (_SZ, [_I]),
     "ddk_attention_split_ok": (_I, [_I, _I, _I, _I]),
     "ddk_attention_split_from_x": (_I, [_P, _P, _P, _P, _F, _P, _P, _I, _I, _I, _I, _P, _SZ, _P]),
+    "ddk_attention_split_from_x_form": (_I, [_P, _P, _P, _P, _F, _P, _P, _I, _I, _I, _I, _I, _P, _SZ, _P]),
     "ddk_pack_qkv_operand": (_I, [_P, _P, _I, _I, _P]),
     "ddk_linattn_small_from_x": (_I, [_P, _P, _P, _P, _F, _P, _P, _I, _I, _I, _I, _P]),
     "ddk_conv3x3_gn_mish_ok": (_I, [_I, _I, _I, _I, _I, _I]),
diff --git a/downsampled-diffusion_amd/ddk/ops.py b/downsampled-diffusion_amd/ddk/ops.py
--- a/downsampled-diffusion_amd/ddk/ops.py
+++ b/downsampled-diffusion_amd/ddk/ops.py
@@ -1178,7 +1178,7 @@
     return torch.zeros(max(nbytes, 128) // 4, device=device, dtype=torch.float32)
 
 
-def attention_split_from_x(x, w_qkv, ln_g, ln_b, heads=4, eps=LN_EPS, workspace=None):
+def attention_split_from_x(x, w_qkv, ln_g, ln_b, heads=4, eps=LN_EPS, workspace=None, form=None, out=None, ctx=None):
     b, h, w, c = x.shape
     lib = L.load()
     if not lib.ddk_attention_split_ok(b, h * w, c, heads):
@@ -1190,10 +1190,18 @@
     c1 = lnw.sum(dim=1).contiguous()
     c2 = (wq * bb[None, :]).sum(dim=1).contiguous()
     ws = attention_split_workspace(b, x.device) if workspace is None else workspace
-    ctx = torch.empty((b, heads, 32, 32), device=x.device, dtype=torch.float32)
-    out = torch.empty((b, h, w, heads * 32), device=x.device, dtype=torch.float32)
-    L.check(lib.ddk_attention_split_from_x(L.ptr(_f32(x)), L.ptr(lnw), L.ptr(c1), L.ptr(c2), eps, L.ptr(ctx), L.ptr(out), b, h * w, c, heads,
-                                           L.ptr(ws), ws.numel() * 4, L.stream()), "attention_split_from_x")
+    if ctx is None:
+        ctx = torch.empty((b, heads, 32, 32), device=x.device, dtype=torch.float32)
+    if out is None:
+        out = torch.empty((b, h, w, heads * 32), device=x.device, dtype=torch.float32)
+    assert ctx.shape == (b, heads, 32, 32) and out.shape == (b, h, w, heads * 32) and ctx.is_contiguous() and out.is_contiguous()
+    assert ctx.dtype == out.dtype == torch.float32 and ctx.device == out.device == x.device
+    if form is None:
+        L.check(lib.ddk_attention_split_from_x(L.ptr(_f32(x)), L.ptr(lnw), L.ptr(c1), L.ptr(c2), eps, L.ptr(ctx), L.ptr(out), b, h * w, c, heads,
+                                               L.ptr(ws), ws.numel() * 4, L.stream()), "attention_split_from_x")
+    else:
+        L.check(lib.ddk_attention_split_from_x_form(L.ptr(_f32(x)), L.ptr(lnw), L.ptr(c1), L.ptr(c2), eps, L.ptr(ctx), L.ptr(out), b, h * w, c,
+                                                    heads, int(form), L.ptr(ws), ws.numel() * 4, L.stream()), "attention_split_from_x_form")
     return out, ctx
 
 
diff --git a/include/ddk.h b/include/ddk.h
--- a/include/ddk.h
+++ b/include/ddk.h
@@ -137,6 +137,9 @@
 int ddk_attention_split_ok(int B, int HW, int C, int heads);
 int ddk_attention_split_from_x(const float* x, const float* w_folded, const float* c1, const float* c2, float ln_eps, float* ctx, float* out,
                                int B, int HW, int C, int heads, void* workspace, size_t workspace_bytes, ddk_stream_t s);
+int ddk_attention_split_from_x_form(const float* x, const float* w_folded, const float* c1, const float* c2, float ln_eps, float* ctx,
+                                    float* out, int B, int HW, int C, int heads, int form, void* workspace, size_t workspace_bytes,
+                                    ddk_stream_t s);
 int ddk_linattn_fused_small(const float* qkv, float* ctx, float* out, int B, int HW, int heads, ddk_stream_t s);
 int ddk_linattn_apply(const float* qkv, const float* ctx, float* out, int B, int HW, int heads, ddk_stream_t s);
 int ddk_pack_qkv_operand(const float* folded_w, float* dst, int heads, int c_pad, ddk_stream_t s);
```

Result: no change. 26.56, median of 6 (+0.2%).
